# ChenyangLEI/All-In-One-Deflicker

Hardware: AMD Instinct MI355X
Metric: atlas-fit sampled points/sec (stage1, 10k iters) @1/2/4/8 GPU; PSNR vs ref (higher is better)
Workload: dtype f32 (MLP chains f16x3: operands split into 2 fp16 of their value scaled per row, 3 partial products; weight-gradient GEMM bf16x6; fp32 accumulate)

## Files before the change

### all-in-one-deflicker_amd/atlasfit.py

```python
import ctypes as C
import os
import sys

import numpy as np

NET_MAPPING1, NET_ATLAS, NET_MAPPING2, NET_ALPHA = 0, 1, 2, 3
_HERE = os.path.dirname(os.path.abspath(__file__))
_LIB_PATH = os.path.join(_HERE, "lib", "libatlasfit.so")
_lib = None

ABI_SYMBOLS = [
    "af_create", "af_destroy", "af_last_error", "af_upload_video", "af_param_count", "af_set_params",
    "af_get_params", "af_get_adam_state", "af_set_adam_state", "af_pretrain", "af_train_steps",
    "af_render_frame", "af_render_frame_u8", "af_render_frame_at", "af_psnr", "af_sync", "af_debug_forward", "af_set_debug", "af_get_last_grads",
    "af_set_timing", "af_get_timing", "af_step_work", "af_loss_width", "af_config_size", "af_debug_records", "af_debug_plan",
    "af_resize_bilinear", "af_resize_area", "af_flow_consistency", "af_debug_dw_clocks", "af_debug_step_clocks", "af_set_dw_mode", "af_set_mlp_mode", "af_debug_dw_schedule",
    "af_debug_set_dw_cost", "af_debug_tiles", "af_get_modes",
    "af_render_layers", "af_mapping_area", "af_render_atlas_texture", "af_render_edit", "af_render_loss_maps",
    "af_warp_error_pair", "af_warp_error",
    "af_filter_create", "af_filter_destroy", "af_filter_param_count", "af_filter_set_params", "af_filter_reset", "af_filter_frame",
    "af_filter_debug_activation", "af_conv2d",
    "af_raft_create", "af_raft_destroy", "af_raft_param_count", "af_raft_info", "af_raft_set_params", "af_raft_encode", "af_raft_flow",
    "af_raft_step", "af_raft_lookup", "af_raft_debug_activation", "af_raft_conv2d", "af_raft_gru", "af_raft_instance_norm",
]


AF_ERANGE = -6


class AtlasFitError(RuntimeError):
    def __init__(self, code, msg):
        super().__init__("atlasfit error %d: %s" % (code, msg))
        self.code = code


class AfConfig(C.Structure):
    _fields_ = [
        ("resx", C.c_int32), ("resy", C.c_int32), ("number_of_frames", C.c_int32),
        ("samples_batch", C.c_int32),
        ("number_of_channels_mapping1", C.c_int32), ("number_of_layers_mapping1", C.c_int32),
        ("number_of_channels_atlas", C.c_int32), ("number_of_layers_atlas", C.c_int32),
        ("positional_encoding_num_atlas", C.c_int32),
        ("use_positional_encoding_mapping1", C.c_int32),
        ("derivative_amount", C.c_int32),
        ("include_global_rigidity_loss", C.c_int32),
        ("global_rigidity_derivative_amount_fg", C.c_int32),
        ("stop_global_rigidity", C.c_int32),
        ("use_gradient_loss", C.c_int32),
        ("rgb_coeff", C.c_float), ("gradient_loss_coeff", C.c_float), ("rigidity_coeff", C.c_float),
        ("optical_flow_coeff", C.c_float),
        ("global_rigidity_coeff_fg", C.c_float),
        ("uv_mapping_scale", C.c_float),
        ("lr", C.c_float),
        ("pretrain_batch", C.c_int32),
        ("two_layer", C.c_int32),
        ("number_of_channels_mapping2", C.c_int32), ("number_of_layers_mapping2", C.c_int32),
        ("number_of_channels_alpha", C.c_int32), ("number_of_layers_alpha", C.c_int32),
        ("positional_encoding_num_alpha", C.c_int32),
        ("use_positional_encoding_mapping2", C.c_int32),
        ("global_rigidity_derivative_amount_bg", C.c_int32),
        ("stop_bootstrapping_iteration", C.c_int32),
        ("global_rigidity_coeff_bg", C.c_float),
        ("alpha_bootstrapping_factor", C.c_float), ("alpha_flow_factor", C.c_float), ("sparsity_coeff", C.c_float),
        ("number_of_positional_encoding_mapping1", C.c_int32), ("number_of_positional_encoding_mapping2", C.c_int32),
        ("reserved", C.c_int32 * 2),
    ]


REFERENCE_CONFIG = {
    "maximum_number_of_frames": 200, "iters_num": 10001, "samples_batch": 10000, "optical_flow_coeff": 500.0,
    "evaluate_every": 10000, "derivative_amount": 1, "rgb_coeff": 5000, "rigidity_coeff": 1.0,
    "uv_mapping_scale": 0.8, "pretrain_mapping1": True, "pretrain_mapping2": True,
    "alpha_bootstrapping_factor": 2000.0, "alpha_flow_factor": 4900.0, "positional_encoding_num_alpha": 5,
    "number_of_channels_atlas": 256, "number_of_layers_atlas": 8, "number_of_channels_alpha": 256,
    "number_of_layers_alpha": 8, "stop_bootstrapping_iteration": 10000, "number_of_channels_mapping1": 256,
    "number_of_layers_mapping1": 6, "number_of_channels_mapping2": 256, "number_of_layers_mapping2": 4,
    "gradient_loss_coeff": 1000, "use_gradient_loss": True, "sparsity_coeff": 1000.0,
    "positional_encoding_num_atlas": 10, "use_positional_encoding_mapping1": False,
    "number_of_positional_encoding_mapping1": 4, "use_positional_encoding_mapping2": False,
    "number_of_positional_encoding_mapping2": 2, "pretrain_iter_number": 100, "load_checkpoint": False,
    "checkpoint_path": "", "include_global_rigidity_loss": True, "global_rigidity_derivative_amount_fg": 100,
    "global_rigidity_derivative_amount_bg": 100, "global_rigidity_coeff_fg": 5.0, "global_rigidity_coeff_bg": 50.0,
    "stop_global_rigidity": 5000,
}


def default_config(resx, resy, number_of_frames, config=None, two_layer=False, **over):
    cfg = dict(REFERENCE_CONFIG)
    if config:
        cfg.update(config)
    cfg.update(over)
    c = AfConfig()
    c.two_layer = int(bool(two_layer))
    c.number_of_channels_mapping2 = int(cfg["number_of_channels_mapping2"])
    c.number_of_layers_mapping2 = int(cfg["number_of_layers_mapping2"])
    c.number_of_channels_alpha = int(cfg["number_of_channels_alpha"])
    c.number_of_layers_alpha = int(cfg["number_of_layers_alpha"])
    c.positional_encoding_num_alpha = int(cfg["positional_encoding_num_alpha"])
    c.use_positional_encoding_mapping2 = int(bool(cfg["use_positional_encoding_mapping2"]))
    c.number_of_positional_encoding_mapping1 = int(cfg.get("number_of_positional_encoding_mapping1", 4))
    c.number_of_positional_encoding_mapping2 = int(cfg.get("number_of_positional_encoding_mapping2", 2))
    c.global_rigidity_derivative_amount_bg = int(cfg["global_rigidity_derivative_amount_bg"])
    c.stop_bootstrapping_iteration = int(cfg["stop_bootstrapping_iteration"])
    c.global_rigidity_coeff_bg = float(cfg["global_rigidity_coeff_bg"])
    c.alpha_bootstrapping_factor = float(cfg["alpha_bootstrapping_factor"])
    c.alpha_flow_factor = float(cfg["alpha_flow_factor"])
    c.sparsity_coeff = float(cfg["sparsity_coeff"])
    c.resx, c.resy, c.number_of_frames = int(resx), int(resy), int(number_of_frames)
    c.samples_batch = int(cfg["samples_batch"])
    c.number_of_channels_mapping1 = int(cfg["number_of_channels_mapping1"])
    c.number_of_layers_mapping1 = int(cfg["number_of_layers_mapping1"])
    c.number_of_channels_atlas = int(cfg["number_of_channels_atlas"])
    c.number_of_layers_atlas = int(cfg["number_of_layers_atlas"])
    c.positional_encoding_num_atlas = int(cfg["positional_encoding_num_atlas"])
    c.use_positional_encoding_mapping1 = int(bool(cfg["use_positional_encoding_mapping1"]))
    c.derivative_amount = int(cfg["derivative_amount"])
    c.include_global_rigidity_loss = int(bool(cfg["include_global_rigidity_loss"]))
    c.global_rigidity_derivative_amount_fg = int(cfg["global_rigidity_derivative_amount_fg"])
    c.stop_global_rigidity = int(cfg["stop_global_rigidity"])
    c.use_gradient_loss = int(bool(cfg["use_gradient_loss"]))
    c.rgb_coeff = float(cfg["rgb_coeff"])
    c.gradient_loss_coeff = float(cfg["gradient_loss_coeff"])
    c.rigidity_coeff = float(cfg["rigidity_coeff"])
    c.optical_flow_coeff = float(cfg["optical_flow_coeff"])
    c.global_rigidity_coeff_fg = float(cfg["global_rigidity_coeff_fg"])
    c.uv_mapping_scale = float(cfg["uv_mapping_scale"])
    c.lr = float(cfg.get("lr", 1e-4))
    c.pretrain_batch = int(cfg.get("pretrain_batch", 10000))
    return c


def load_library(path=None):
    global _lib
    if _lib is not None:
        return _lib
    import torch
    path = path or os.environ.get("AF_LIB_PATH") or _LIB_PATH
    if not os.path.exists(path):
        raise AtlasFitError(-100, "libatlasfit.so not built: run `python %s`" % os.path.join(_HERE, "build.py"))
    lib = C.CDLL(path)
    vp, i32, i64, u64, sz = C.c_void_p, C.c_int, C.c_int64, C.c_uint64, C.c_size_t
    fp = C.POINTER(C.c_float)
    sig = {
        "af_create": (i32, [C.POINTER(AfConfig), i32, C.POINTER(vp)]),
        "af_destroy": (None, [vp]),
        "af_last_error": (C.c_char_p, [vp]),
        "af_upload_video": (i32, [vp, vp, vp, vp, vp, vp, vp, i32]),
        "af_param_count": (sz, [vp, i32]),
        "af_set_params": (i32, [vp, i32, vp, sz]),
        "af_get_params": (i32, [vp, i32, vp, sz]),
        "af_get_adam_state": (i32, [vp, i32, vp, vp, C.POINTER(i64)]),
        "af_set_adam_state": (i32, [vp, i32, vp, vp, i64]),
        "af_pretrain": (i32, [vp, i32, i32, vp, vp, u64, vp]),
        "af_train_steps": (i32, [vp, i32, i32, vp, u64, vp]),
        "af_render_frame": (i32, [vp, i32, vp, C.POINTER(C.c_double)]),
        "af_render_frame_u8": (i32, [vp, i32, vp, vp, i32, C.POINTER(C.c_double)]),
        "af_render_frame_at": (i32, [vp, i32, i32, i32, vp, vp, vp, C.POINTER(C.c_double), i32]),
        "af_psnr": (i32, [vp, C.POINTER(C.c_double), vp]),
        "af_sync": (i32, [vp]),
        "af_debug_forward": (i32, [vp, i32, vp, i32, vp]),
        "af_set_debug": (i32, [vp, i32]),
        "af_get_last_grads": (i32, [vp, i32, vp, sz]),
        "af_set_timing": (i32, [vp, i32]),
        "af_get_timing": (i32, [vp, vp, vp, vp, i32]),
        "af_step_work": (i32, [vp, i32, C.POINTER(i64 * 4), C.POINTER(C.c_double)]),
        "af_loss_width": (i32, [vp]),
        "af_config_size": (sz, []),
        "af_debug_records": (i32, [vp, vp, i32, vp]),
        "af_debug_plan": (i32, [i32, i32, i32, i32, C.POINTER(i32 * 3)]),
        "af_resize_bilinear": (i32, [i32, vp, i32, i32, i32, i32, vp, i32, i32, i64, i64, i64, C.c_double, C.c_double, i32]),
        "af_resize_area": (i32, [i32, vp, i32, i32, i32, vp, i32, i32, i32]),
        "af_flow_consistency": (i32, [i32, vp, vp, i32, i32, vp, i64, i64, C.c_float, i32]),
        "af_debug_dw_clocks": (i32, [vp, i32, vp, i32]),
        "af_debug_step_clocks": (i32, [vp, i32, vp, i32]),
        "af_debug_dw_schedule": (i32, [vp, i32, vp, i32]),
        "af_set_dw_mode": (i32, [vp, i32]),
        "af_set_mlp_mode": (i32, [vp, i32]),
        "af_debug_set_dw_cost": (i32, [vp, vp, C.c_double]),
        "af_debug_tiles": (i32, [vp, i32, i32, i32, i32, i32, i32, vp]),
        "af_get_modes": (i32, [vp, C.POINTER(i32), C.POINTER(i32)]),
        "af_render_layers": (i32, [vp, i32, vp, vp, vp, vp, vp]),
        "af_mapping_area": (i32, [vp, i32, vp]),
        "af_render_atlas_texture": (i32, [vp, i32, C.c_float, C.c_float, C.c_float, vp]),
        "af_render_edit": (i32, [vp, i32, i32, vp, vp, vp, vp, vp, vp, vp, vp, vp]),
        "af_render_loss_maps": (i32, [vp, i32, vp, vp, vp, vp, vp, vp, vp]),
        "af_warp_error_pair": (i32, [i32, vp, vp, vp, vp, i32, i32, i32, C.POINTER(C.c_double), vp, vp, i32]),
        "af_warp_error": (i32, [vp, i32, i32, vp, C.POINTER(C.c_double)]),
    }
    for name, (res, args) in sig.items():
        f = getattr(lib, name)
        f.restype, f.argtypes = res, args
    if lib.af_config_size() != C.sizeof(AfConfig):
        raise AtlasFitError(-101, "af_config mirror (%d B) does not match libatlasfit.so (%d B): rebuild" % (C.sizeof(AfConfig), lib.af_config_size()))
    _lib = lib
    return lib


def _f32(a):
    return np.ascontiguousarray(a, dtype=np.float32)


def _ptr(a):
    return a.ctypes.data_as(C.c_void_p) if a is not None else None


def imlp_shapes(net, cfg=None, pe_atlas=10, pe_alpha=5):
    hid = {NET_MAPPING1: 256, NET_MAPPING2: 256, NET_ATLAS: 256, NET_ALPHA: 256}
    nl = {NET_MAPPING1: 6, NET_MAPPING2: 4, NET_ATLAS: 8, NET_ALPHA: 8}
    if cfg is not None:
        hid = {NET_MAPPING1: cfg.number_of_channels_mapping1, NET_MAPPING2: cfg.number_of_channels_mapping2,
               NET_ATLAS: cfg.number_of_channels_atlas, NET_ALPHA: cfg.number_of_channels_alpha}
        nl = {NET_MAPPING1: cfg.number_of_layers_mapping1, NET_MAPPING2: cfg.number_of_layers_mapping2,
              NET_ATLAS: cfg.number_of_layers_atlas, NET_ALPHA: cfg.number_of_layers_alpha}
        pe_atlas, pe_alpha = cfg.positional_encoding_num_atlas, cfg.positional_encoding_num_alpha
    if net not in hid:
        raise ValueError("net")
    h, L = int(hid[net]), int(nl[net])
    enc = {NET_MAPPING1: 3, NET_MAPPING2: 3, NET_ATLAS: 4 * pe_atlas, NET_ALPHA: 6 * pe_alpha}[net]
    if cfg is not None:
        if net == NET_MAPPING1 and cfg.use_positional_encoding_mapping1:
            enc = 6 * int(cfg.number_of_positional_encoding_mapping1)
        if net == NET_MAPPING2 and cfg.use_positional_encoding_mapping2:
            enc = 6 * int(cfg.number_of_positional_encoding_mapping2)
    out = {NET_MAPPING1: 2, NET_MAPPING2: 2, NET_ATLAS: 3, NET_ALPHA: 1}[net]
    skips = (4, 7) if net == NET_ATLAS else ()
    dims = []
    for i in range(L):
        fan_in = enc if i == 0 else (h + enc if i in skips else h)
        dims.append((out if i == L - 1 else h, fan_in))
    return dims


def flatten_state_dict(sd, net, cfg=None):
    parts = []
    for i, (o, k) in enumerate(imlp_shapes(net, cfg)):
        w = np.asarray(sd["hidden.%d.weight" % i].detach().cpu().numpy() if hasattr(sd["hidden.%d.weight" % i], "detach") else sd["hidden.%d.weight" % i], dtype=np.float32)
        b = np.asarray(sd["hidden.%d.bias" % i].detach().cpu().numpy() if hasattr(sd["hidden.%d.bias" % i], "detach") else sd["hidden.%d.bias" % i], dtype=np.float32)
        assert w.shape == (o, k) and b.shape == (o,), (i, w.shape, b.shape)
        parts += [w.reshape(-1), b]
    return np.concatenate(parts)


def unflatten_state_dict(flat, net, cfg=None):
    out, off = {}, 0
    for i, (o, k) in enumerate(imlp_shapes(net, cfg)):
        out["hidden.%d.weight" % i] = flat[off:off + o * k].reshape(o, k).copy(); off += o * k
        out["hidden.%d.bias" % i] = flat[off:off + o].copy(); off += o
    assert off == flat.size
    return out


def _util_chk(rc):
# ... 455 lines not shown
```

### all-in-one-deflicker_amd/csrc/af_dev.h

```cpp
#pragma once
#include <stdint.h>

#define AF_HID        256
#define AF_TROWS      32
#define AF_TILE_F     (AF_HID * AF_TROWS)
#define AF_CHUNK_MAX  65536
#define AF_MAX_LAYERS 8
#define AF_KIND_MAP_PE 4
#define AF_MAX_NETS   4
#define AF_REC_F      16
#define AF_LOSS_W     16

enum { AF_NET_MAP1 = 0, AF_NET_ATLAS = 1, AF_NET_MAP2 = 2, AF_NET_ALPHA = 3 };
enum { AF_IN_XYT = 0, AF_IN_PE2 = 1, AF_IN_PE3 = 2 };

enum { REC_RGB = 0, REC_DX = 3, REC_DY = 6, REC_FF = 9, REC_FB = 11, REC_MF = 13, REC_MB = 14, REC_FG = 15 };

enum { DW_8x8 = 0, DW_8x2 = 1, DW_8x1 = 2, DW_1x8 = 3, DW_1x2 = 4 };

struct AfChunk { uint32_t off; uint32_t bytes; };

struct FwdArgs {
  const float* wimg;
  const float* bias;
  const float* in;
  const float* in1;
  float* out;
  float* acts;
  uint32_t* masks;
  float* pe_tile;
  float in_scale, in_shift0, in_shift1;
  int split_row;
  int tile0;
  int NT;
  int nt_stride;
  const int* live_rows;
  int live_base;
  int nl;
};

struct BwdArgs {
  const float* wimg;
  const float* out;
  const float* dout;
  const uint32_t* masks;
  float* dz;
  float* dz_last;
  const float* pe_tile;
  float* din0; float* din1;
  float din_scale;
  int split_row;
  int nrows;
  int tile0;
  int NT;
  int nt_stride;
  const int* live_rows; int live_base;
  int nl;
};

#define AF_STAMP_WG 4096
struct MultiFwd { int n; int net[AF_MAX_NETS]; int wg_end[AF_MAX_NETS]; FwdArgs a[AF_MAX_NETS]; unsigned long long* wg_stamp; };
struct MultiBwd { int n; int net[AF_MAX_NETS]; int wg_end[AF_MAX_NETS]; BwdArgs a[AF_MAX_NETS]; int nprod; unsigned long long* wg_stamp; };

struct DwJob {
  const float* A; const float* B;
  uint32_t a_stride, b_stride;
  int shape;
  uint32_t part_off;
  uint32_t part_blk;
  int live_base;
  const int* live_rows;
};
struct DwSeg { int job, t0, t1, slot; };
#define DW_MAXSEG 16
struct DwArgs {
  const DwJob* jobs; const DwSeg* segs;
  float* partial;
  unsigned long long* wg_clock;
  unsigned long long* wg_stamp;
};

#if defined(__HIPCC__)
#include <hip/hip_runtime.h>
#define AF_STAMP(m, i) if ((m).wg_stamp && threadIdx.x == 0 && blockIdx.x < AF_STAMP_WG) { (m).wg_stamp[blockIdx.x * 4 + 2 * (i)] = __builtin_amdgcn_s_memrealtime(); (m).wg_stamp[blockIdx.x * 4 + 2 * (i) + 1] = __builtin_amdgcn_s_memtime(); }
typedef float    f32x16 __attribute__((ext_vector_type(16)));
typedef float    f32x4  __attribute__((ext_vector_type(4)));
typedef uint32_t u32x4  __attribute__((ext_vector_type(4)));

#define AF_DEV __device__ __forceinline__

AF_DEV __amdgpu_buffer_rsrc_t af_rsrc(const void* p, uint32_t bytes) {
  return __builtin_amdgcn_make_buffer_rsrc((void*)p, 0, (int)bytes, 0x00020000);
}
AF_DEV __amdgpu_buffer_rsrc_t af_rsrc_uniform(const void* p, uint32_t bytes) {
  const uint64_t a = (uint64_t)p;
  const uint32_t lo = __builtin_amdgcn_readfirstlane((uint32_t)a), hi = __builtin_amdgcn_readfirstlane((uint32_t)(a >> 32));
  return __builtin_amdgcn_make_buffer_rsrc((void*)(((uint64_t)hi << 32) | lo), 0, (int)__builtin_amdgcn_readfirstlane(bytes), 0x00020000);
}
AF_DEV float af_bl32(__amdgpu_buffer_rsrc_t r, int voff, int soff) {
  return __builtin_bit_cast(float, __builtin_amdgcn_raw_buffer_load_b32(r, voff, soff, 0));
}
AF_DEV f32x4 af_bl128(__amdgpu_buffer_rsrc_t r, int voff, int soff) {
  return __builtin_bit_cast(f32x4, __builtin_amdgcn_raw_buffer_load_b128(r, voff, soff, 0));
}
AF_DEV void af_bs32(float v, __amdgpu_buffer_rsrc_t r, int voff, int soff) {
  __builtin_amdgcn_raw_buffer_store_b32(__builtin_bit_cast(uint32_t, v), r, voff, soff, 0);
}
#ifndef AF_TILE_AUX
#define AF_TILE_AUX 2
#endif
AF_DEV void af_bs32_tile(float v, __amdgpu_buffer_rsrc_t r, int voff, int soff) {
  __builtin_amdgcn_raw_buffer_store_b32(__builtin_bit_cast(uint32_t, v), r, voff, soff, AF_TILE_AUX);
}
AF_DEV void af_bs128(f32x4 v, __amdgpu_buffer_rsrc_t r, int voff, int soff) {
  __builtin_amdgcn_raw_buffer_store_b128(__builtin_bit_cast(u32x4, v), r, voff, soff, 0);
}
AF_DEV void af_glds16(const void* g, void* lds) {
  __builtin_amdgcn_global_load_lds((const __attribute__((address_space(1))) void*)g,
                                   (__attribute__((address_space(3))) void*)lds, 16, 0, 0);
}
AF_DEV void af_wait_vm0() { asm volatile("s_waitcnt vmcnt(0)" ::: "memory"); }

AF_DEV void af_stage_chunk(const char* src, uint32_t bytes, char* dst, int tid, int wave) {
  const int nit = (int)(bytes >> 12);
  for (int it = 0; it < nit; ++it)
    af_glds16(src + it * 4096 + tid * 16, dst + it * 4096 + wave * 1024);
}

__host__ __device__ inline int af_pe_slot_of_feature(int pe_kind, int e) {
  if (pe_kind != 2) return e;
  int h, rho;
  if (e < 24) { int k = e / 6, c = e % 6; h = k >> 1; rho = (k & 1) * 6 + c; }
  else        { int c = e - 24; h = c / 3; rho = 12 + c % 3; }
  return ((rho >> 2) << 3) + (h << 2) + (rho & 3);
}
__host__ __device__ inline uint32_t af_img_index(uint32_t mpad, uint32_t m, uint32_t k) {
  return ((((k >> 3) * 2 + ((k >> 2) & 1)) * mpad + m) << 2) + (k & 3);
}
#endif
```

### all-in-one-deflicker_amd/csrc/elem.h

```cpp
#pragma once
#include "af_dev.h"

struct PackArgs {
  const float* frames;
  const float* flow_f;
  const float* flow_b;
  const float* mask_f;
  const float* mask_b;
  const float* mask_fg;
  float* table;
  int resx, resy, F;
  unsigned long long* nvalid;
};

struct ResizeArgs {
  const void* src; int src_u8;
  int sh, sw, ch;
  float* dst; int dh, dw;
  long long pix_stride, ch_stride, offset;
  double scale0, scale1;
};
enum { AREA_GENERAL = 0, AREA_BLOCK = 1, AREA_2X2 = 2 };
struct AreaArgs {
  const unsigned char* src; int sh, sw, ch;
// ... 17 lines not shown
  int N, resx, resy, F;
  float half_main, half_grad, half_frames;
  int d_local, d_global, nseg;
  float* coords;
  float* x0_tile;
  float* samples;
  int* counts;
  float* coords2;
  float* x0_tile2;
  float* coordsA;
  int d_global2;
  int* flow_rank;
  unsigned long long* scan;
  uint32_t epoch;
  unsigned long long* ticket;
  unsigned long long ticket_base;
  int* live;
};

struct LossArgs {
  const float* samples; const float* out_map; const float* out_atlas;
  float* dout_map; float* dout_atlas;
  const int* counts;
  const int* flow_rank; const int* live;
  float* loss_part;
  int N, nseg;
  float L, uv_scale; int d_local, d_global;
  float c_rgb, c_grad, c_rig, c_grig, c_flow;
};

struct LossSegArgs {
  const float* samples;
  const float* out_m1; const float* out_m2; const float* out_alpha; const float* out_atlas;
  float* dout_m1; float* dout_m2; float* dout_alpha; float* dout_atlas;
  const int* counts; float* loss_part;
  const int* flow_rank; const int* live;
  int N, nseg;
  float L, uv_scale; int d_local, d_global_fg, d_global_bg;
  float c_rgb, c_grad, c_rig, c_grig_fg, c_grig_bg, c_flow, c_boot, c_aflow, c_sparse;
};

struct PrePrepArgs {
  const int64_t* ys; const int64_t* xs;
  uint64_t seed; uint32_t iter;
  int N, resx, resy;
  float half_main, t;
  float* coords; float* x0_tile;
};
struct PreLossArgs { const float* coords; const float* out_map; float* dout_map; float* loss_part; int N; float uv_scale; };

struct CoordsAtArgs {
  float* coords;
  int resx, resy;
  int oh, ow;
  float half_main, t;
  long long r0; int n, n_pad;
};
struct FinishAtArgs {
  const float* out_atlas; const float* out_alpha; size_t row2;
  int n;
  float* rgb_out;
  unsigned char* u8_out;
  const unsigned char* ref;
  double* sse_part;
};

struct AdamJob {
  uint32_t part_off, part_blk, nslots, pld;
  uint32_t out_real, in_real, out_real_pad;
  uint32_t p_off;
  uint32_t p_ld;
  uint32_t col0;
  int32_t  b_off;
  uint32_t f_off;
  uint32_t f_mpad;
  int32_t  b_img_off;
  uint32_t b_mpad;
  uint32_t bias_img_off;
  uint32_t pe_kind;
  uint32_t hid_cols;
  int32_t  sf_off; uint32_t sf_kind, sf_mpad, sf_k0;
  int32_t  sb_off; uint32_t sb_kind, sb_mpad;
  int32_t  hf_off, hb_off;
};
struct AdamHyper { float step_size, bc2_sqrt, one_minus_b1, beta2, one_minus_b2, eps; };
struct AdamBufs { float* params; float* m; float* v; float* img_f; float* img_b; float* bias_img; char* sf; char* sb; char* hf; char* hb; };
struct AdamArgs {
  const AdamJob* jobs; const float* partial;
  AdamBufs bufs; AdamHyper hy;
  float* grad_out;
  const float* loss_part; float* loss_out; int* counts; int loss_nblk;
  int* nan_flag;
  int check_counts;
};

struct EditArgs {
  const float* uv1; const float* uv2; const float* out_alpha;
  int npix, res;
  int active[2]; float minx[2], miny[2], pixel_size[2];
  const float* tex[2];
  float* edit; float* edit_layer[2]; float* use[2];
};

struct LossMapArgs {
  float* coords; const float* table; size_t rec0;
  int resx, resy, rows_pad, frame, d;
  int seg_c, seg_ym, seg_xm, seg_t;
  float half_main, half_frames, t_centre;
  const float* out_m1; const float* out_m2;
  const float* out_alpha;
  const float* out_atlas;
  int flow_map;
  float L, uv_scale;
  float* rigidity1; float* rigidity2; float* flow1; float* flow2; float* flow_alpha; float* rgb_err; float* residual;
};

struct WarpErrArgs {
  const float* img1; const float* img2; const float* flow12; const float* flow21;
  size_t img_pair_stride, flow_pair_stride;
  int h, w, align_corners;
  float* noc; float* warped;
  double* part;
};
```

### all-in-one-deflicker_amd/csrc/elem.hip

```cpp
#include "af_dev.h"
#include "elem.h"

AF_DEV void philox4x32(uint32_t c0, uint32_t c1, uint32_t c2, uint32_t c3, uint32_t k0, uint32_t k1, uint32_t (&o)[4]) {
#pragma unroll
  for (int r = 0; r < 10; ++r) {
    const uint64_t p0 = (uint64_t)0xD2511F53u * c0, p1 = (uint64_t)0xCD9E8D57u * c2;
    const uint32_t n0 = (uint32_t)(p1 >> 32) ^ c1 ^ k0, n1 = (uint32_t)p1;
    const uint32_t n2 = (uint32_t)(p0 >> 32) ^ c3 ^ k1, n3 = (uint32_t)p0;
    c0 = n0; c1 = n1; c2 = n2; c3 = n3;
    k0 += 0x9E3779B9u; k1 += 0xBB67AE85u;
  }
  o[0] = c0; o[1] = c1; o[2] = c2; o[3] = c3;
}
AF_DEV uint64_t af_rand_below(uint64_t seed, uint32_t iter, uint32_t n, uint32_t stream, uint64_t bound) {
  uint32_t o[4];
  philox4x32(n, iter, stream, 0x41544c53u, (uint32_t)seed, (uint32_t)(seed >> 32), o);
  const uint64_t r = ((uint64_t)o[1] << 32) | o[0];
  return __umul64hi(r, bound);
}

__global__ void k_pack_table(PackArgs a) {
  const size_t P2 = (size_t)a.resx * a.resy;
  const size_t idx = (size_t)blockIdx.x * blockDim.x + threadIdx.x;
  const bool in_range = idx < P2 * a.F;
// ... 504 lines not shown
  const int y = a.ys ? (int)a.ys[n] : (int)af_rand_below(a.seed, a.iter, (uint32_t)n, 1u, (uint64_t)a.resy);
  const int x = a.xs ? (int)a.xs[n] : (int)af_rand_below(a.seed, a.iter, (uint32_t)n, 2u, (uint64_t)a.resx);
  const float xc = (float)x / a.half_main - 1.f, yc = (float)y / a.half_main - 1.f;
  f32x4 v = {xc, yc, a.t, 0.f};
  *(f32x4*)(a.coords + (size_t)n * 4) = v;
  if (a.x0_tile) {
    float* tl = a.x0_tile + ((size_t)n >> 5) * 1024 + (n & 31);
    tl[0] = xc; tl[32] = yc; tl[64] = a.t;
  }
}

__global__ __launch_bounds__(256) void k_pre_loss(PreLossArgs a) {
  __shared__ float red[4];
  const int n = blockIdx.x * blockDim.x + threadIdx.x;
  float l = 0.f;
  if (n < a.N) {
    const f32x4 c = *(const f32x4*)(a.coords + (size_t)n * 4);
    const f32x4 o = *(const f32x4*)(a.out_map + (size_t)n * 4);
    const float eu = c[0] * a.uv_scale - o[0], ev = c[1] * a.uv_scale - o[1];
    l = sqrtf(eu * eu + ev * ev);
    const float w = l > 0.f ? -1.f / (l * (float)a.N) : 0.f;
    put_d2(a.dout_map, (size_t)n, w * eu, w * ev);
  }
  l = block_sum(l, red);
  if (threadIdx.x == 0) { float* o = a.loss_part + (size_t)blockIdx.x * AF_LOSS_W; o[0] = l; for (int i = 1; i < AF_LOSS_W; ++i) o[i] = 0.f; }
}

AF_DEV uint16_t bf16_rne(float x) {
  const uint32_t u = __builtin_bit_cast(uint32_t, x);
  return (uint16_t)((u + 0x7fffu + ((u >> 16) & 1u)) >> 16);
}
AF_DEV void emit_bf3(char* block, uint32_t m, uint32_t k, float p) {
  const uint32_t T = k >> 5, q = (k >> 3) & 3, hh = (k >> 2) & 1, pp = k & 3;
  const uint32_t s = 2 * T + (q >> 1), i = 4 * (q & 1) + pp;
  const uint16_t h = bf16_rne(p);
  const float r1 = p - __builtin_bit_cast(float, (uint32_t)h << 16);
  const uint16_t mi = bf16_rne(r1);
  const float r2 = r1 - __builtin_bit_cast(float, (uint32_t)mi << 16);
  const uint16_t lo = bf16_rne(r2);
  const size_t base = ((size_t)((s * 8 + (m >> 5)) * 3) * 2 + hh) * 32 * 16 + (size_t)(m & 31) * 16 + i * 2;
  *(uint16_t*)(block + base) = h;
  *(uint16_t*)(block + base + 1024) = mi;
  *(uint16_t*)(block + base + 2048) = lo;
}

AF_DEV void emit_hf2(char* block, uint32_t m, uint32_t k, float p) {
  const uint32_t T = k >> 5, q = (k >> 3) & 3, hh = (k >> 2) & 1, pp = k & 3;
  const uint32_t s = 2 * T + (q >> 1), i = 4 * (q & 1) + pp;
  const float ps = p * 4096.f;
  const _Float16 h = (_Float16)ps;
  const _Float16 l = (_Float16)(ps - (float)h);
  const size_t base = ((size_t)((s * 8 + (m >> 5)) * 2) * 2 + hh) * 32 * 16 + (size_t)(m & 31) * 16 + i * 2;
  *(_Float16*)(block + base) = h;
  *(_Float16*)(block + base + 1024) = l;
}

AF_DEV void emit_weight(const AdamJob& j, const AdamBufs& b, uint32_t o, uint32_t i, float p) {
  const uint32_t col = j.col0 + i;
  uint32_t k = col;
  if (col >= j.hid_cols) k = j.hid_cols + (uint32_t)af_pe_slot_of_feature((int)j.pe_kind, (int)(col - j.hid_cols));
  b.img_f[j.f_off + af_img_index(j.f_mpad, o, k)] = p;
  if (j.b_img_off >= 0 && col < (j.hid_cols ? j.hid_cols : j.p_ld)) {
    const uint32_t mrow = j.hid_cols ? col : (uint32_t)af_pe_slot_of_feature((int)j.pe_kind, (int)col);
    b.img_b[(uint32_t)j.b_img_off + af_img_index(j.b_mpad, mrow, o)] = p;
    if (b.sb && j.sb_off >= 0) {
      if (j.sb_kind == 0) ((float*)(b.sb + j.sb_off))[af_img_index(j.sb_mpad, mrow, o)] = p;
      else                emit_bf3(b.sb + j.sb_off, mrow, o, p);
    }
    if (b.hb && j.hb_off >= 0) {
      if (j.sb_kind == 0) ((float*)(b.hb + j.hb_off))[af_img_index(j.sb_mpad, mrow, o)] = p;
      else                emit_hf2(b.hb + j.hb_off, mrow, o, p);
    }
  }
  if (b.sf && j.sf_off >= 0) {
    if (j.sf_kind == 0) ((float*)(b.sf + j.sf_off))[af_img_index(j.sf_mpad, o, k - j.sf_k0)] = p;
    else                emit_bf3(b.sf + j.sf_off, o, k, p);
  }
  if (b.hf && j.hf_off >= 0) {
    if (j.sf_kind == 0) ((float*)(b.hf + j.hf_off))[af_img_index(j.sf_mpad, o, k - j.sf_k0)] = p;
    else                emit_hf2(b.hf + j.hf_off, o, k, p);
  }
}

template <bool UPDATE>
__global__ __launch_bounds__(256) void k_adam(AdamArgs a) {
  const AdamJob j = a.jobs[blockIdx.y];
  const uint32_t e = blockIdx.x * blockDim.x + threadIdx.x;
  const uint32_t nw = j.out_real * j.in_real;
  const uint32_t nb = j.b_off >= 0 ? j.out_real : 0u;
  if (e < nw + nb) {
    const bool is_bias = e >= nw;
    const uint32_t o = is_bias ? e - nw : e / j.in_real;
    const uint32_t i = is_bias ? 0u : e - o * j.in_real;
    const uint32_t pidx = is_bias ? (uint32_t)j.b_off + o : j.p_off + o * j.p_ld + i;
    float p = a.bufs.params[pidx];
    if (UPDATE) {
      const float* pp = a.partial + j.part_off + (is_bias ? j.out_real_pad * j.pld + o : o * j.pld + i);
      float g = 0.f;
      uint32_t s = 0;
      for (; s + 8 <= j.nslots; s += 8) {
        float t[8];
#pragma unroll
        for (int q = 0; q < 8; ++q) t[q] = pp[(size_t)(s + q) * j.part_blk];
#pragma unroll
        for (int q = 0; q < 8; ++q) g += t[q];
      }
      if (s + 4 <= j.nslots) {
        float t[4];
#pragma unroll
        for (int q = 0; q < 4; ++q) t[q] = pp[(size_t)(s + q) * j.part_blk];
#pragma unroll
        for (int q = 0; q < 4; ++q) g += t[q];
        s += 4;
      }
      if (s + 2 <= j.nslots) {
        const float t0 = pp[(size_t)s * j.part_blk], t1 = pp[(size_t)(s + 1) * j.part_blk];
        g += t0; g += t1; s += 2;
      }
      if (s < j.nslots) g += pp[(size_t)s * j.part_blk];
      float m = a.bufs.m[pidx], v = a.bufs.v[pidx];
      m = m + (g - m) * a.hy.one_minus_b1;
      v = v * a.hy.beta2 + (a.hy.one_minus_b2 * g) * g;
      const float denom = sqrtf(v) / a.hy.bc2_sqrt + a.hy.eps;
      p = p - a.hy.step_size * (m / denom);
      a.bufs.m[pidx] = m; a.bufs.v[pidx] = v; a.bufs.params[pidx] = p;
      if (a.grad_out) a.grad_out[pidx] = g;
    }
    if (a.nan_flag && !(fabsf(p) <= 3.4028235e38f)) atomicOr(a.nan_flag, 1);
    if (a.nan_flag && a.bufs.hf && !is_bias && j.sf_kind == 1 && fabsf(p) >= 8.f) atomicOr(a.nan_flag, 2);
    if (is_bias) a.bufs.bias_img[j.bias_img_off + o] = p;
    else emit_weight(j, a.bufs, o, i, p);
  }
  if (UPDATE && blockIdx.x == 0 && blockIdx.y == 0 && a.loss_out) {
    if (threadIdx.x < AF_LOSS_W - 2) {
      float s = 0.f;
      for (int b = 0; b < a.loss_nblk; ++b) s += a.loss_part[b * AF_LOSS_W + threadIdx.x];
      a.loss_out[threadIdx.x] = s;
      if (a.nan_flag && !(s == s)) atomicOr(a.nan_flag, 1);
    } else if (threadIdx.x < AF_LOSS_W) {
      a.loss_out[threadIdx.x] = (float)a.counts[threadIdx.x - (AF_LOSS_W - 2)];
      if (a.nan_flag && a.check_counts && a.counts[threadIdx.x - (AF_LOSS_W - 2)] == 0) atomicOr(a.nan_flag, 1);
      a.counts[threadIdx.x - (AF_LOSS_W - 2)] = 0;
    }
  }
}

__global__ void k_frame_coords(float* coords, int resx, int resy, float half_main, float t, int npix_pad) {
  const int r = blockIdx.x * blockDim.x + threadIdx.x;
  if (r >= npix_pad) return;
  const int npix = resx * resy;
  f32x4 v = {0.f, 0.f, 0.f, 0.f};
  if (r < npix) { const int y = r / resx, x = r - y * resx; v[0] = (float)x / half_main - 1.f; v[1] = (float)y / half_main - 1.f; v[2] = t; }
  *(f32x4*)(coords + (size_t)r * 4) = v;
}

__global__ __launch_bounds__(256) void k_frame_finish(const float* out_atlas, const float* table, float* rgb_out, double* sse_part,
                                                     int npix, size_t rec0) {
  __shared__ double red[4];
  const int r = blockIdx.x * blockDim.x + threadIdx.x;
  double sse = 0.0;
  if (r < npix) {
    const f32x4 t = *(const f32x4*)(out_atlas + (size_t)r * 4);
    const float* rec = table + (rec0 + r) * AF_REC_F;
#pragma unroll
    for (int c = 0; c < 3; ++c) {
      const float v = (t[c] + 1.f) * 0.5f;
      rgb_out[(size_t)r * 3 + c] = v;
      const double d = (double)rec[REC_RGB + c] - (double)v;
      sse += d * d;
    }
  }
#pragma unroll
  for (int o = 32; o > 0; o >>= 1) sse += __shfl_xor(sse, o);
  if ((threadIdx.x & 63) == 0) red[threadIdx.x >> 6] = sse;
  __syncthreads();
  if (threadIdx.x == 0) sse_part[blockIdx.x] = (red[0] + red[1]) + (red[2] + red[3]);
}

__global__ __launch_bounds__(256) void k_frame_finish_seg(const float* out_atlas, const float* out_alpha, size_t row2, const float* table,
                                                         float* rgb_out, double* sse_part, int npix, size_t rec0) {
  __shared__ double red[4];
  const int r = blockIdx.x * blockDim.x + threadIdx.x;
  double sse = 0.0;
  if (r < npix) {
    const f32x4 t1 = *(const f32x4*)(out_atlas + (size_t)r * 4);
    const f32x4 t2 = *(const f32x4*)(out_atlas + (row2 + r) * 4);
    const float al = alpha_of(out_alpha[(size_t)r * 4]);
    const float* rec = table + (rec0 + r) * AF_REC_F;
#pragma unroll
    for (int c = 0; c < 3; ++c) {
      const float v = ((t1[c] + 1.f) * 0.5f) * al + ((t2[c] + 1.f) * 0.5f) * (1.f - al);
      rgb_out[(size_t)r * 3 + c] = v;
      const double d = (double)rec[REC_RGB + c] - (double)v;
      sse += d * d;
    }
  }
#pragma unroll
  for (int o = 32; o > 0; o >>= 1) sse += __shfl_xor(sse, o);
  if ((threadIdx.x & 63) == 0) red[threadIdx.x >> 6] = sse;
  __syncthreads();
  if (threadIdx.x == 0) sse_part[blockIdx.x] = (red[0] + red[1]) + (red[2] + red[3]);
}
// ... 138 lines not shown
```

### all-in-one-deflicker_amd/csrc/host.hip

```cpp
#include <hip/hip_runtime.h>
#include <float.h>
#include <math.h>
#include <cmath>
#include <stdio.h>
#include <string.h>
#include <algorithm>
#include <string>
#include <vector>

#include "../../include/atlasfit.h"
#include "af_dev.h"
#include "elem.h"

extern "C" {
int af_launch_fwd_multi(MultiFwd* m, int train, hipStream_t s);
int af_launch_bwd_multi(MultiBwd* m, hipStream_t s);
int af_mlp_init();
int af_mlp_chunk_bytes(int net, int which, int nl);
int af_launch_fwd_multi_bf(MultiFwd* m, int train, hipStream_t s);
int af_launch_bwd_multi_bf(MultiBwd* m, hipStream_t s);
int af_mlp_bf_init();
int af_mlp_chunk_bytes_bf(int net, int which, int nl);
int af_launch_fwd_multi_hf(MultiFwd* m, int train, hipStream_t s);
int af_launch_bwd_multi_hf(MultiBwd* m, hipStream_t s);
int af_mlp_hf_init();
int af_mlp_chunk_bytes_hf(int net, int which, int nl);
int af_launch_fwd16(int net, const FwdArgs* a, hipStream_t s);
int af_launch_bwd16(int net, const BwdArgs* a, hipStream_t s);
int af_mlp16_init();
int af_launch_dw(const DwArgs* a, int nwg, int mode, hipStream_t s);
int af_dw_init();
int af_launch_pack(const PackArgs* a, hipStream_t s);
int af_launch_prep(const PrepArgs* a, hipStream_t s);
int af_launch_loss_single(const LossArgs* a, hipStream_t s);
int af_launch_loss_seg(const LossSegArgs* a, hipStream_t s);
int af_launch_resize(const ResizeArgs* a, hipStream_t s);
int af_launch_resize_area(const AreaArgs* a, hipStream_t s);
int af_launch_consistency(const ConsistencyArgs* a, hipStream_t s);
int af_launch_frame_finish_seg(const float* out_atlas, const float* out_alpha, size_t row2, const float* table, float* rgb_out, double* sse_part,
                               int npix, size_t rec0, hipStream_t s);
int af_launch_pre_prep(const PrePrepArgs* a, hipStream_t s);
int af_launch_pre_loss(const PreLossArgs* a, hipStream_t s);
int af_launch_adam(const AdamArgs* a, int njobs, int update, hipStream_t s);
int af_launch_frame_coords(float* coords, int resx, int resy, float half_main, float t, int npix_pad, hipStream_t s);
int af_launch_frame_finish(const float* out_atlas, const float* table, float* rgb_out, double* sse_part, int npix, size_t rec0, hipStream_t s);
int af_launch_frame_u8(const float* rgb, unsigned char* out, int npix, hipStream_t s);
int af_launch_frame_coords_at(const CoordsAtArgs* a, hipStream_t s);
int af_launch_frame_finish_at(const FinishAtArgs* a, hipStream_t s);
int af_launch_layer_finish(const float* uv1s, const float* uv2s, const float* out_atlas, size_t row2, const float* out_alpha, int npix,
                           float* uv1, float* uv2, float* alpha, float* rgb1, float* rgb2, hipStream_t s);
int af_launch_area_reduce(const float* uv, const float* out_alpha, const float* table, size_t rec0, int npix, int which, float* part, hipStream_t s);
int af_launch_tex_coords(float* coords, int res, int row0, int nrows, float sx, float ex, float sy, float ey, int rows_pad, hipStream_t s);
int af_launch_tex_finish(const float* out_atlas, int rows, float* out, hipStream_t s);
int af_launch_edit(const EditArgs* a, hipStream_t s);
int af_launch_lossmap_rows(const LossMapArgs* a, hipStream_t s);
int af_launch_lossmap_finish(const LossMapArgs* a, hipStream_t s);
int af_launch_warp_error(const WarpErrArgs* a, int kind, int npairs, hipStream_t s);
}

namespace {

thread_local std::string g_create_error;

struct StreamPlan {
  size_t f_base = 0, b_base = 0;
  long long f_hid[AF_MAX_LAYERS], f_fp[AF_MAX_LAYERS], b_hid[AF_MAX_LAYERS], b_fp[AF_MAX_LAYERS];
};

struct NetDesc {
  int kern = -1;
  int id = -1, NL = 0, in_kind = 0, in_feat0 = 0, out = 0, pe_feats = 0, pe_kind = 0;
  unsigned skip = 0; bool dx0 = false; bool used = false;
  int in_feat[AF_MAX_LAYERS], out_feat[AF_MAX_LAYERS];
  size_t w_off[AF_MAX_LAYERS], b_off[AF_MAX_LAYERS];
  size_t nparams = 0, p_base = 0;
  int hid = AF_HID; size_t nlogical = 0; std::vector<uint32_t> lmap;
  size_t f_off[AF_MAX_LAYERS]; int f_mpad[AF_MAX_LAYERS], f_groups[AF_MAX_LAYERS];
  long long b_off_img[AF_MAX_LAYERS]; int b_mpad[AF_MAX_LAYERS];
  size_t f_base = 0, b_base = 0, bias_base = 0;
  std::vector<AfChunk> fchunks, bchunks;
  StreamPlan bf, hf;
  int nt_cap = 0;
  float *coords = nullptr, *x0_tile = nullptr;
  float *acts = nullptr, *dz = nullptr, *dz_last = nullptr, *pe_tile = nullptr, *out_buf = nullptr, *dout = nullptr;
  uint32_t* masks = nullptr;
};

struct Sched {
  std::vector<DwJob> jobs; std::vector<AdamJob> ajobs; std::vector<DwSeg> segs;
  int nwg = 0; size_t partial_floats = 0;
  DwJob* d_jobs = nullptr; AdamJob* d_ajobs = nullptr; DwSeg* d_segs = nullptr;
};

struct TimedEv { int cls; hipEvent_t a, b; };

}

struct af_handle {
  af_config cfg;
  bool seg = false;
  int device = 0; hipStream_t stream = nullptr; int ncu = 256;
  std::string err;
  NetDesc nets[AF_MAX_NETS];
  size_t total_params = 0, img_f_floats = 0, img_b_floats = 0, bias_floats = 0, sf_bytes = 0, sb_bytes = 0;
  char *img_sf = nullptr, *img_sb = nullptr;
  char *img_hf = nullptr, *img_hb = nullptr; size_t hf_bytes = 0, hb_bytes = 0;
  int mlp_mode = 3;
  float *params = nullptr, *adam_m = nullptr, *adam_v = nullptr, *pre_m = nullptr, *pre_v = nullptr, *grads = nullptr;
  float *img_f = nullptr, *img_b = nullptr, *bias_img = nullptr;
  long long adam_step = 0;
  float* table = nullptr; bool have_video = false;
  int N = 0;
  float *samples = nullptr, *loss_part = nullptr, *loss_log = nullptr;
  int* counts = nullptr; int loss_nblk_cap = 0; size_t loss_log_cap = 0;
  int* nan_flag = nullptr;
  int cur_nseg = 0;
  int* flow_rank = nullptr; unsigned long long* scan = nullptr; int* live = nullptr; uint32_t prep_epoch = 0; unsigned long long prep_tickets = 0;
  unsigned long long* nvalid = nullptr; double p_valid[2] = {1.0, 1.0};
  int plan_flow_rows = 0;
  Sched sched[4]; float* partial = nullptr; size_t partial_cap = 0;
  unsigned long long* dw_clock = nullptr;
  unsigned long long* step_stamp = nullptr;
  int render_rows_cap = 0; float *r_coords = nullptr, *r_uv = nullptr, *r_uv2 = nullptr, *r_al = nullptr, *r_t = nullptr, *r_rgb = nullptr; double* r_sse = nullptr;
  unsigned char* r_u8 = nullptr;
  unsigned char* r_at = nullptr;
  std::vector<double> frame_sse; std::vector<char> frame_sse_valid;
  float* l_buf = nullptr; size_t l_cap = 0;
  bool debug = false; unsigned timing = 0, timing_every = 1; bool timing_live = true;
  double flop_fwd[AF_MAX_NETS] = {0}, flop_dx[AF_MAX_NETS] = {0};
  bool dw_cost_set = false; double dw_cost[5] = {0}, dw_seg_cost = 0;
  int dw_mode = 1;
  std::vector<TimedEv> evs; double t_ms[16] = {0}, t_flops[16] = {0}; long long t_cnt[16] = {0};

  int fail(int code, const char* what, hipError_t e = hipSuccess) {
    char buf[512];
    if (e != hipSuccess) snprintf(buf, sizeof buf, "%s: %s", what, hipGetErrorString(e));
    else snprintf(buf, sizeof buf, "%s", what);
    err = buf;
    return code;
  }
};

#define HCHK(x) do { hipError_t e_ = (x); if (e_ != hipSuccess) return h->fail(AF_EHIP, #x, e_); } while (0)
#define AF_TEX_MAX 16384
#define LCHK(x) do { int r_ = (x); if (r_ != 0) return h->fail(AF_EHIP, #x, (hipError_t)r_); } while (0)

namespace {

enum { T_PREP = 0, T_FWD_1 = 1, T_FWD_2 = 2, T_LOSS = 3, T_BWD_1 = 4, T_BWD_2 = 5, T_DW = 6, T_ADAM = 7 };

template <class T> hipError_t dalloc(T** p, size_t n) { return hipMalloc((void**)p, std::max<size_t>(n, 1) * sizeof(T)); }

void describe_net(NetDesc& n, int id, int NL, int in_kind, int pe_freqs, int out, unsigned skip, bool dx0, int hid = AF_HID) {
  n.id = id; n.kern = (in_kind == AF_IN_PE3 && out == 2) ? AF_KIND_MAP_PE : id; n.NL = NL; n.in_kind = in_kind; n.out = out; n.skip = skip; n.dx0 = dx0; n.used = true;
  const int in_dim = in_kind == AF_IN_PE2 ? 2 : 3;
  n.pe_feats = in_kind == AF_IN_XYT ? 0 : 2 * in_dim * pe_freqs;
  n.pe_kind = in_kind == AF_IN_PE3 ? 2 : (in_kind == AF_IN_PE2 ? 1 : 0);
  n.in_feat0 = in_kind == AF_IN_XYT ? 3 : n.pe_feats;
  size_t off = 0;
  for (int l = 0; l < NL; ++l) {
    n.in_feat[l] = l == 0 ? n.in_feat0 : (AF_HID + (((skip >> l) & 1) ? n.pe_feats : 0));
    n.out_feat[l] = l == NL - 1 ? out : AF_HID;
    n.w_off[l] = off; off += (size_t)n.in_feat[l] * n.out_feat[l];
    n.b_off[l] = off; off += n.out_feat[l];
  }
  n.nparams = off;
  n.hid = hid; n.nlogical = off; n.lmap.clear();
  if (hid != AF_HID) {
    for (int l = 0; l < NL; ++l) {
      const int pin = n.in_feat[l], pout = n.out_feat[l];
      const int lout = l == NL - 1 ? out : hid;
      const int extra = l == 0 ? n.in_feat0 : (pin - AF_HID);
// ... 31 lines not shown
      for (int c = 0; c < 4; ++c) { n.fchunks.push_back({(uint32_t)foff, (uint32_t)(8 * gbytes)}); foff += 8 * gbytes; }
      if ((n.skip >> l) & 1) { const size_t bytes = round_up(peg * gbytes, 4096); n.fchunks.push_back({(uint32_t)foff, (uint32_t)bytes}); foff += bytes; }
    }
  }
  f_cursor += foff / 4;
  size_t boff = 0;
  for (int l = 0; l < n.NL; ++l) { n.b_off_img[l] = -1; n.b_mpad[l] = 0; }
  for (int l = n.NL - 1; l >= (n.dx0 ? 0 : 1); --l) {
    const int mpad = l == 0 ? 64 : AF_HID;
    const int groups = l == n.NL - 1 ? 1 : 32;
    n.b_mpad[l] = mpad; n.b_off_img[l] = (long long)(n.b_base + boff / 4);
    const size_t gbytes = (size_t)2 * mpad * 16;
    if (groups * gbytes <= AF_CHUNK_MAX) { n.bchunks.push_back({(uint32_t)boff, (uint32_t)(groups * gbytes)}); boff += groups * gbytes; }
    else for (int c = 0; c < 4; ++c) { n.bchunks.push_back({(uint32_t)boff, (uint32_t)(8 * gbytes)}); boff += 8 * gbytes; }
  }
  b_cursor += boff / 4;
}

struct ChainFamily {
  int cls;
  int (*fwd)(MultiFwd*, int, hipStream_t);
  int (*bwd)(MultiBwd*, hipStream_t);
  int (*chunk_bytes)(int net, int which, int nl);
  int hid_chunks, wbytes;
};
const ChainFamily k_fp32 = {0, af_launch_fwd_multi, af_launch_bwd_multi, af_mlp_chunk_bytes, 4, 4};
const ChainFamily k_bf16x6 = {1, af_launch_fwd_multi_bf, af_launch_bwd_multi_bf, af_mlp_chunk_bytes_bf, 8, 6};
const ChainFamily k_f16x3 = {2, af_launch_fwd_multi_hf, af_launch_bwd_multi_hf, af_mlp_chunk_bytes_hf, 4, 4};
const ChainFamily& chain_family(int mlp_mode) { return mlp_mode == 3 ? k_f16x3 : (mlp_mode ? k_bf16x6 : k_fp32); }

bool plan_stream(NetDesc& n, StreamPlan& sp, const ChainFamily& fam, size_t& f_cursor, size_t& b_cursor) {
  const auto chunk_bytes = fam.chunk_bytes; const int hid_chunks = fam.hid_chunks;
  const int peg = n.in_kind == AF_IN_PE3 ? 4 : (n.in_kind == AF_IN_PE2 ? 5 : 0);
  const int cb_l0 = chunk_bytes(n.kern, 0, n.NL), cb_hid = chunk_bytes(n.kern, 1, n.NL), cb_skip = chunk_bytes(n.kern, 2, n.NL);
  const int cb_last = chunk_bytes(n.kern, 3, n.NL), cb_blast = chunk_bytes(n.kern, 4, n.NL), cb_bl0h = chunk_bytes(n.kern, 5, n.NL);
  for (int l = 0; l < AF_MAX_LAYERS; ++l) sp.f_hid[l] = sp.f_fp[l] = sp.b_hid[l] = sp.b_fp[l] = -1;
  sp.f_base = f_cursor; sp.b_base = b_cursor;
  size_t off = 0;
  sp.f_fp[0] = (long long)off; off += cb_l0;
  if ((size_t)cb_l0 < round_up((size_t)(n.in_kind == AF_IN_XYT ? 1 : peg) * 2 * AF_HID * 16, 4096)) return false;
  for (int l = 1; l < n.NL - 1; ++l) {
    sp.f_hid[l] = (long long)off; off += (size_t)hid_chunks * cb_hid;
    if ((n.skip >> l) & 1) { sp.f_fp[l] = (long long)off; off += cb_skip; }
  }
  sp.f_fp[n.NL - 1] = (long long)off; off += cb_last;
  f_cursor += off;
  off = 0;
  sp.b_fp[n.NL - 1] = (long long)off; off += cb_blast;
  for (int l = n.NL - 2; l >= 1; --l) { sp.b_hid[l] = (long long)off; off += (size_t)hid_chunks * cb_hid; }
  if (n.dx0) { sp.b_fp[0] = (long long)off; off += (size_t)2 * cb_bl0h; }
  b_cursor += off;
  return hid_chunks * cb_hid == AF_HID * AF_HID * fam.wbytes && cb_blast == 2 * AF_HID * 16 && 2 * cb_bl0h == 32 * 2 * 64 * 16;
}

bool check_chunk_plan(const NetDesc& n) {
  std::vector<int> f, b;
  f.push_back(af_mlp_chunk_bytes(n.kern, 0, n.NL));
  for (int l = 1; l < n.NL - 1; ++l) { for (int c = 0; c < 4; ++c) f.push_back(af_mlp_chunk_bytes(n.kern, 1, n.NL)); if ((n.skip >> l) & 1) f.push_back(af_mlp_chunk_bytes(n.kern, 2, n.NL)); }
  f.push_back(af_mlp_chunk_bytes(n.kern, 3, n.NL));
  b.push_back(af_mlp_chunk_bytes(n.kern, 4, n.NL));
  for (int l = n.NL - 2; l >= 1; --l) for (int c = 0; c < 4; ++c) b.push_back(af_mlp_chunk_bytes(n.kern, 1, n.NL));
  if (n.dx0) b.push_back(af_mlp_chunk_bytes(n.kern, 5, n.NL));
  auto same = [](const std::vector<AfChunk>& plan, const std::vector<int>& want) {
    if (plan.size() != want.size()) return false;
    uint32_t off = 0;
    for (size_t i = 0; i < plan.size(); ++i) { if (plan[i].off != off || (int)plan[i].bytes != want[i]) return false; off += plan[i].bytes; }
    return true;
  };
  return same(n.fchunks, f) && same(n.bchunks, b);
}

int shape_tiles(int shape, int& To, int& Ti) {
  switch (shape) {
    case DW_8x8: To = 8; Ti = 8; return 256;
    case DW_8x2: To = 8; Ti = 2; return 64;
    case DW_8x1: To = 8; Ti = 1; return 32;
    case DW_1x8: To = 1; Ti = 8; return 32;
    default:     To = 1; Ti = 2; return 16;
  }
}

struct NetUse { NetDesc* n; int NT; int live_base = -1; int NT_plan = -1; };

bool build_sched(af_handle* h, Sched& sc, const std::vector<NetUse>& uses) {
  sc.jobs.clear(); sc.ajobs.clear(); sc.segs.clear();
  std::vector<int> job_nt, job_cap;
  int cur_live_base = -1, cur_cap = 0;
  auto add = [&](NetDesc& n, int NT, int l, int shape, const float* A, uint32_t as, const float* B, uint32_t bs,
                 int col0, int in_real, bool owns_bias) {
    int To, Ti; shape_tiles(shape, To, Ti);
    DwJob j{}; j.A = A; j.B = B; j.a_stride = as; j.b_stride = bs; j.shape = shape;
    if (cur_live_base >= 0) { j.live_base = cur_live_base; j.live_rows = h->live; }
    j.part_blk = (uint32_t)(To * 32 * Ti * 32 + To * 32);
    sc.jobs.push_back(j); job_nt.push_back(NT); job_cap.push_back(cur_cap);
    AdamJob a{};
    a.part_blk = j.part_blk; a.pld = Ti * 32; a.out_real = n.out_feat[l]; a.in_real = in_real; a.out_real_pad = To * 32;
    a.p_off = (uint32_t)(n.p_base + n.w_off[l] + col0); a.p_ld = n.in_feat[l]; a.col0 = col0;
    a.b_off = owns_bias ? (int32_t)(n.p_base + n.b_off[l]) : -1;
    a.f_off = (uint32_t)n.f_off[l]; a.f_mpad = n.f_mpad[l];
    a.b_img_off = (int32_t)n.b_off_img[l]; a.b_mpad = n.b_mpad[l];
    a.bias_img_off = (uint32_t)(n.bias_base + (size_t)l * AF_HID);
    a.pe_kind = n.pe_kind;
    a.hid_cols = l == 0 ? (n.in_kind == AF_IN_XYT ? n.in_feat[l] : 0) : AF_HID;
    const bool last_l = l == n.NL - 1;
    a.sf_k0 = 0; a.sf_mpad = last_l ? 4 : AF_HID; a.sb_mpad = l == 0 ? 64 : AF_HID;
    if (l == 0 || last_l)  { a.sf_kind = 0; a.sf_off = (int32_t)(n.bf.f_base + n.bf.f_fp[l]); }
    else if (col0 == 0)    { a.sf_kind = 1; a.sf_off = (int32_t)(n.bf.f_base + n.bf.f_hid[l]); }
    else                   { a.sf_kind = 0; a.sf_off = (int32_t)(n.bf.f_base + n.bf.f_fp[l]); a.sf_k0 = AF_HID; }
    if (n.b_off_img[l] < 0)      { a.sb_kind = 0; a.sb_off = -1; }
    else if (last_l || l == 0)   { a.sb_kind = 0; a.sb_off = (int32_t)(n.bf.b_base + n.bf.b_fp[l]); }
    else                         { a.sb_kind = 1; a.sb_off = (int32_t)(n.bf.b_base + n.bf.b_hid[l]); }
    a.hf_off = (int32_t)(n.hf.f_base + (a.sf_kind == 1 ? n.hf.f_hid[l] : n.hf.f_fp[l]));
    a.hb_off = a.sb_off < 0 ? -1 : (int32_t)(n.hf.b_base + (a.sb_kind == 1 ? n.hf.b_hid[l] : n.hf.b_fp[l]));
    sc.ajobs.push_back(a);
  };
  for (const NetUse& u : uses) {
    NetDesc& n = *u.n;
    const int NT = u.NT_plan >= 0 ? std::min(u.NT_plan, u.NT) : u.NT;
    cur_live_base = u.live_base; cur_cap = u.NT;
    const size_t ts = (size_t)u.NT * AF_TILE_F;
    for (int l = 0; l < n.NL; ++l) {
      const bool last = l == n.NL - 1, sk = (n.skip >> l) & 1;
      if (l == 0) {
        if (n.in_kind == AF_IN_XYT) add(n, NT, 0, DW_8x1, n.dz, AF_TILE_F, n.x0_tile, 1024, 0, 3, true);
        else                        add(n, NT, 0, DW_8x2, n.dz, AF_TILE_F, n.pe_tile, 2048, 0, n.pe_feats, true);
      } else if (!last) {
        add(n, NT, l, DW_8x8, n.dz + l * ts, AF_TILE_F, n.acts + (l - 1) * ts, AF_TILE_F, 0, AF_HID, true);
        if (sk) add(n, NT, l, DW_8x2, n.dz + l * ts, AF_TILE_F, n.pe_tile, 2048, AF_HID, n.pe_feats, false);
      } else {
        add(n, NT, l, DW_1x8, n.dz_last, 1024, n.acts + (l - 1) * ts, AF_TILE_F, 0, AF_HID, true);
        if (sk) add(n, NT, l, DW_1x2, n.dz_last, 1024, n.pe_tile, 2048, AF_HID, n.pe_feats, false);
      }
    }
  }
  const int nj = (int)sc.jobs.size();
  static const double kTileCost[3][5] = {{306.0, 94.0, 62.0, 62.0, 46.0}, {306.0, 166.0, 140.0, 143.0, 97.0}, {306.0, 168.0, 157.0, 150.0, 95.0}};
  double seg_cost = 60.0;
  double cost_row[5];
  for (int i = 0; i < 5; ++i) cost_row[i] = kTileCost[h->dw_mode][i];
  if (h->dw_cost_set) {
    for (int i = 0; i < 5; ++i) cost_row[i] = h->dw_cost[i];
    if (h->dw_seg_cost > 0) seg_cost = h->dw_seg_cost;
  }
  auto tile_cost = [&](int j) { return cost_row[sc.jobs[j].shape]; };
  double work = 0;
  for (int j = 0; j < nj; ++j) work += tile_cost(j) * job_nt[j];
  int nwg = (int)std::min<double>(h->ncu, std::max(1.0, work / (4.0 * 276.0)));
  std::vector<int> order(nj);
  for (int j = 0; j < nj; ++j) order[j] = j;
  std::stable_sort(order.begin(), order.end(), [&](int a, int b) { return tile_cost(a) * job_nt[a] > tile_cost(b) * job_nt[b]; });
  std::vector<int> nslots(nj, 0);
  std::vector<std::vector<DwSeg>> wg(nwg);
  const double total = work + seg_cost * (nj + nwg);
  const double target = total / nwg;
  int w = 0; double cum = 0;
  for (int oi = 0; oi < nj; ++oi) {
    const int j = order[oi]; int t = 0; const double tc = tile_cost(j);
    while (t < job_nt[j]) {
      const double bound = (w + 1) * target;
      int take;
      if (w == nwg - 1) take = job_nt[j] - t;
      else {
        take = (int)floor((bound - cum - seg_cost) / tc + 0.5);
        if (take <= 0 || (int)wg[w].size() >= DW_MAXSEG) { ++w; continue; }
        take = std::min(take, job_nt[j] - t);
      }
      wg[w].push_back({j, t, t + take, nslots[j]++});
      cum += seg_cost + tc * take; t += take;
      if (t == job_nt[j]) wg[w].back().t1 = job_cap[j];
      if (w < nwg - 1 && cum >= bound - 0.5 * tc) ++w;
    }
  }
  sc.nwg = nwg;
  for (int i = 0; i < nwg; ++i) if (wg[i].size() > DW_MAXSEG) return false;
  sc.segs.assign((size_t)nwg * DW_MAXSEG, DwSeg{-1, 0, 0, 0});
  for (int i = 0; i < nwg; ++i)
    for (size_t s = 0; s < wg[i].size() && s < DW_MAXSEG; ++s) sc.segs[(size_t)i * DW_MAXSEG + s] = wg[i][s];
  size_t off = 0;
  for (int j = 0; j < nj; ++j) {
    sc.jobs[j].part_off = (uint32_t)off; sc.ajobs[j].part_off = (uint32_t)off; sc.ajobs[j].nslots = nslots[j];
    off += (size_t)nslots[j] * sc.jobs[j].part_blk;
  }
  sc.partial_floats = off;
  return true;
}

hipError_t upload_sched(Sched& sc) {
  hipError_t e;
  if (sc.d_jobs) { (void)hipFree(sc.d_jobs); (void)hipFree(sc.d_ajobs); (void)hipFree(sc.d_segs); sc.d_jobs = nullptr; }
  if ((e = dalloc(&sc.d_jobs, sc.jobs.size())) != hipSuccess) return e;
  if ((e = dalloc(&sc.d_ajobs, sc.ajobs.size())) != hipSuccess) return e;
  if ((e = dalloc(&sc.d_segs, sc.segs.size())) != hipSuccess) return e;
  if ((e = hipMemcpy(sc.d_jobs, sc.jobs.data(), sc.jobs.size() * sizeof(DwJob), hipMemcpyHostToDevice)) != hipSuccess) return e;
  if ((e = hipMemcpy(sc.d_ajobs, sc.ajobs.data(), sc.ajobs.size() * sizeof(AdamJob), hipMemcpyHostToDevice)) != hipSuccess) return e;
  return hipMemcpy(sc.d_segs, sc.segs.data(), sc.segs.size() * sizeof(DwSeg), hipMemcpyHostToDevice);
}

int tiles_of(int rows) { return (rows + 31) / 32; }

int planned_flow_rows(const af_handle* h) {
  const double N = h->N, pf = h->p_valid[0], pb = h->p_valid[1];
  const double e = N * (pf + pb), sd = sqrt(std::max(0.0, N * (pf * (1.0 - pf) + pb * (1.0 - pb))));
  return (int)std::min(2.0 * N, ceil(e + 4.0 * sd) + 32.0);
}

bool build_main_scheds(af_handle* h) {
  NetDesc& M = h->nets[AF_NET_MAP1]; NetDesc& A = h->nets[AF_NET_ATLAS]; NetDesc& M2 = h->nets[AF_NET_MAP2]; NetDesc& AL = h->nets[AF_NET_ALPHA];
  const int N = h->N; const bool seg = h->seg;
  h->plan_flow_rows = planned_flow_rows(h);
  for (int v = 0; v < 2; ++v) {
    const int nseg = v == 0 ? 9 : 7, fb = (nseg - 2) * N;
    std::vector<NetUse> uses = {{&M, tiles_of(nseg * N), fb, tiles_of(fb + h->plan_flow_rows)}};
    if (seg) { uses.push_back({&M2, tiles_of(nseg * N), fb, tiles_of(fb + h->plan_flow_rows)}); uses.push_back({&AL, tiles_of(5 * N), 3 * N, tiles_of(3 * N + h->plan_flow_rows)}); }
    uses.push_back({&A, tiles_of((seg ? 6 : 3) * N)});
    if (!build_sched(h, h->sched[v], uses)) return false;
  }
  return true;
}

hipError_t alloc_net_buffers(NetDesc& n, int rows_cap, bool own_coords) {
  n.nt_cap = tiles_of(rows_cap);
  const size_t nt = n.nt_cap, rp = nt * 32;
  hipError_t e;
  if ((e = dalloc(&n.acts, (size_t)(n.NL - 1) * nt * AF_TILE_F)) != hipSuccess) return e;
  if ((e = dalloc(&n.dz, (size_t)(n.NL - 1) * nt * AF_TILE_F)) != hipSuccess) return e;
  if ((e = dalloc(&n.masks, (size_t)(n.NL - 1) * nt * 64 * 4)) != hipSuccess) return e;
  if ((e = dalloc(&n.dz_last, nt * 1024)) != hipSuccess) return e;
  if ((e = dalloc(&n.pe_tile, n.pe_feats ? nt * 2048 : 1)) != hipSuccess) return e;
  if ((e = dalloc(&n.out_buf, rp * 4)) != hipSuccess) return e;
  if ((e = dalloc(&n.dout, rp * 4)) != hipSuccess) return e;
  if ((e = hipMemset(n.dz_last, 0, nt * 1024 * 4)) != hipSuccess) return e;
  if (n.pe_feats && (e = hipMemset(n.pe_tile, 0, nt * 2048 * 4)) != hipSuccess) return e;
  if ((e = hipMemset(n.out_buf, 0, rp * 16)) != hipSuccess) return e;
  if ((e = hipMemset(n.dout, 0, rp * 16)) != hipSuccess) return e;
  if (own_coords) {
    if ((e = dalloc(&n.coords, rp * 4)) != hipSuccess) return e;
    if ((e = hipMemset(n.coords, 0, rp * 16)) != hipSuccess) return e;
    if (n.in_kind == AF_IN_XYT) {
      if ((e = dalloc(&n.x0_tile, nt * 1024)) != hipSuccess) return e;
      if ((e = hipMemset(n.x0_tile, 0, nt * 4096)) != hipSuccess) return e;
    }
  }
  return hipSuccess;
}

void free_net(NetDesc& n) {
  (void)hipFree(n.acts); (void)hipFree(n.dz); (void)hipFree(n.masks); (void)hipFree(n.dz_last); (void)hipFree(n.pe_tile); (void)hipFree(n.out_buf); (void)hipFree(n.dout);
  (void)hipFree(n.coords); (void)hipFree(n.x0_tile);
}

const float* chain_wimg(const af_handle* h, const NetDesc& n, bool fwd) {
  switch (chain_family(h->mlp_mode).cls) {
    case 0:  return fwd ? h->img_f + n.f_base : h->img_b + n.b_base;
    case 1:  return (const float*)(fwd ? h->img_sf + n.bf.f_base : h->img_sb + n.bf.b_base);
    default: return (const float*)(fwd ? h->img_hf + n.hf.f_base : h->img_hb + n.hf.b_base);
  }
}

FwdArgs fwd_args(af_handle* h, NetDesc& n, const float* in, float* out, int NT, bool train) {
  FwdArgs a{};
  a.wimg = chain_wimg(h, n, true); a.bias = h->bias_img + n.bias_base;
  a.in = in; a.in1 = nullptr; a.out = out; a.acts = train ? n.acts : nullptr; a.masks = train ? n.masks : nullptr; a.pe_tile = train ? n.pe_tile : nullptr;
  a.in_scale = 0.5f; a.in_shift0 = 0.5f; a.in_shift1 = -0.5f; a.split_row = 0x7fffffff;
  a.NT = NT; a.nt_stride = NT; a.nl = n.NL;
  return a;
}

BwdArgs bwd_args(af_handle* h, NetDesc& n, int NT) {
  BwdArgs a{};
  a.wimg = chain_wimg(h, n, false); a.out = n.out_buf; a.dout = n.dout; a.masks = n.masks;
  a.dz = n.dz; a.dz_last = n.dz_last; a.pe_tile = n.pe_tile; a.din0 = nullptr; a.din1 = nullptr; a.din_scale = 0.5f;
  a.split_row = 0x7fffffff; a.nrows = 0; a.NT = NT; a.nt_stride = NT; a.nl = n.NL;
  return a;
}
FwdArgs fp32_images(FwdArgs a, const af_handle* h, const NetDesc& n) { a.wimg = h->img_f + n.f_base; return a; }
BwdArgs fp32_images(BwdArgs a, const af_handle* h, const NetDesc& n) { a.wimg = h->img_b + n.b_base; return a; }

struct Timer {
  af_handle* h; int cls; hipEvent_t a = nullptr, b = nullptr;
  Timer(af_handle* h_, int c, double flops = 0.0) : h(h_), cls(c) {
    if (on()) { (void)hipEventCreate(&a); (void)hipEventCreate(&b); (void)hipEventRecord(a, h->stream); h->t_flops[cls] += flops; }
  }
  ~Timer() { if (on()) { (void)hipEventRecord(b, h->stream); h->evs.push_back({cls, a, b}); } }
  bool on() const { return h->timing_live && ((h->timing >> cls) & 1u); }
};

void drain_timers(af_handle* h) {
  for (TimedEv& e : h->evs) {
    float ms = 0; (void)hipEventSynchronize(e.b); (void)hipEventElapsedTime(&ms, e.a, e.b);
    h->t_ms[e.cls] += ms; h->t_cnt[e.cls] += 1;
    (void)hipEventDestroy(e.a); (void)hipEventDestroy(e.b);
  }
  h->evs.clear();
}

AdamHyper adam_hyper(double lr, long long step) {
  const double b1 = 0.9, b2 = 0.999, eps = 1e-8;
  const double bc1 = 1.0 - pow(b1, (double)step), bc2 = 1.0 - pow(b2, (double)step);
  AdamHyper hy;
  hy.step_size = (float)(lr / bc1); hy.bc2_sqrt = (float)sqrt(bc2);
  hy.one_minus_b1 = (float)(1.0 - b1); hy.beta2 = (float)b2; hy.one_minus_b2 = (float)(1.0 - b2); hy.eps = (float)eps;
  return hy;
}

AdamBufs adam_bufs(af_handle* h, float* m, float* v) {
  const int cls = chain_family(h->mlp_mode).cls;
  const bool bf = cls == 1, hf = cls == 2;
  return {h->params, m, v, h->img_f, h->img_b, h->bias_img, bf ? h->img_sf : nullptr, bf ? h->img_sb : nullptr, hf ? h->img_hf : nullptr, hf ? h->img_hb : nullptr};
}

int repack(af_handle* h, Sched& sc) {
  AdamArgs a{};
  a.jobs = sc.d_ajobs; a.partial = h->partial;
  a.bufs = adam_bufs(h, h->adam_m, h->adam_v);
  a.nan_flag = h->nan_flag;
  LCHK(af_launch_adam(&a, (int)sc.ajobs.size(), 0, h->stream));
  return 0;
}

bool glob_on(const af_config& c, int iter) { return c.include_global_rigidity_loss && iter <= c.stop_global_rigidity; }

double part_rows(int tile0, int NT, int rows_total) { return (double)std::max(0, std::min(NT * 32, rows_total) - tile0 * 32); }

struct FwdPart { int net; FwdArgs a; int rows_total; };
struct BwdPart { int net; BwdArgs a; int rows_total; };

int launch_fwd(af_handle* h, int cls, std::initializer_list<FwdPart> parts, bool train) {
  MultiFwd m{}; double fl = 0;
  for (const FwdPart& p : parts) {
    if (p.a.NT <= p.a.tile0) continue;
    m.net[m.n] = h->nets[p.net].kern; m.a[m.n] = p.a; ++m.n;
    fl += part_rows(p.a.tile0, p.a.NT, p.rows_total) * h->flop_fwd[p.net];
  }
  if (m.n == 0) return 0;
  if (h->step_stamp && train && (cls == T_FWD_1 || cls == T_FWD_2)) m.wg_stamp = h->step_stamp + (size_t)(cls == T_FWD_1 ? 0 : 1) * AF_STAMP_WG * 4;
  Timer t(h, cls, fl);
  LCHK(chain_family(h->mlp_mode).fwd(&m, train ? 1 : 0, h->stream));
  return 0;
}
int launch_bwd(af_handle* h, int cls, std::initializer_list<BwdPart> parts) {
  MultiBwd m{}; double fl = 0;
  for (const BwdPart& p : parts) {
    if (p.a.NT <= p.a.tile0) continue;
    m.net[m.n] = h->nets[p.net].kern; m.a[m.n] = p.a; ++m.n;
    fl += part_rows(p.a.tile0, p.a.NT, p.rows_total) * h->flop_dx[p.net];
  }
  if (m.n == 0) return 0;
  if (h->step_stamp && (cls == T_BWD_1 || cls == T_BWD_2)) m.wg_stamp = h->step_stamp + (size_t)(cls == T_BWD_1 ? 2 : 3) * AF_STAMP_WG * 4;
  Timer t(h, cls, fl);
  m.nprod = h->mlp_mode == 2 ? 3 : 6;
  LCHK(chain_family(h->mlp_mode).bwd(&m, h->stream));
  return 0;
}
template <class Args> Args with_live(Args a, const af_handle* h, int live_base) { a.live_rows = h->live; a.live_base = live_base; return a; }
FwdArgs tile_range(FwdArgs a, int t0, int t1) { a.tile0 = t0; a.NT = t1; return a; }
BwdArgs tile_range(BwdArgs a, int t0, int t1) { a.tile0 = t0; a.NT = t1; return a; }

void plan_mapping_split(int ncu, int NT_map, int NT_atlas, int dep_rows, int& T1, int& T2) {
  const int round = ncu * 4, t1 = NT_map / round * round;
  T1 = t1 * 32 >= dep_rows ? t1 : NT_map;
  const int extra = (NT_atlas + 3) / 4 + (NT_map - T1 + 3) / 4 - ncu;
  T2 = std::min(NT_map, T1 + 4 * std::max(0, extra));
}

int finish_step(af_handle* h, Sched& sc, float* m, float* v, long long step, float* loss_out, int loss_nblk, double dw_flops, bool check_counts = true) {
  { Timer t(h, T_DW, dw_flops); DwArgs d{sc.d_jobs, sc.d_segs, h->partial, h->dw_clock, h->step_stamp ? h->step_stamp + (size_t)4 * AF_STAMP_WG * 4 : nullptr}; LCHK(af_launch_dw(&d, sc.nwg, h->dw_mode, h->stream)); }
  {
    Timer t(h, T_ADAM);
    AdamArgs a{};
    a.jobs = sc.d_ajobs; a.partial = h->partial;
    a.bufs = adam_bufs(h, m, v);
    a.hy = adam_hyper(h->cfg.lr, step);
    a.grad_out = h->debug ? h->grads : nullptr;
    a.loss_part = h->loss_part; a.loss_out = loss_out; a.counts = h->counts; a.loss_nblk = loss_nblk; a.nan_flag = h->nan_flag;
    a.check_counts = check_counts ? 1 : 0;
    LCHK(af_launch_adam(&a, (int)sc.ajobs.size(), 1, h->stream));
  }
  return 0;
}

int take_nan_flag(af_handle* h, int& flag) {
  flag = 0;
  HCHK(hipMemcpy(&flag, h->nan_flag, 4, hipMemcpyDeviceToHost));
  if (flag) HCHK(hipMemset(h->nan_flag, 0, 4));
  return 0;
}

int ensure_loss_log(af_handle* h, size_t steps) {
  if (steps * AF_LOSS_W <= h->loss_log_cap) return 0;
  if (h->loss_log) (void)hipFree(h->loss_log);
  h->loss_log = nullptr; h->loss_log_cap = 0;
  HCHK(dalloc(&h->loss_log, steps * AF_LOSS_W));
  h->loss_log_cap = steps * AF_LOSS_W;
  return 0;
}

int enqueue_single_step(af_handle* h, int i, const int64_t* d_inds, uint64_t seed, float* loss_out) {
  const af_config& c = h->cfg;
  NetDesc& M = h->nets[AF_NET_MAP1]; NetDesc& A = h->nets[AF_NET_ATLAS];
  const int N = h->N, L = std::max(c.resx, c.resy);
  const bool glob = glob_on(c, i);
  const int nseg = glob ? 9 : 7;
  Sched& sc = h->sched[glob ? 0 : 1];
  const int NT_map = tiles_of(nseg * N), NT_atlas = tiles_of(3 * N);
  if (nseg != h->cur_nseg) {
    HCHK(hipMemsetAsync(M.dout, 0, (size_t)M.nt_cap * 32 * 16, h->stream));
    h->cur_nseg = nseg;
  }
  {
    Timer t(h, T_PREP);
    PrepArgs p{};
    p.table = h->table; p.inds = d_inds; p.seed = seed; p.iter = (uint32_t)i;
    p.N = N; p.resx = c.resx; p.resy = c.resy; p.F = c.number_of_frames;
    p.half_main = (float)(L / 2.0); p.half_grad = (float)(c.resx / 2.0); p.half_frames = (float)(c.number_of_frames / 2.0);
    p.d_local = c.derivative_amount; p.d_global = c.global_rigidity_derivative_amount_fg; p.nseg = nseg;
    p.coords = M.coords; p.x0_tile = M.x0_tile; p.samples = h->samples; p.counts = h->counts;
    p.flow_rank = h->flow_rank; p.scan = h->scan; p.live = h->live; p.epoch = ++h->prep_epoch;
    p.ticket = h->scan + (N + 255) / 256; p.ticket_base = h->prep_tickets;
    LCHK(af_launch_prep(&p, h->stream));
    h->prep_tickets += (unsigned long long)((N + 255) / 256);
  }
  int rc, T1, T2;
  plan_mapping_split(h->ncu, std::min(NT_map, tiles_of((nseg - 2) * N + h->plan_flow_rows)), NT_atlas, 3 * N, T1, T2);
  const int flow_base = (nseg - 2) * N;
  const FwdArgs fm = with_live(fwd_args(h, M, M.coords, M.out_buf, NT_map, true), h, flow_base);
  if ((rc = launch_fwd(h, T_FWD_1, {{AF_NET_MAP1, tile_range(fm, 0, T1), nseg * N}}, true)) != 0) return rc;
  if ((rc = launch_fwd(h, T_FWD_2, {{AF_NET_MAP1, tile_range(fm, T1, T2), nseg * N},
                                    {AF_NET_ATLAS, fwd_args(h, A, M.out_buf, A.out_buf, NT_atlas, true), 3 * N},
                                    {AF_NET_MAP1, tile_range(fm, T2, NT_map), nseg * N}}, true)) != 0) return rc;
  {
    Timer t(h, T_LOSS);
    LossArgs l{};
    l.samples = h->samples; l.out_map = M.out_buf; l.out_atlas = A.out_buf; l.dout_map = M.dout; l.dout_atlas = A.dout;
    l.counts = h->counts; l.loss_part = h->loss_part; l.N = N; l.nseg = nseg; l.flow_rank = h->flow_rank; l.live = h->live;
    l.L = (float)L; l.uv_scale = c.uv_mapping_scale; l.d_local = c.derivative_amount; l.d_global = c.global_rigidity_derivative_amount_fg;
    l.c_rgb = c.rgb_coeff; l.c_grad = c.use_gradient_loss ? c.gradient_loss_coeff : 0.f; l.c_rig = c.rigidity_coeff;
    l.c_grig = glob ? c.global_rigidity_coeff_fg : 0.f; l.c_flow = c.optical_flow_coeff;
    LCHK(af_launch_loss_single(&l, h->stream));
  }
  h->adam_step += 1;
  {
    BwdArgs ba = bwd_args(h, A, NT_atlas); ba.din0 = M.dout; ba.nrows = 3 * N;
    const BwdArgs bm = with_live(bwd_args(h, M, NT_map), h, flow_base);
    if ((rc = launch_bwd(h, T_BWD_1, {{AF_NET_MAP1, tile_range(bm, T1, T2), nseg * N}, {AF_NET_ATLAS, ba, 3 * N},
                                      {AF_NET_MAP1, tile_range(bm, T2, NT_map), nseg * N}})) != 0) return rc;
    if ((rc = launch_bwd(h, T_BWD_2, {{AF_NET_MAP1, tile_range(bm, 0, T1), nseg * N}})) != 0) return rc;
  }
  const double dwf = (double)nseg * N * h->flop_fwd[AF_NET_MAP1] + 3.0 * N * h->flop_fwd[AF_NET_ATLAS];
  return finish_step(h, sc, h->adam_m, h->adam_v, h->adam_step, loss_out, (N + 255) / 256, dwf);
}

int enqueue_seg_step(af_handle* h, int i, const int64_t* d_inds, uint64_t seed, float* loss_out) {
  const af_config& c = h->cfg;
  NetDesc& M1 = h->nets[AF_NET_MAP1]; NetDesc& M2 = h->nets[AF_NET_MAP2]; NetDesc& A = h->nets[AF_NET_ATLAS]; NetDesc& AL = h->nets[AF_NET_ALPHA];
  const int N = h->N, L = std::max(c.resx, c.resy);
  const bool glob = glob_on(c, i);
  const int nseg = glob ? 9 : 7;
  Sched& sc = h->sched[glob ? 0 : 1];
  const int NT_map = tiles_of(nseg * N), NT_atlas = tiles_of(6 * N), NT_alpha = tiles_of(5 * N);
  if (nseg != h->cur_nseg) {
    HCHK(hipMemsetAsync(M1.dout, 0, (size_t)M1.nt_cap * 32 * 16, h->stream));
    HCHK(hipMemsetAsync(M2.dout, 0, (size_t)M2.nt_cap * 32 * 16, h->stream));
    h->cur_nseg = nseg;
  }
  {
    Timer t(h, T_PREP);
    PrepArgs p{};
    p.table = h->table; p.inds = d_inds; p.seed = seed; p.iter = (uint32_t)i;
    p.N = N; p.resx = c.resx; p.resy = c.resy; p.F = c.number_of_frames;
    p.half_main = (float)(L / 2.0); p.half_grad = (float)(c.resx / 2.0); p.half_frames = (float)(c.number_of_frames / 2.0);
    p.d_local = c.derivative_amount; p.d_global = c.global_rigidity_derivative_amount_fg; p.nseg = nseg;
    p.coords = M1.coords; p.x0_tile = M1.x0_tile; p.samples = h->samples; p.counts = h->counts;
    p.coords2 = M2.coords; p.x0_tile2 = M2.x0_tile; p.coordsA = AL.coords; p.d_global2 = c.global_rigidity_derivative_amount_bg;
    p.flow_rank = h->flow_rank; p.scan = h->scan; p.live = h->live; p.epoch = ++h->prep_epoch;
    p.ticket = h->scan + (N + 255) / 256; p.ticket_base = h->prep_tickets;
    LCHK(af_launch_prep(&p, h->stream));
    h->prep_tickets += (unsigned long long)((N + 255) / 256);
  }
  int rc;
  const int wg_atlas = (NT_atlas + 3) / 4, pad = (h->ncu - wg_atlas % h->ncu) % h->ncu;
  const int T_al = std::max(0, std::min(NT_alpha, tiles_of(3 * N + h->plan_flow_rows)) - 4 * pad);
  const int flow_base = (nseg - 2) * N;
  const FwdArgs fal = with_live(fwd_args(h, AL, AL.coords, AL.out_buf, NT_alpha, true), h, 3 * N);
  FwdArgs fat = fwd_args(h, A, M1.out_buf, A.out_buf, NT_atlas, true);
  fat.in1 = M2.out_buf; fat.split_row = 3 * N;
  if ((rc = launch_fwd(h, T_FWD_1, {{AF_NET_ALPHA, tile_range(fal, 0, T_al), 5 * N},
                                    {AF_NET_MAP1, with_live(fwd_args(h, M1, M1.coords, M1.out_buf, NT_map, true), h, flow_base), nseg * N},
                                    {AF_NET_MAP2, with_live(fwd_args(h, M2, M2.coords, M2.out_buf, NT_map, true), h, flow_base), nseg * N}}, true)) != 0) return rc;
  if ((rc = launch_fwd(h, T_FWD_2, {{AF_NET_ATLAS, fat, 6 * N}, {AF_NET_ALPHA, tile_range(fal, T_al, NT_alpha), 5 * N}}, true)) != 0) return rc;
  {
    Timer t(h, T_LOSS);
    LossSegArgs l{};
    l.samples = h->samples; l.out_m1 = M1.out_buf; l.out_m2 = M2.out_buf; l.out_alpha = AL.out_buf; l.out_atlas = A.out_buf;
    l.dout_m1 = M1.dout; l.dout_m2 = M2.dout; l.dout_alpha = AL.dout; l.dout_atlas = A.dout;
    l.counts = h->counts; l.loss_part = h->loss_part; l.N = N; l.nseg = nseg; l.flow_rank = h->flow_rank; l.live = h->live;
    l.L = (float)L; l.uv_scale = c.uv_mapping_scale; l.d_local = c.derivative_amount;
    l.d_global_fg = c.global_rigidity_derivative_amount_fg; l.d_global_bg = c.global_rigidity_derivative_amount_bg;
    l.c_rgb = c.rgb_coeff; l.c_grad = c.use_gradient_loss ? c.gradient_loss_coeff : 0.f; l.c_rig = c.rigidity_coeff;
    l.c_grig_fg = glob ? c.global_rigidity_coeff_fg : 0.f; l.c_grig_bg = glob ? c.global_rigidity_coeff_bg : 0.f;
    l.c_flow = c.optical_flow_coeff;
    l.c_boot = i > c.stop_bootstrapping_iteration ? 0.f : c.alpha_bootstrapping_factor;
    l.c_aflow = c.alpha_flow_factor; l.c_sparse = c.sparsity_coeff;
    LCHK(af_launch_loss_seg(&l, h->stream));
  }
  h->adam_step += 1;
  {
    BwdArgs ba = bwd_args(h, A, NT_atlas);
    ba.din0 = M1.dout; ba.din1 = M2.dout; ba.split_row = 3 * N; ba.nrows = 6 * N;
    const BwdArgs bal = with_live(bwd_args(h, AL, NT_alpha), h, 3 * N);
    if ((rc = launch_bwd(h, T_BWD_1, {{AF_NET_ATLAS, ba, 6 * N}, {AF_NET_ALPHA, tile_range(bal, T_al, NT_alpha), 5 * N}})) != 0) return rc;
    if ((rc = launch_bwd(h, T_BWD_2, {{AF_NET_ALPHA, tile_range(bal, 0, T_al), 5 * N}, {AF_NET_MAP1, with_live(bwd_args(h, M1, NT_map), h, flow_base), nseg * N},
                                      {AF_NET_MAP2, with_live(bwd_args(h, M2, NT_map), h, flow_base), nseg * N}})) != 0) return rc;
  }
  const double dwf = (double)nseg * N * (h->flop_fwd[AF_NET_MAP1] + h->flop_fwd[AF_NET_MAP2]) + 6.0 * N * h->flop_fwd[AF_NET_ATLAS] + 5.0 * N * h->flop_fwd[AF_NET_ALPHA];
  return finish_step(h, sc, h->adam_m, h->adam_v, h->adam_step, loss_out, (N + 255) / 256, dwf);
}

}

extern "C" {

size_t af_config_size(void) { return sizeof(af_config); }

namespace {
struct Staged {
  void* d = nullptr; bool own = false;
  hipError_t in(const void* p, size_t bytes, bool on_device) {
    if (on_device) { d = const_cast<void*>(p); return hipSuccess; }
    hipError_t e = hipMalloc(&d, std::max<size_t>(bytes, 1)); if (e != hipSuccess) return e;
    own = true;
    return p ? hipMemcpy(d, p, bytes, hipMemcpyHostToDevice) : hipSuccess;
  }
  ~Staged() { if (own) (void)hipFree(d); }
};
int util_fail(const char* what, hipError_t e) { g_create_error = std::string(what) + ": " + hipGetErrorString(e); return AF_EHIP; }
}

int af_resize_bilinear(int device_ordinal, const void* src, int src_u8, int sh, int sw, int ch, float* dst, int dh, int dw,
                       int64_t pix_stride, int64_t ch_stride, int64_t offset, double scale0, double scale1, int on_device) {
  if (!src || !dst || sh <= 0 || sw <= 0 || dh <= 0 || dw <= 0 || ch <= 0 || pix_stride <= 0) { g_create_error = "af_resize_bilinear: arguments"; return AF_EINVAL; }
  hipError_t e = hipSetDevice(device_ordinal); if (e != hipSuccess) return util_fail("hipSetDevice", e);
  if (!on_device && (pix_stride != ch || ch_stride != 1 || offset != 0)) { g_create_error = "af_resize_bilinear: host destinations must be HWC contiguous"; return AF_EINVAL; }
  Staged s, d;
  const size_t sbytes = (size_t)sh * sw * ch * (src_u8 ? 1 : 4), dbytes = (size_t)dh * dw * ch * 4;
  if ((e = s.in(src, sbytes, on_device)) != hipSuccess) return util_fail("stage source", e);
  if ((e = d.in(on_device ? (const void*)dst : nullptr, dbytes, on_device)) != hipSuccess) return util_fail("stage destination", e);
  ResizeArgs a{s.d, src_u8, sh, sw, ch, (float*)d.d, dh, dw, pix_stride, ch_stride, offset, scale0, scale1};
  int r = af_launch_resize(&a, nullptr); if (r) return util_fail("k_resize_bilinear", (hipError_t)r);
  if ((e = hipStreamSynchronize(nullptr)) != hipSuccess) return util_fail("k_resize_bilinear", e);
  if (!on_device && (e = hipMemcpy(dst, d.d, dbytes, hipMemcpyDeviceToHost)) != hipSuccess) return util_fail("copy back", e);
  return AF_OK;
}

static void area_table(int ssize, int dsize, double scale, std::vector<int>& ofs, std::vector<int>& idx, std::vector<float>& w) {
  for (int d = 0; d < dsize; ++d) {
    const double f1 = d * scale, f2 = f1 + scale, cell = std::min(scale, ssize - f1);
    int s1 = (int)std::ceil(f1);
    const int s2 = std::min((int)std::floor(f2), ssize - 1);
    s1 = std::min(s1, s2);
    ofs.push_back((int)idx.size());
    if (s1 - f1 > 1e-3) { idx.push_back(s1 - 1); w.push_back((float)((s1 - f1) / cell)); }
    for (int s = s1; s < s2; ++s) { idx.push_back(s); w.push_back((float)(1.0 / cell)); }
    if (f2 - s2 > 1e-3) { idx.push_back(s2); w.push_back((float)(std::min(std::min(f2 - s2, 1.0), cell) / cell)); }
  }
  ofs.push_back((int)idx.size());
}

int af_resize_area(int device_ordinal, const uint8_t* src, int sh, int sw, int ch, uint8_t* dst, int dh, int dw, int on_device) {
  if (!src || !dst) { g_create_error = "af_resize_area: null pointer"; return AF_EINVAL; }
  if (ch < 1 || ch > 4) { g_create_error = "af_resize_area: ch must be 1..4"; return AF_EINVAL; }
  if (dh < 1) { g_create_error = "af_resize_area: dh < 1"; return AF_EINVAL; }
  if (dw < 1) { g_create_error = "af_resize_area: dw < 1"; return AF_EINVAL; }
  if (dh > sh) { g_create_error = "af_resize_area: dh > sh (INTER_AREA is implemented for shrinking only)"; return AF_EINVAL; }
  if (dw > sw) { g_create_error = "af_resize_area: dw > sw (INTER_AREA is implemented for shrinking only)"; return AF_EINVAL; }
  if (dh == sh && dw == sw) { g_create_error = "af_resize_area: dh == sh && dw == sw (nothing to resize)"; return AF_EINVAL; }
  if ((int64_t)dh * dw > ((int64_t)1 << 38)) { g_create_error = "af_resize_area: image too large"; return AF_EINVAL; }
  hipError_t e = hipSetDevice(device_ordinal); if (e != hipSuccess) return util_fail("hipSetDevice", e);
  AreaArgs a{};
  a.sh = sh; a.sw = sw; a.ch = ch; a.dh = dh; a.dw = dw;
  const double scale_x = 1.0 / ((double)dw / sw), scale_y = 1.0 / ((double)dh / sh);
  const int isx = (int)std::nearbyint(scale_x), isy = (int)std::nearbyint(scale_y);
  const bool fast = std::fabs(scale_x - isx) < DBL_EPSILON && std::fabs(scale_y - isy) < DBL_EPSILON &&
                    (int64_t)isx * dw == sw && (int64_t)isy * dh == sh;
  std::vector<int> tab;
  Staged t;
  if (fast) {
    a.mode = (isx == 2 && isy == 2 && ch != 2) ? AREA_2X2 : AREA_BLOCK;
    a.isx = isx; a.isy = isy; a.inv_area = (float)(1.f / (float)((int64_t)isx * isy));
  } else {
    std::vector<int> xofs, yofs, xidx, yidx; std::vector<float> xa, ya;
    area_table(sw, dw, scale_x, xofs, xidx, xa);
    area_table(sh, dh, scale_y, yofs, yidx, ya);
    for (int v : xidx) if (v < 0 || v >= sw) { g_create_error = "af_resize_area: x table out of range"; return AF_EINVAL; }
    for (int v : yidx) if (v < 0 || v >= sh) { g_create_error = "af_resize_area: y table out of range"; return AF_EINVAL; }
    const size_t o_yofs = xofs.size(), o_xidx = o_yofs + yofs.size(), o_yidx = o_xidx + xidx.size(), o_xa = o_yidx + yidx.size(), o_ya = o_xa + xa.size();
    tab.resize(o_ya + ya.size());
    std::copy(xofs.begin(), xofs.end(), tab.begin()); std::copy(yofs.begin(), yofs.end(), tab.begin() + o_yofs);
    std::copy(xidx.begin(), xidx.end(), tab.begin() + o_xidx); std::copy(yidx.begin(), yidx.end(), tab.begin() + o_yidx);
    if (!xa.empty()) memcpy(tab.data() + o_xa, xa.data(), xa.size() * 4);
    if (!ya.empty()) memcpy(tab.data() + o_ya, ya.data(), ya.size() * 4);
    if ((e = t.in(tab.data(), tab.size() * 4, false)) != hipSuccess) return util_fail("stage tables", e);
    const int* base = (const int*)t.d;
    a.mode = AREA_GENERAL;
    a.xofs = base; a.yofs = base + o_yofs; a.xidx = base + o_xidx; a.yidx = base + o_yidx;
    a.xa = (const float*)(base + o_xa); a.ya = (const float*)(base + o_ya);
  }
  Staged s, d;
  const size_t sbytes = (size_t)sh * sw * ch, dbytes = (size_t)dh * dw * ch;
  if ((e = s.in(src, sbytes, on_device)) != hipSuccess) return util_fail("stage source", e);
  if ((e = d.in(on_device ? (const void*)dst : nullptr, dbytes, on_device)) != hipSuccess) return util_fail("stage destination", e);
  a.src = (const unsigned char*)s.d; a.dst = (unsigned char*)d.d;
  int r = af_launch_resize_area(&a, nullptr); if (r) return util_fail("k_resize_area", (hipError_t)r);
  if ((e = hipStreamSynchronize(nullptr)) != hipSuccess) return util_fail("k_resize_area", e);
  if (!on_device && (e = hipMemcpy(dst, d.d, dbytes, hipMemcpyDeviceToHost)) != hipSuccess) return util_fail("copy back", e);
  return AF_OK;
}

int af_flow_consistency(int device_ordinal, const float* f12, const float* f21, int h, int w, float* out,
                        int64_t pix_stride, int64_t offset, float thresh, int on_device) {
  if (!f12 || !f21 || !out || h <= 0 || w <= 0 || pix_stride <= 0) { g_create_error = "af_flow_consistency: arguments"; return AF_EINVAL; }
  hipError_t e = hipSetDevice(device_ordinal); if (e != hipSuccess) return util_fail("hipSetDevice", e);
  if (!on_device && (pix_stride != 1 || offset != 0)) { g_create_error = "af_flow_consistency: host destinations must be contiguous"; return AF_EINVAL; }
  Staged a12, a21, o;
  const size_t fb = (size_t)h * w * 8, ob = (size_t)h * w * 4;
  if ((e = a12.in(f12, fb, on_device)) != hipSuccess || (e = a21.in(f21, fb, on_device)) != hipSuccess) return util_fail("stage flows", e);
  if ((e = o.in(on_device ? (const void*)out : nullptr, ob, on_device)) != hipSuccess) return util_fail("stage output", e);
  ConsistencyArgs a{(const float*)a12.d, (const float*)a21.d, h, w, (float*)o.d, pix_stride, offset, thresh};
  int r = af_launch_consistency(&a, nullptr); if (r) return util_fail("k_flow_consistency", (hipError_t)r);
  if ((e = hipStreamSynchronize(nullptr)) != hipSuccess) return util_fail("k_flow_consistency", e);
  if (!on_device && (e = hipMemcpy(out, o.d, ob, hipMemcpyDeviceToHost)) != hipSuccess) return util_fail("copy back", e);
  return AF_OK;
}

static double warp_error_of(const double* part, int nblk, int npix) {
  double sse = 0.0, cnt = 0.0;
  for (int b = 0; b < nblk; ++b) { sse += part[2 * b]; cnt += part[2 * b + 1]; }
  return sse / (3.0 * (cnt > 0.0 ? cnt : (double)npix));
}

int af_warp_error_pair(int device_ordinal, const float* img1, const float* img2, const float* flow12, const float* flow21, int h, int w,
                       int align_corners, double* err, float* noc, float* warped, int on_device) {
  if (!img1 || !img2 || !flow12 || !flow21 || !err || h < 2 || w < 2 || (align_corners != 0 && align_corners != 1)) {
    g_create_error = "af_warp_error_pair: arguments"; return AF_EINVAL;
  }
  if ((int64_t)h * w > INT32_MAX / 4) { g_create_error = "af_warp_error_pair: image too large"; return AF_EINVAL; }
  hipError_t e = hipSetDevice(device_ordinal); if (e != hipSuccess) return util_fail("hipSetDevice", e);
  const int npix = h * w, nblk = (npix + 255) / 256;
  const size_t ib = (size_t)npix * 12, fb = (size_t)npix * 8;
  Staged s1, s2, s12, s21, sn, sw, sp;
  if ((e = s1.in(img1, ib, on_device)) != hipSuccess || (e = s2.in(img2, ib, on_device)) != hipSuccess ||
      (e = s12.in(flow12, fb, on_device)) != hipSuccess || (e = s21.in(flow21, fb, on_device)) != hipSuccess) return util_fail("stage inputs", e);
  if (noc && (e = sn.in(on_device ? (const void*)noc : nullptr, (size_t)npix * 4, on_device)) != hipSuccess) return util_fail("stage noc", e);
  if (warped && (e = sw.in(on_device ? (const void*)warped : nullptr, ib, on_device)) != hipSuccess) return util_fail("stage warped", e);
  if ((e = sp.in(nullptr, (size_t)nblk * 16, false)) != hipSuccess) return util_fail("block partials", e);
  WarpErrArgs a{(const float*)s1.d, (const float*)s2.d, (const float*)s12.d, (const float*)s21.d, 0, 0, h, w, align_corners,
                noc ? (float*)sn.d : nullptr, warped ? (float*)sw.d : nullptr, (double*)sp.d};
  int r = af_launch_warp_error(&a, 2, 1, nullptr); if (r) return util_fail("k_warp_error", (hipError_t)r);
  std::vector<double> part((size_t)nblk * 2);
  if ((e = hipMemcpy(part.data(), sp.d, (size_t)nblk * 16, hipMemcpyDeviceToHost)) != hipSuccess) return util_fail("k_warp_error", e);
  if (!on_device && noc && (e = hipMemcpy(noc, sn.d, (size_t)npix * 4, hipMemcpyDeviceToHost)) != hipSuccess) return util_fail("copy back", e);
  if (!on_device && warped && (e = hipMemcpy(warped, sw.d, ib, hipMemcpyDeviceToHost)) != hipSuccess) return util_fail("copy back", e);
  *err = warp_error_of(part.data(), nblk, npix);
  return AF_OK;
}

const char* af_last_error(const af_handle* h) { return h ? h->err.c_str() : g_create_error.c_str(); }

void af_set_thread_error(const char* m) { g_create_error = m; }

int af_create(const af_config* cfg, int device_ordinal, af_handle** out) {
  if (!cfg || !out) { g_create_error = "af_create: null argument"; return AF_EINVAL; }
  *out = nullptr;
  auto bad = [&](const char* m) { g_create_error = std::string("af_create: ") + m; return (int)AF_EINVAL; };
  if (cfg->resx <= 1 || cfg->resy <= 1 || cfg->number_of_frames <= 0) return bad("resx/resy/number_of_frames");
  if (cfg->samples_batch <= 0) return bad("samples_batch");
  auto width_ok = [](int w) { return w >= 1 && w <= AF_HID; };
  if (!width_ok(cfg->number_of_channels_mapping1) || !width_ok(cfg->number_of_channels_atlas)) return bad("number_of_channels_mapping1 / number_of_channels_atlas must be 1..256 (config_flow_100.json:19,24)");
  auto layers_ok = [](int n) { return n >= 2 && n <= AF_MAX_LAYERS; };
  if (!layers_ok(cfg->number_of_layers_mapping1) || !layers_ok(cfg->number_of_layers_atlas)) return bad("number_of_layers_mapping1 / number_of_layers_atlas must be 2..8");
  if (cfg->positional_encoding_num_atlas < 1 || cfg->positional_encoding_num_atlas > 10) return bad("positional_encoding_num_atlas must be 1..10");
  auto pe_ok = [](int k) { return k >= 1 && k <= 5; };
  if (cfg->use_positional_encoding_mapping1 && !pe_ok(cfg->number_of_positional_encoding_mapping1)) return bad("number_of_positional_encoding_mapping1 must be 1..5 when use_positional_encoding_mapping1 is set");
  if (cfg->derivative_amount <= 0 || cfg->global_rigidity_derivative_amount_fg <= 0) return bad("derivative amounts");
  const bool seg = cfg->two_layer != 0;
  if (seg) {
    if (!width_ok(cfg->number_of_channels_mapping2) || !width_ok(cfg->number_of_channels_alpha)) return bad("number_of_channels_mapping2 / number_of_channels_alpha must be 1..256 (config_flow_100.json:21,26)");
    if (!layers_ok(cfg->number_of_layers_mapping2) || !layers_ok(cfg->number_of_layers_alpha)) return bad("number_of_layers_mapping2 / number_of_layers_alpha must be 2..8");
    if (cfg->positional_encoding_num_alpha < 1 || cfg->positional_encoding_num_alpha > 5) return bad("positional_encoding_num_alpha must be 1..5");
    if (cfg->use_positional_encoding_mapping2 && !pe_ok(cfg->number_of_positional_encoding_mapping2)) return bad("number_of_positional_encoding_mapping2 must be 1..5 when use_positional_encoding_mapping2 is set");
    if (cfg->global_rigidity_derivative_amount_bg <= 0) return bad("global_rigidity_derivative_amount_bg");
  }
  hipError_t e = hipSetDevice(device_ordinal);
  if (e != hipSuccess) { g_create_error = std::string("af_create: hipSetDevice: ") + hipGetErrorString(e); return AF_EHIP; }
  af_handle* h = new af_handle();
  h->cfg = *cfg; h->device = device_ordinal; h->seg = seg;
  if (h->cfg.pretrain_batch <= 0) h->cfg.pretrain_batch = 10000;
  if (h->cfg.lr <= 0) h->cfg.lr = 1e-4f;
  auto die = [&](int code) { g_create_error = h->err; af_destroy(h); return code; };
#define CCHK(x) do { hipError_t e_ = (x); if (e_ != hipSuccess) { h->fail(AF_EHIP, #x, e_); return die(e_ == hipErrorOutOfMemory ? AF_ENOMEM : AF_EHIP); } } while (0)
  hipDeviceProp_t prop; CCHK(hipGetDeviceProperties(&prop, device_ordinal));
  h->ncu = prop.multiProcessorCount > 0 ? prop.multiProcessorCount : 256;
  CCHK(hipStreamCreateWithFlags(&h->stream, hipStreamNonBlocking));
  CCHK((hipError_t)af_mlp_init()); CCHK((hipError_t)af_mlp16_init()); CCHK((hipError_t)af_dw_init()); CCHK((hipError_t)af_mlp_bf_init()); CCHK((hipError_t)af_mlp_hf_init());

  const int nl_atlas = cfg->number_of_layers_atlas;
  const unsigned atlas_skip = (nl_atlas > 4 ? (1u << 4) : 0u) | (nl_atlas > 7 ? (1u << 7) : 0u);
  if (cfg->use_positional_encoding_mapping1) describe_net(h->nets[AF_NET_MAP1], AF_NET_MAP1, cfg->number_of_layers_mapping1, AF_IN_PE3, cfg->number_of_positional_encoding_mapping1, 2, 0u, false, cfg->number_of_channels_mapping1);
  else describe_net(h->nets[AF_NET_MAP1], AF_NET_MAP1, cfg->number_of_layers_mapping1, AF_IN_XYT, 0, 2, 0u, false, cfg->number_of_channels_mapping1);
  describe_net(h->nets[AF_NET_ATLAS], AF_NET_ATLAS, nl_atlas, AF_IN_PE2, cfg->positional_encoding_num_atlas, 3, atlas_skip, true, cfg->number_of_channels_atlas);
  if (seg) {
    if (cfg->use_positional_encoding_mapping2) describe_net(h->nets[AF_NET_MAP2], AF_NET_MAP2, cfg->number_of_layers_mapping2, AF_IN_PE3, cfg->number_of_positional_encoding_mapping2, 2, 0u, false, cfg->number_of_channels_mapping2);
    else describe_net(h->nets[AF_NET_MAP2], AF_NET_MAP2, cfg->number_of_layers_mapping2, AF_IN_XYT, 0, 2, 0u, false, cfg->number_of_channels_mapping2);
    describe_net(h->nets[AF_NET_ALPHA], AF_NET_ALPHA, cfg->number_of_layers_alpha, AF_IN_PE3, cfg->positional_encoding_num_alpha, 1, 0u, false, cfg->number_of_channels_alpha);
  }
  for (NetDesc& n : h->nets) if (n.used) {
    auto lw = [&](int w) { return w == AF_HID ? n.hid : (w > AF_HID ? w - AF_HID + n.hid : w); };
    double f = 0, d = n.dx0 ? (double)n.in_feat0 * n.hid : 0.0;
    for (int l = 0; l < n.NL; ++l) {
      const double lin = l == 0 ? n.in_feat0 : lw(n.in_feat[l]), lout = l == n.NL - 1 ? n.out : n.hid;
      f += lin * lout; if (l >= 1) d += (double)n.hid * lout;
    }
    h->flop_fwd[n.id] = 2.0 * f; h->flop_dx[n.id] = 2.0 * d;
  }
  size_t fc = 0, bc = 0, biasc = 0, pc = 0;
  for (NetDesc& n : h->nets) if (n.used) {
    n.p_base = pc; pc += n.nparams; plan_images(n, fc, bc, biasc);
    if (!check_chunk_plan(n)) { h->fail(AF_EINVAL, "weight-image plan does not match the kernels' chunk sequence"); return die(AF_EINVAL); }
    if (!plan_stream(n, n.bf, k_bf16x6, h->sf_bytes, h->sb_bytes)) { h->fail(AF_EINVAL, "bf16 stream plan does not match the kernels' chunk sizes"); return die(AF_EINVAL); }
    if (!plan_stream(n, n.hf, k_f16x3, h->hf_bytes, h->hb_bytes)) { h->fail(AF_EINVAL, "fp16 stream plan does not match the kernels' chunk sizes"); return die(AF_EINVAL); }
  }
  h->sf_bytes += 49152 + 65536; h->sb_bytes += 49152 + 65536;
  if (h->sf_bytes >= ((size_t)1 << 31) || h->sb_bytes >= ((size_t)1 << 31)) { h->fail(AF_EINVAL, "stream images exceed 2 GB"); return die(AF_EINVAL); }
  CCHK(hipMalloc((void**)&h->img_sf, h->sf_bytes)); CCHK(hipMalloc((void**)&h->img_sb, h->sb_bytes));
  CCHK(hipMemset(h->img_sf, 0, h->sf_bytes)); CCHK(hipMemset(h->img_sb, 0, h->sb_bytes));
  h->hf_bytes += 2 * 65536; h->hb_bytes += 2 * 65536;
  if (h->hf_bytes >= ((size_t)1 << 31) || h->hb_bytes >= ((size_t)1 << 31)) { h->fail(AF_EINVAL, "stream images exceed 2 GB"); return die(AF_EINVAL); }
  CCHK(hipMalloc((void**)&h->img_hf, h->hf_bytes)); CCHK(hipMalloc((void**)&h->img_hb, h->hb_bytes));
  CCHK(hipMemset(h->img_hf, 0, h->hf_bytes)); CCHK(hipMemset(h->img_hb, 0, h->hb_bytes));
  fc += AF_CHUNK_MAX / 4; bc += AF_CHUNK_MAX / 4;
  h->total_params = pc; h->img_f_floats = fc; h->img_b_floats = bc; h->bias_floats = biasc;
  CCHK(dalloc(&h->params, pc)); CCHK(dalloc(&h->adam_m, pc)); CCHK(dalloc(&h->adam_v, pc));
  CCHK(dalloc(&h->pre_m, pc)); CCHK(dalloc(&h->pre_v, pc)); CCHK(dalloc(&h->grads, pc));
  CCHK(dalloc(&h->img_f, fc)); CCHK(dalloc(&h->img_b, bc)); CCHK(dalloc(&h->bias_img, biasc));
  CCHK(hipMemset(h->params, 0, pc * 4)); CCHK(hipMemset(h->adam_m, 0, pc * 4)); CCHK(hipMemset(h->adam_v, 0, pc * 4));
  CCHK(hipMemset(h->pre_m, 0, pc * 4)); CCHK(hipMemset(h->pre_v, 0, pc * 4)); CCHK(hipMemset(h->grads, 0, pc * 4));
  CCHK(hipMemset(h->img_f, 0, fc * 4)); CCHK(hipMemset(h->img_b, 0, bc * 4)); CCHK(hipMemset(h->bias_img, 0, biasc * 4));
  h->N = cfg->samples_batch;
  const int N = h->N, rows_pre = h->cfg.pretrain_batch;
  NetDesc& M = h->nets[AF_NET_MAP1]; NetDesc& A = h->nets[AF_NET_ATLAS]; NetDesc& M2 = h->nets[AF_NET_MAP2]; NetDesc& AL = h->nets[AF_NET_ALPHA];
  CCHK(alloc_net_buffers(M, std::max(9 * N, rows_pre), true));
  CCHK(alloc_net_buffers(A, (seg ? 6 : 3) * N, false));
  if (seg) {
    CCHK(alloc_net_buffers(M2, std::max(9 * N, rows_pre), true));
    CCHK(alloc_net_buffers(AL, 5 * N, true));
  }
  CCHK(dalloc(&h->samples, (size_t)N * AF_REC_F));
  h->loss_nblk_cap = (std::max(N, rows_pre) + 255) / 256;
  CCHK(dalloc(&h->loss_part, (size_t)h->loss_nblk_cap * AF_LOSS_W)); CCHK(hipMemset(h->loss_part, 0, (size_t)h->loss_nblk_cap * AF_LOSS_W * 4));
  CCHK(dalloc(&h->counts, 2)); CCHK(hipMemset(h->counts, 0, 8));
  CCHK(dalloc(&h->nan_flag, 1)); CCHK(hipMemset(h->nan_flag, 0, 4));
  CCHK(dalloc(&h->flow_rank, (size_t)2 * N)); CCHK(hipMemset(h->flow_rank, 0xff, (size_t)2 * N * 4));
  CCHK(dalloc(&h->scan, (size_t)(N + 255) / 256 + 1)); CCHK(hipMemset(h->scan, 0, (size_t)((N + 255) / 256 + 1) * 8));
  CCHK(dalloc(&h->live, 1)); CCHK(hipMemset(h->live, 0, 4));
  CCHK(dalloc(&h->nvalid, 128));
  bool ok = build_main_scheds(h);
  ok = ok && build_sched(h, h->sched[2], {{&M, tiles_of(rows_pre)}});
  if (seg) ok = ok && build_sched(h, h->sched[3], {{&M2, tiles_of(rows_pre)}});
  if (!ok) { h->fail(AF_EINVAL, "dW schedule needs more than DW_MAXSEG segments per workgroup"); return die(AF_EINVAL); }
  size_t pf = 0;
  for (int i = 0; i < (seg ? 4 : 3); ++i) { CCHK(upload_sched(h->sched[i])); pf = std::max(pf, h->sched[i].partial_floats); }
  CCHK(dalloc(&h->partial, pf)); h->partial_cap = pf;
  h->frame_sse.assign(cfg->number_of_frames, 0.0); h->frame_sse_valid.assign(cfg->number_of_frames, 0);
  if (repack(h, h->sched[0]) != 0) return die(AF_EHIP);
  CCHK(hipStreamSynchronize(h->stream));
#undef CCHK
  *out = h;
  return AF_OK;
}

void af_destroy(af_handle* h) {
  if (!h) return;
  (void)hipSetDevice(h->device);
  if (h->stream) (void)hipStreamSynchronize(h->stream);
  drain_timers(h);
  for (NetDesc& n : h->nets) if (n.used) free_net(n);
  for (Sched& s : h->sched) { (void)hipFree(s.d_jobs); (void)hipFree(s.d_ajobs); (void)hipFree(s.d_segs); }
  (void)hipFree(h->params); (void)hipFree(h->adam_m); (void)hipFree(h->adam_v); (void)hipFree(h->pre_m); (void)hipFree(h->pre_v); (void)hipFree(h->grads);
  (void)hipFree(h->img_f); (void)hipFree(h->img_b); (void)hipFree(h->bias_img); (void)hipFree(h->table); (void)hipFree(h->img_sf); (void)hipFree(h->img_sb); (void)hipFree(h->img_hf); (void)hipFree(h->img_hb);
  (void)hipFree(h->samples); (void)hipFree(h->loss_part); (void)hipFree(h->loss_log); (void)hipFree(h->counts); (void)hipFree(h->nan_flag); (void)hipFree(h->flow_rank); (void)hipFree(h->scan); (void)hipFree(h->live); (void)hipFree(h->nvalid);
  (void)hipFree(h->partial); (void)hipFree(h->dw_clock); (void)hipFree(h->step_stamp); (void)hipFree(h->r_coords); (void)hipFree(h->r_uv); (void)hipFree(h->r_uv2); (void)hipFree(h->r_al);
  (void)hipFree(h->r_t); (void)hipFree(h->r_rgb); (void)hipFree(h->r_sse); (void)hipFree(h->r_u8); (void)hipFree(h->r_at); (void)hipFree(h->l_buf);
  if (h->stream) (void)hipStreamDestroy(h->stream);
  delete h;
}

int af_sync(af_handle* h) {
  if (!h) return AF_EINVAL;
  HCHK(hipSetDevice(h->device)); HCHK(hipStreamSynchronize(h->stream));
  return AF_OK;
}

int af_upload_video(af_handle* h, const float* frames, const float* flow_fwd, const float* flow_bwd,
                    const float* mask_fwd, const float* mask_bwd, const float* mask_fg, int on_device) {
  if (!h) return AF_EINVAL;
  if (!frames || !flow_fwd || !flow_bwd || !mask_fwd || !mask_bwd) return h->fail(AF_EINVAL, "af_upload_video: null tensor");
  if (h->seg && !mask_fg) return h->fail(AF_EINVAL, "af_upload_video: a two_layer handle needs mask_fg (mask_frames, unwrap_utils.py:68-70)");
  HCHK(hipSetDevice(h->device));
  const size_t P2 = (size_t)h->cfg.resx * h->cfg.resy, F = h->cfg.number_of_frames, P = P2 * F;
  if (!h->table) { hipError_t e = dalloc(&h->table, P * AF_REC_F); if (e != hipSuccess) return h->fail(AF_ENOMEM, "record table", e); }
  const float* src[6] = {frames, flow_fwd, flow_bwd, mask_fwd, mask_bwd, mask_fg};
  const size_t cnt[6] = {P * 3, P * 2, P * 2, P, P, P};
  float* tmp[6] = {nullptr, nullptr, nullptr, nullptr, nullptr, nullptr};
  const float* dev[6];
// ... 72 lines not shown
  std::fill(h->frame_sse_valid.begin(), h->frame_sse_valid.end(), 0);
  return AF_OK;
}

int af_get_params(af_handle* h, int net, float* flat, size_t n) {
  int rc = check_net(h, net, n); if (rc) return rc;
  if (!flat) return h->fail(AF_EINVAL, "af_get_params: null");
  HCHK(hipSetDevice(h->device)); HCHK(hipStreamSynchronize(h->stream));
  return get_flat(h, h->nets[net], h->params, flat);
}

int af_get_adam_state(af_handle* h, int net, float* m, float* v, int64_t* step) {
  if (!h) return AF_EINVAL;
  if (net < 0 || net >= AF_MAX_NETS || !h->nets[net].used) return h->fail(AF_EINVAL, "unknown net");
  HCHK(hipSetDevice(h->device)); HCHK(hipStreamSynchronize(h->stream));
  const NetDesc& n = h->nets[net];
  int rc = AF_OK;
  if (m && (rc = get_flat(h, n, h->adam_m, m)) != AF_OK) return rc;
  if (v && (rc = get_flat(h, n, h->adam_v, v)) != AF_OK) return rc;
  if (step) *step = h->adam_step;
  return AF_OK;
}

int af_set_adam_state(af_handle* h, int net, const float* m, const float* v, int64_t step) {
  if (!h) return AF_EINVAL;
  if (net < 0 || net >= AF_MAX_NETS || !h->nets[net].used) return h->fail(AF_EINVAL, "unknown net");
  if (step < 0) return h->fail(AF_EINVAL, "negative step");
  HCHK(hipSetDevice(h->device)); HCHK(hipStreamSynchronize(h->stream));
  const NetDesc& n = h->nets[net];
  int rc = AF_OK;
  if (m && (rc = put_flat(h, n, h->adam_m, m)) != AF_OK) return rc;
  if (v && (rc = put_flat(h, n, h->adam_v, v)) != AF_OK) return rc;
  h->adam_step = step;
  return AF_OK;
}

static int rebuild_dw_scheds(af_handle* h) {
  HCHK(hipSetDevice(h->device)); HCHK(hipStreamSynchronize(h->stream));
  bool ok = build_main_scheds(h);
  ok = ok && build_sched(h, h->sched[2], {{&h->nets[AF_NET_MAP1], tiles_of(h->cfg.pretrain_batch)}});
  if (h->seg) ok = ok && build_sched(h, h->sched[3], {{&h->nets[AF_NET_MAP2], tiles_of(h->cfg.pretrain_batch)}});
  if (!ok) return h->fail(AF_EINVAL, "dW schedule needs more than DW_MAXSEG segments per workgroup");
  for (int i = 0; i < (h->seg ? 4 : 3); ++i) {
    HCHK(upload_sched(h->sched[i]));
    if (h->sched[i].partial_floats > h->partial_cap) {
      (void)hipFree(h->partial); h->partial = nullptr; h->partial_cap = 0;
      HCHK(dalloc(&h->partial, h->sched[i].partial_floats)); h->partial_cap = h->sched[i].partial_floats;
    }
  }
  return AF_OK;
}
int af_set_dw_mode(af_handle* h, int mode) {
  if (!h) return AF_EINVAL;
  if (mode < 0 || mode > 2) return h->fail(AF_EINVAL, "af_set_dw_mode: 0 (fp32 MFMA), 1 (bf16x6) or 2 (bf16x3)");
  if (mode == h->dw_mode) return AF_OK;
  h->dw_mode = mode;
  return rebuild_dw_scheds(h);
}
int af_debug_set_dw_cost(af_handle* h, const double* cost5, double seg_cost) {
  if (!h) return AF_EINVAL;
  if (!cost5) { if (!h->dw_cost_set) return AF_OK; h->dw_cost_set = false; h->dw_seg_cost = 0; return rebuild_dw_scheds(h); }
  for (int i = 0; i < 5; ++i)
    if (!(cost5[i] > 0.0) || !std::isfinite(cost5[i])) return h->fail(AF_EINVAL, "af_debug_set_dw_cost: every tile cost must be finite and > 0");
  if (std::isnan(seg_cost) || std::isinf(seg_cost)) return h->fail(AF_EINVAL, "af_debug_set_dw_cost: seg_cost must be finite (<= 0 keeps the shipped one)");
  const double r = *std::max_element(cost5, cost5 + 5) / *std::min_element(cost5, cost5 + 5);
  if (r > 1.0e3) return h->fail(AF_EINVAL, "af_debug_set_dw_cost: cost ratios beyond 1000:1 cut segments the DW_MAXSEG lists cannot hold");
  double keep[5]; const bool was = h->dw_cost_set; const double keep_seg = h->dw_seg_cost;
  for (int i = 0; i < 5; ++i) { keep[i] = h->dw_cost[i]; h->dw_cost[i] = cost5[i]; }
  h->dw_cost_set = true; h->dw_seg_cost = seg_cost > 0 ? seg_cost : 0;
  const int rc = rebuild_dw_scheds(h);
  if (rc != AF_OK) {
    const std::string msg = h->err;
    for (int i = 0; i < 5; ++i) h->dw_cost[i] = keep[i];
    h->dw_cost_set = was; h->dw_seg_cost = keep_seg;
    (void)rebuild_dw_scheds(h);
    h->err = msg;
  }
  return rc;
}
int af_set_mlp_mode(af_handle* h, int mode) {
  if (!h) return AF_EINVAL;
  if (mode < 0 || mode > 3) return h->fail(AF_EINVAL, "af_set_mlp_mode: 0 (fp32 MFMA), 1 (bf16x6), 2 (bf16x6 forward, three-product bf16 backward chain) or 3 (f16x3: two-term fp16 split with a scale per row)");
  const int cls_old = chain_family(h->mlp_mode).cls, cls_new = chain_family(mode).cls;
  h->mlp_mode = mode;
  if (cls_new != cls_old && cls_new != 0) {
    HCHK(hipSetDevice(h->device));
    const int rc = repack(h, h->sched[0]); if (rc) return rc;
    HCHK(hipStreamSynchronize(h->stream));
  }
  return AF_OK;
}
int af_get_modes(const af_handle* h, int* mlp_mode, int* dw_mode) {
  if (!h) return AF_EINVAL;
  if (mlp_mode) *mlp_mode = h->mlp_mode;
  if (dw_mode) *dw_mode = h->dw_mode;
  return AF_OK;
}
int af_set_debug(af_handle* h, int enable) { if (!h) return AF_EINVAL; h->debug = enable != 0; return AF_OK; }
int af_set_timing(af_handle* h, int class_mask) {
  if (!h) return AF_EINVAL;
  h->timing = (unsigned)class_mask & 0xFFFFu;
  const unsigned every = ((unsigned)class_mask >> 16) & 0xFFu;
  h->timing_every = every ? every : 1;
  return AF_OK;
}
int af_get_timing(af_handle* h, double* ms16, int64_t* counts16, double* flops16, int reset) {
  if (!h) return AF_EINVAL;
  (void)hipSetDevice(h->device); (void)hipStreamSynchronize(h->stream); drain_timers(h);
  for (int i = 0; i < 16; ++i) {
    if (ms16) ms16[i] = h->t_ms[i];
    if (counts16) counts16[i] = h->t_cnt[i];
    if (flops16) flops16[i] = h->t_flops[i];
    if (reset) { h->t_ms[i] = 0; h->t_cnt[i] = 0; h->t_flops[i] = 0; }
  }
  return AF_OK;
}

int af_get_last_grads(af_handle* h, int net, float* flat, size_t n) {
  int rc = check_net(h, net, n); if (rc) return rc;
  HCHK(hipSetDevice(h->device)); HCHK(hipStreamSynchronize(h->stream));
  return get_flat(h, h->nets[net], h->grads, flat);
}

int af_loss_width(const af_handle* h) { return h && h->seg ? 16 : 8; }

int af_pretrain(af_handle* h, int net, int pretrain_iters, const int64_t* ys, const int64_t* xs, uint64_t seed, float* losses_out) {
  if (!h) return AF_EINVAL;
  if (!(net == AF_MAPPING1 || (net == AF_MAPPING2 && h->seg))) return h->fail(AF_EINVAL, "af_pretrain: net must be a mapping net of this handle");
  if (pretrain_iters < 0 || ((ys == nullptr) != (xs == nullptr))) return h->fail(AF_EINVAL, "af_pretrain: arguments");
  HCHK(hipSetDevice(h->device));
  const int F = h->cfg.number_of_frames, NB = h->cfg.pretrain_batch;
  const size_t steps = (size_t)pretrain_iters * F;
  if (steps == 0) return AF_OK;
  NetDesc& M = h->nets[net];
  Sched& sc = h->sched[net == AF_MAPPING1 ? 2 : 3];
  int rc = ensure_loss_log(h, steps); if (rc) return rc;
  int64_t *d_ys = nullptr, *d_xs = nullptr;
  if (ys) {
    HCHK(dalloc(&d_ys, steps * NB)); HCHK(dalloc(&d_xs, steps * NB));
    HCHK(hipMemcpy(d_ys, ys, steps * NB * 8, hipMemcpyHostToDevice));
    HCHK(hipMemcpy(d_xs, xs, steps * NB * 8, hipMemcpyHostToDevice));
  }
  const int NT = tiles_of(NB);
  HCHK(hipMemsetAsync(M.dout, 0, (size_t)M.nt_cap * 32 * 16, h->stream));
  HCHK(hipMemsetAsync(h->pre_m, 0, h->total_params * 4, h->stream));
  HCHK(hipMemsetAsync(h->pre_v, 0, h->total_params * 4, h->stream));
  h->cur_nseg = 0;
  const float half_main = (float)(std::max(h->cfg.resx, h->cfg.resy) / 2.0);
  size_t s = 0;
  for (int it = 0; it < pretrain_iters && rc == 0; ++it)
    for (int f = 0; f < F && rc == 0; ++f, ++s) {
      PrePrepArgs p{};
      p.ys = d_ys ? d_ys + s * NB : nullptr; p.xs = d_xs ? d_xs + s * NB : nullptr;
      p.seed = seed; p.iter = (uint32_t)s; p.N = NB; p.resx = h->cfg.resx; p.resy = h->cfg.resy;
      p.half_main = half_main; p.t = (float)((double)f / (F / 2.0) - 1.0);
      p.coords = M.coords; p.x0_tile = M.x0_tile;
      if (af_launch_pre_prep(&p, h->stream)) { rc = h->fail(AF_EHIP, "pre_prep"); break; }
      const bool hf = h->mlp_mode == 3;
      if (hf) { if ((rc = launch_fwd(h, T_FWD_1, {{net, fwd_args(h, M, M.coords, M.out_buf, NT, true), NB}}, true)) != 0) break; }
      else { Timer t(h, T_FWD_1, (double)NB * h->flop_fwd[net]); const FwdArgs fa = fp32_images(fwd_args(h, M, M.coords, M.out_buf, NT, true), h, M);
        if (af_launch_fwd16(M.kern, &fa, h->stream)) { rc = h->fail(AF_EHIP, "fwd16"); break; } }
      PreLossArgs l{M.coords, M.out_buf, M.dout, h->loss_part, NB, h->cfg.uv_mapping_scale};
      if (af_launch_pre_loss(&l, h->stream)) { rc = h->fail(AF_EHIP, "pre_loss"); break; }
      if (hf) { if ((rc = launch_bwd(h, T_BWD_2, {{net, bwd_args(h, M, NT), NB}})) != 0) break; }
      else { Timer t(h, T_BWD_2, (double)NB * h->flop_dx[net]); const BwdArgs ba = fp32_images(bwd_args(h, M, NT), h, M);
        if (af_launch_bwd16(M.kern, &ba, h->stream)) { rc = h->fail(AF_EHIP, "bwd16"); break; } }
      rc = finish_step(h, sc, h->pre_m, h->pre_v, (long long)s + 1, h->loss_log + s * AF_LOSS_W, (NB + 255) / 256, (double)NB * h->flop_fwd[net], false);
    }
  hipError_t e = hipStreamSynchronize(h->stream);
  drain_timers(h);
  if (d_ys) { (void)hipFree(d_ys); (void)hipFree(d_xs); }
  if (rc) return rc;
  if (e != hipSuccess) return h->fail(AF_EHIP, "af_pretrain sync", e);
  { int dev_nan = 0; int r2 = take_nan_flag(h, dev_nan); if (r2) return r2; if (dev_nan & 1) return h->fail(AF_ENAN, "af_pretrain: NaN loss or non-finite parameter");
    if ((dev_nan & 2) && h->mlp_mode == 3) return h->fail(AF_ERANGE, "af_pretrain: a hidden-layer weight reached |w| >= 8, beyond what the fp16 weight images of af_set_mlp_mode(h, 3) are scaled for; use mode 1 (bf16x6)"); }
  if (losses_out) {
    std::vector<float> tmp(steps * AF_LOSS_W);
    HCHK(hipMemcpy(tmp.data(), h->loss_log, steps * AF_LOSS_W * 4, hipMemcpyDeviceToHost));
    for (size_t i = 0; i < steps; ++i) losses_out[i] = tmp[i * AF_LOSS_W] / (float)NB;
  }
  std::fill(h->frame_sse_valid.begin(), h->frame_sse_valid.end(), 0);
  return AF_OK;
}

int af_train_steps(af_handle* h, int first_iter, int n_iters, const int64_t* inds, uint64_t seed, float* losses_out) {
  if (!h) return AF_EINVAL;
  if (!h->have_video) return h->fail(AF_ESTATE, "af_train_steps: no video uploaded");
  if (n_iters < 0 || first_iter < 0) return h->fail(AF_EINVAL, "af_train_steps: arguments");
  if (n_iters == 0) return AF_OK;
  HCHK(hipSetDevice(h->device));
  const af_config& c = h->cfg;
  const int N = h->N;
  int rc = ensure_loss_log(h, n_iters); if (rc) return rc;
  int64_t* d_inds = nullptr;
  if (inds) {
    HCHK(dalloc(&d_inds, (size_t)n_iters * N));
    HCHK(hipMemcpy(d_inds, inds, (size_t)n_iters * N * 8, hipMemcpyHostToDevice));
  }
  HCHK(hipMemsetAsync(h->counts, 0, 8, h->stream));
  for (int k = 0; k < n_iters && rc == 0; ++k) {
    const int64_t* di = d_inds ? d_inds + (size_t)k * N : nullptr;
    float* lo = h->loss_log + (size_t)k * AF_LOSS_W;
    h->timing_live = (k % (int)h->timing_every) == 0;
    rc = h->seg ? enqueue_seg_step(h, first_iter + k, di, seed, lo) : enqueue_single_step(h, first_iter + k, di, seed, lo);
  }
  h->timing_live = true;
  hipError_t e = hipStreamSynchronize(h->stream);
  drain_timers(h);
  if (d_inds) (void)hipFree(d_inds);
  if (rc) return rc;
  if (e != hipSuccess) return h->fail(AF_EHIP, "af_train_steps sync", e);
  std::fill(h->frame_sse_valid.begin(), h->frame_sse_valid.end(), 0);
  int dev_nan = 0;
  if ((rc = take_nan_flag(h, dev_nan)) != 0) return rc;
  if (losses_out) {
    std::vector<float> tmp((size_t)n_iters * AF_LOSS_W);
    HCHK(hipMemcpy(tmp.data(), h->loss_log, (size_t)n_iters * AF_LOSS_W * 4, hipMemcpyDeviceToHost));
    bool nan = false;
    const float invN = 1.f / (float)N;
    for (int k = 0; k < n_iters; ++k) {
      const int i = first_iter + k;
      const bool glob = glob_on(c, i);
      const float* s = &tmp[(size_t)k * AF_LOSS_W];
      const float nf = s[AF_LOSS_W - 2], nb = s[AF_LOSS_W - 1];
      float total;
      if (!h->seg) {
        float* o = losses_out + (size_t)k * 8;
        o[0] = s[0] * invN; o[1] = c.use_gradient_loss ? s[1] * invN : 0.f; o[2] = s[2] * invN; o[3] = glob ? s[3] * invN : 0.f;
        o[4] = 0.5f * (s[5] / nb) + 0.5f * (s[4] / nf);
        o[5] = c.rigidity_coeff * o[2] + (glob ? c.global_rigidity_coeff_fg * o[3] : 0.f) + c.rgb_coeff * o[0] + c.optical_flow_coeff * o[4] + c.gradient_loss_coeff * o[1];
        o[6] = nf; o[7] = nb;
        total = o[5];
      } else {
        float* o = losses_out + (size_t)k * 16;
        const float boot = i > c.stop_bootstrapping_iteration ? 0.f : c.alpha_bootstrapping_factor;
        o[0] = s[0] * invN; o[1] = c.use_gradient_loss ? s[1] * invN : 0.f; o[2] = s[2] * invN; o[3] = s[3] * invN;
        o[4] = glob ? s[4] * invN : 0.f; o[5] = glob ? s[5] * invN : 0.f;
        o[6] = 0.5f * (s[7] / nb) + 0.5f * (s[6] / nf);
        o[7] = 0.5f * (s[9] / nb) + 0.5f * (s[8] / nf);
        o[8] = (s[10] / nf + s[11] / nb) * 0.5f;
        o[9] = s[12] * invN; o[10] = s[13] * invN;
        o[11] = c.rigidity_coeff * (o[2] + o[3]) + c.rgb_coeff * o[0] + c.optical_flow_coeff * (o[6] + o[7]) + boot * o[9]
              + c.alpha_flow_factor * o[8] + c.sparsity_coeff * o[10] + c.gradient_loss_coeff * o[1]
              + (glob ? c.global_rigidity_coeff_fg * o[4] + c.global_rigidity_coeff_bg * o[5] : 0.f);
        o[12] = nf; o[13] = nb; o[14] = 0.f; o[15] = 0.f;
        total = o[11];
      }
      if (!(total == total)) nan = true;
    }
    if (nan) return h->fail(AF_ENAN, "af_train_steps: NaN loss (a batch without valid flow pixels, as in the reference, or divergence)");
  }
  if (dev_nan & 1) return h->fail(AF_ENAN, "af_train_steps: NaN loss or non-finite parameter (a batch without valid flow pixels, as in the reference, or divergence)");
  if ((dev_nan & 2) && h->mlp_mode == 3) return h->fail(AF_ERANGE, "af_train_steps: a hidden-layer weight reached |w| >= 8, beyond what the fp16 weight images of af_set_mlp_mode(h, 3) are scaled for; use mode 1 (bf16x6)");
  return AF_OK;
}

int af_step_work(const af_handle* h, int iter, int64_t rows4[4], double* flops) {
  if (!h) return AF_EINVAL;
  const int64_t nseg = glob_on(h->cfg, iter) ? 9 : 7, N = h->N;
  int64_t r[4] = {nseg * N, (h->seg ? 6 : 3) * N, h->seg ? nseg * N : 0, h->seg ? 5 * N : 0};
  double f = 0;
  for (int i = 0; i < 4; ++i) { if (rows4) rows4[i] = r[i]; f += (double)r[i] * (2.0 * h->flop_fwd[i] + h->flop_dx[i]); }
  if (flops) *flops = f;
  return AF_OK;
}

static int ensure_render(af_handle* h, int rows) {
  if (rows <= h->render_rows_cap) return 0;
  (void)hipFree(h->r_coords); (void)hipFree(h->r_uv); (void)hipFree(h->r_uv2); (void)hipFree(h->r_al); (void)hipFree(h->r_t); (void)hipFree(h->r_rgb); (void)hipFree(h->r_sse);
  h->r_coords = h->r_uv = h->r_uv2 = h->r_al = h->r_t = h->r_rgb = nullptr; h->r_sse = nullptr; h->render_rows_cap = 0;
  const size_t rp = (size_t)tiles_of(rows) * 32;
  HCHK(dalloc(&h->r_coords, rp * 4)); HCHK(dalloc(&h->r_uv, rp * 4)); HCHK(dalloc(&h->r_t, rp * 4 * (h->seg ? 2 : 1)));
  if (h->seg) { HCHK(dalloc(&h->r_uv2, rp * 4)); HCHK(dalloc(&h->r_al, rp * 4)); }
  HCHK(dalloc(&h->r_rgb, rp * 3)); HCHK(dalloc(&h->r_sse, (rp + 255) / 256));
  h->render_rows_cap = rows;
  return 0;
}

int af_debug_plan(int ncu, int rows_map, int rows_atlas, int dep_rows, int out3[3]) {
  if (!out3 || ncu <= 0) return AF_EINVAL;
  const int NT_map = tiles_of(rows_map), NT_atlas = tiles_of(rows_atlas);
  plan_mapping_split(ncu, NT_map, NT_atlas, dep_rows, out3[0], out3[1]);
  out3[2] = NT_map;
  return AF_OK;
}

int af_debug_dw_clocks(af_handle* h, int enable, uint64_t* out, int cap_wg) {
  if (!h) return AF_EINVAL;
  HCHK(hipSetDevice(h->device)); HCHK(hipStreamSynchronize(h->stream));
  if (enable && !h->dw_clock) { HCHK(dalloc(&h->dw_clock, (size_t)h->ncu * 2)); HCHK(hipMemset(h->dw_clock, 0, (size_t)h->ncu * 16)); }
  if (out && h->dw_clock) HCHK(hipMemcpy(out, h->dw_clock, (size_t)std::min(cap_wg, h->ncu) * 16, hipMemcpyDeviceToHost));
  if (!enable && h->dw_clock) { (void)hipFree(h->dw_clock); h->dw_clock = nullptr; }
  return h->ncu;
}

int af_debug_step_clocks(af_handle* h, int enable, uint64_t* out, int cap_wg) {
  if (!h) return AF_EINVAL;
  HCHK(hipSetDevice(h->device)); HCHK(hipStreamSynchronize(h->stream));
  const size_t n = (size_t)5 * AF_STAMP_WG * 4;
  if (enable && !h->step_stamp) { HCHK(dalloc(&h->step_stamp, n)); HCHK(hipMemset(h->step_stamp, 0, n * 8)); }
  if (out && h->step_stamp) {
    const int w = std::min(cap_wg, AF_STAMP_WG);
    for (int l = 0; l < 5; ++l) HCHK(hipMemcpy(out + (size_t)l * w * 4, h->step_stamp + (size_t)l * AF_STAMP_WG * 4, (size_t)w * 32, hipMemcpyDeviceToHost));
  }
  if (h->step_stamp) HCHK(hipMemset(h->step_stamp, 0, n * 8));
  if (!enable && h->step_stamp) { (void)hipFree(h->step_stamp); h->step_stamp = nullptr; }
  return AF_STAMP_WG;
}

int af_debug_dw_schedule(af_handle* h, int which, int32_t* out, int cap_wg) {
  if (!h || which < 0 || which > 3) return AF_EINVAL;
  const Sched& sc = h->sched[which];
  int live = 0;
  if (out) { (void)hipSetDevice(h->device); (void)hipStreamSynchronize(h->stream); (void)hipMemcpy(&live, h->live, 4, hipMemcpyDeviceToHost); }
  if (out) {
    for (int w = 0; w < std::min(cap_wg, sc.nwg); ++w)
      for (int k = 0; k < DW_MAXSEG; ++k) {
        const DwSeg& sg = sc.segs[(size_t)w * DW_MAXSEG + k];
        int32_t* o = out + ((size_t)w * DW_MAXSEG + k) * 4;
        o[0] = sg.job < 0 ? -1 : sc.jobs[sg.job].shape; o[1] = sg.t0; o[2] = sg.t1; o[3] = sg.job;
        if (sg.job >= 0 && sc.jobs[sg.job].live_rows) o[2] = std::max(sg.t0, std::min(sg.t1, tiles_of(sc.jobs[sg.job].live_base + live)));
      }
  }
  return sc.nwg;
}

int af_debug_records(af_handle* h, const int64_t* inds, int n, float* out) {
  if (!h || !inds || !out || n <= 0) return AF_EINVAL;
  if (!h->have_video) return h->fail(AF_ESTATE, "af_debug_records: no video uploaded");
  HCHK(hipSetDevice(h->device)); HCHK(hipStreamSynchronize(h->stream));
  const int64_t P = (int64_t)h->cfg.resx * h->cfg.resy * h->cfg.number_of_frames;
  for (int i = 0; i < n; ++i) {
    if (inds[i] < 0 || inds[i] >= P) return h->fail(AF_EINVAL, "af_debug_records: index out of range");
    HCHK(hipMemcpy(out + (size_t)i * AF_REC_F, h->table + (size_t)inds[i] * AF_REC_F, AF_REC_F * 4, hipMemcpyDeviceToHost));
  }
  return AF_OK;
}

int af_debug_forward(af_handle* h, int net, const float* in, int rows, float* out) {
  if (!h || !in || !out || rows <= 0) return AF_EINVAL;
  if (net < 0 || net >= AF_MAX_NETS || !h->nets[net].used) return h->fail(AF_EINVAL, "unknown net");
  HCHK(hipSetDevice(h->device));
  int rc = ensure_render(h, rows); if (rc) return rc;
  const int NT = tiles_of(rows);
  HCHK(hipMemsetAsync(h->r_coords, 0, (size_t)NT * 32 * 16, h->stream));
  HCHK(hipMemcpyAsync(h->r_coords, in, (size_t)rows * 16, hipMemcpyHostToDevice, h->stream));
  FwdArgs fa = fwd_args(h, h->nets[net], h->r_coords, h->r_uv, NT, false);
  if (h->nets[net].in_kind != AF_IN_XYT) { fa.in_scale = 1.f; fa.in_shift0 = 0.f; fa.in_shift1 = 0.f; }
  { int rc2 = launch_fwd(h, T_FWD_1, {{net, fa, rows}}, false); if (rc2) return rc2; }
  HCHK(hipMemcpyAsync(out, h->r_uv, (size_t)rows * 16, hipMemcpyDeviceToHost, h->stream));
  HCHK(hipStreamSynchronize(h->stream));
  return AF_OK;
}

int af_debug_tiles(af_handle* h, int net, int which, int layer, int nt_stride, int tile0, int ntiles, float* out) {
  if (!h || !out || ntiles <= 0 || tile0 < 0 || layer < 0 || nt_stride <= 0) return AF_EINVAL;
  if (net < 0 || net >= AF_MAX_NETS || !h->nets[net].used) return h->fail(AF_EINVAL, "unknown net");
  const NetDesc& n = h->nets[net];
  if (tile0 + ntiles > nt_stride || nt_stride > n.nt_cap) return h->fail(AF_EINVAL, "af_debug_tiles: tile range");
  const float* src = nullptr; size_t per = 0; bool planes = false;
  switch (which) {
    case 0: src = n.acts; per = AF_TILE_F; planes = true; break;
    case 1: src = n.dz; per = AF_TILE_F; planes = true; break;
    case 2: src = (const float*)n.masks; per = 64 * 4; planes = true; break;
    case 3: src = n.pe_tile; per = 2048; break;
    case 4: src = n.dz_last; per = 1024; break;
    case 5: src = n.x0_tile; per = 1024; break;
    default: return h->fail(AF_EINVAL, "af_debug_tiles: which");
  }
// ... 363 lines not shown
```

### all-in-one-deflicker_amd/csrc/mlphf.hip

```cpp
#include "mlp_common.h"

typedef _Float16 f16x8 __attribute__((ext_vector_type(8)));

#define AF_SLOT_HF 65536
#define AF_BIAS_LDS_HF (2 * AF_SLOT_HF)
#define AF_LDS_BYTES_HF (2 * AF_SLOT_HF + AF_MAX_LAYERS * AF_HID * 4)
#define AF_HF_WSHIFT 12
#define AF_HF_KEEP 8

#ifdef AF_HF_CLK
__device__ unsigned long long* g_hf_clk;
#define HF_MARK(i) do { if (g_hf_clk && threadIdx.x == 0) g_hf_clk[(size_t)blockIdx.x * 32 + (i)] = __builtin_amdgcn_s_memtime(); } while (0)
#else
#define HF_MARK(i) do { } while (0)
#endif

template <class NS> using ChunkBytesHf = ChunkBytes16<NS, AF_SLOT_HF>;

struct HfStream {
  static constexpr int NI = AF_SLOT_HF / 4096;
  const char* src; char* smem; int wave, stg; char* p_dst; int p_it;
  AF_DEV void begin_stage() { p_dst = smem + (stg & 1) * AF_SLOT_HF + wave * 1024; p_it = 0; }
  AF_DEV void issue1() {
    const int k = p_it < NI ? p_it : NI - 1;
// ... 196 lines not shown
#pragma unroll
        for (int p = 0; p < 4; ++p) {
          const int r = q * 4 + p;
          float z = acc[T][r];
          if constexpr (SCALED) z = __builtin_fmaf(z, inv, bq[p]);
          in[T * 16 + r] = z;
        }
        hf_max3(mx, in[T * 16 + q * 4], in[T * 16 + q * 4 + 1]);
        hf_max3(mx, in[T * 16 + q * 4 + 2], in[T * 16 + q * 4 + 3]);
        bq = bnx;
      }
      __builtin_amdgcn_sched_barrier(0);
    }
    if constexpr (TRAIN) ts.r = af_rsrc_uniform(a.acts + ((size_t)l * a.nt_stride + tile) * AF_TILE_F, live ? AF_TILE_F * 4 : 0);
    hf_row_scale(mx, sc, inv);
  };
  auto store_masks = [&](int l) {
    if constexpr (TRAIN) {
      if (live) {
        u32x4 m4 = {fin.mk[0], fin.mk[1], fin.mk[2], fin.mk[3]};
        *(u32x4*)(a.masks + (((size_t)l * a.nt_stride + tile) * 64 + lane) * 4) = m4;
      }
#pragma unroll
      for (int i = 0; i < 4; ++i) fin.mk[i] = 0u;
    }
  };
  auto hook_dma = [&](auto gi) { if constexpr (decltype(gi)::value < 6) { cs.issue1(); cs.issue1(); } };
  auto hook_none = [&](auto) {};

  HF_MARK(1);
  const char* cur = cs.publish(CB::L0);
  cs.issue_bytes(nl > 2 ? CB::HID : CB::last_bytes(nl));
  HF_MARK(2);
  init_bias(acc, bias_lds, 0, h);
  mm_block<8, NS::K0G, 0, 4>(acc, pe, cur + a_off8, hook_none);
  HF_MARK(3);
  pre_out(0, std::false_type{});
  HF_MARK(4);
  const char* lane_base = cs.publish(nl > 2 ? CB::HID : CB::last_bytes(nl)) + lane_off;
  cs.lead5();
  HF_MARK(5);

  if constexpr (HID) {
  int l = 1;
#pragma unroll 1
  do {
    hf_enter<FIN>(pp, in, sc, lane_base, fin);
    const bool skip = NS::SKIP != 0 && ((NS::SKIP >> l) & 1);
    const int behind = l == nl - 2 ? CB::last_bytes(nl) : CB::HID;
    hf_block<(TRAIN && !(AF_ABL & 1)), FIN>(acc, in, sc, pp, lane_base, cs, lane_off, skip ? CB::SKIP : behind, ts, fin);
    store_masks(l - 1);
    if constexpr (NS::SKIP != 0) {
      if (skip) {
        const float up = sc * (float)(1 << AF_HF_WSHIFT);
#pragma unroll
        for (int i = 0; i < NPE; ++i) pe[i] *= up;
        mm_block<8, NS::PEG, 0, 4>(acc, pe, lane_base - lane_off + a_off8, hook_dma);
#pragma unroll
        for (int i = 0; i < NPE; ++i) pe[i] *= inv;
        lane_base = cs.publish(behind) + lane_off;
        cs.lead5();
      }
    }
    HF_MARK(4 + 2 * l);
    pre_out(l, std::true_type{});
    HF_MARK(5 + 2 * l);
  } while (++l <= nl - 2);
  }
  lane_base -= lane_off;
  hf_finish_range<FIN, 0>(in, fin, std::make_integer_sequence<int, 128>{});
  store_masks(nl - 2);
  AF_ELEMWISE_FENCE();

  chain_out_layer<NS, TRAIN>(a, nl, lane_base, bias_lds + (nl - 1) * AF_HID * 4, in, pe, ts, row, lane, h, live);
  HF_MARK(30);
}

template <int... Ps> AF_DEV float hf_absmax(const float (&in)[128], std::integer_sequence<int, Ps...>) {
  float mx = 0.f;
  (hf_max3_abs(mx, in[2 * Ps], in[2 * Ps + 1]), ...);
  return mx;
}

template <class NS>
AF_DEV void mlp_bwd_body_hf(const BwdArgs& a, int wg, char* smem) {
  ChainRows cr;
  if (!chain_rows(a, wg, cr)) return;
  const int tid = cr.tid, wave = cr.wave, lane = cr.lane, j = cr.j, h = cr.h, tile = cr.tile, row = cr.row; const bool live = cr.live;

  using CB = ChunkBytesHf<NS>;
  HfStream cs; cs.smem = smem;
  cs.start(a.wimg, tid, wave);
  cs.issue_bytes(CB::BLAST);
  const int nl = a.nl;

  float dzl[4];
  chain_seed<NS>(a, dzl, row, tile, j, h, live);

  const int a_off8 = (h * 256 + j) * 16;
  const int lane_off = (h * 32 + j) * 16;
  const int voff_t = (4 * h * 32 + j) * 4;
  f32x16 acc[8];
  float in[128];
  TileStore ts{af_rsrc(a.dz, 0), voff_t};
  HfPipe pp;
  float sc = 1.f, inv = 1.f;

  HfFin fin; fin.invp = 1.f;
  auto pre_mask = [&](int l, auto scaled) {
    const u32x4 m4 = *(const u32x4*)(a.masks + (((size_t)(l - 1) * a.nt_stride + tile) * 64 + lane) * 4);
    fin.mk[0] = m4[0]; fin.mk[1] = m4[1]; fin.mk[2] = m4[2]; fin.mk[3] = m4[3];
    fin.invp = decltype(scaled)::value ? inv : 1.f;
#pragma unroll
    for (int T = 0; T < 8; ++T)
#pragma unroll
      for (int r = 0; r < 16; ++r) in[T * 16 + r] = acc[T][r];
    const float mx = hf_absmax(in, std::make_integer_sequence<int, 64>{});
    ts.r = af_rsrc_uniform(a.dz + ((size_t)(l - 1) * a.nt_stride + tile) * AF_TILE_F, live ? AF_TILE_F * 4 : 0);
    hf_row_scale(mx * fin.invp, sc, inv);
  };
  auto hook_dma = [&](auto gi) { if constexpr (decltype(gi)::value < 6) { cs.issue1(); cs.issue1(); } };
  auto hook_dma_store = [&](auto gi) { if constexpr (decltype(gi)::value < 6) { cs.issue1(); cs.issue1(); } ts.template part<decltype(gi)::value>(in); };
  auto hook_none = [&](auto) {};

  HF_MARK(1);
  const char* cur = cs.publish(CB::BLAST);
  cs.issue_bytes(nl > 2 ? CB::HID : (NS::DX0 ? CB::BL0C : 4096));
  HF_MARK(2);
  mm_block<8, 1, 0, NS::OUT, true>(acc, dzl, cur + a_off8, hook_none);
  HF_MARK(3);
  pre_mask(nl - 1, std::false_type{});
  HF_MARK(4);
  const char* lane_base = cs.publish(nl > 2 ? CB::HID : (NS::DX0 ? CB::BL0C : 4096)) + lane_off;
  cs.lead5();
  HF_MARK(5);

#pragma unroll 1
  for (int l = nl - 2; l >= 1; --l) {
    hf_enter<3>(pp, in, sc, lane_base, fin);
    hf_block<!(AF_ABL & 1), 3>(acc, in, sc, pp, lane_base, cs, lane_off, l > 1 ? CB::HID : (NS::DX0 ? CB::BL0C : 4096), ts, fin);
    HF_MARK(4 + 2 * (nl - 1 - l));
    pre_mask(l, std::true_type{});
    HF_MARK(5 + 2 * (nl - 1 - l));
  }
  lane_base -= lane_off;
  hf_finish_range<3, 0>(in, fin, std::make_integer_sequence<int, 128>{});
  AF_ELEMWISE_FENCE();

  if constexpr (NS::DX0) {
    f32x16 acc2[2];
    mm_block<2, 16, 0, 4, true>(acc2, in, lane_base + (h * 64 + j) * 16, hook_dma_store);
    const char* half2 = cs.publish(CB::BL0C);
    mm_block<2, 16, 64, 4>(acc2, in, half2 + (h * 64 + j) * 16, hook_dma);
    chain_dpe_to_uv<NS>(a, acc2, row, tile, j, h, live);
  } else {
    ts.all(in);
  }
  HF_MARK(30);
}

struct HfChains {
  template <class NS, bool TRAIN, bool HID> static AF_DEV void fwd(const FwdArgs& a, int wg, char* smem) { mlp_fwd_body_hf<NS, TRAIN, HID>(a, wg, smem); }
  template <class NS> static AF_DEV void bwd(const BwdArgs& a, int wg, char* smem) { mlp_bwd_body_hf<NS>(a, wg, smem); }
};

template <bool TRAIN>
__global__ __launch_bounds__(256, 1) void k_mlp_fwd_multi_hf(MultiFwd m) {
  extern __shared__ __attribute__((aligned(16))) char smem[];
  AF_STAMP(m, 0);
  HF_MARK(0);
  chains_fwd_multi<HfChains, TRAIN>(m, smem);
  AF_STAMP(m, 1);
}

__global__ __launch_bounds__(256, 1) void k_mlp_bwd_multi_hf(MultiBwd m) {
  extern __shared__ __attribute__((aligned(16))) char smem[];
  AF_STAMP(m, 0);
  HF_MARK(0);
  chains_bwd_multi<HfChains>(m, smem);
  AF_STAMP(m, 1);
}

extern "C" int af_launch_fwd_multi_hf(MultiFwd* m, int train, hipStream_t s) {
  const int tot = multi_grid(*m);
  if (tot <= 0) return 0;
  if (train) hipLaunchKernelGGL((k_mlp_fwd_multi_hf<true>), dim3(tot), dim3(256), AF_LDS_BYTES_HF, s, *m);
  else       hipLaunchKernelGGL((k_mlp_fwd_multi_hf<false>), dim3(tot), dim3(256), AF_LDS_BYTES_HF, s, *m);
  return (int)hipGetLastError();
}
extern "C" int af_launch_bwd_multi_hf(MultiBwd* m, hipStream_t s) {
  const int tot = multi_grid(*m);
  if (tot <= 0) return 0;
  hipLaunchKernelGGL(k_mlp_bwd_multi_hf, dim3(tot), dim3(256), AF_LDS_BYTES_HF, s, *m);
  return (int)hipGetLastError();
}
extern "C" int af_mlp_chunk_bytes_hf(int net, int which, int nl) { return chunk_bytes<ChunkBytesHf>(net, which, nl); }
extern "C" int af_mlp_hf_init() { return lds_opt_in(AF_LDS_BYTES_HF, k_mlp_fwd_multi_hf<true>, k_mlp_fwd_multi_hf<false>, k_mlp_bwd_multi_hf); }
```

### include/atlasfit.h

```cpp
#ifndef ATLASFIT_H
#define ATLASFIT_H
#include <stddef.h>
#include <stdint.h>
#ifdef __cplusplus
extern "C" {
#endif

typedef struct af_handle af_handle;

enum af_status { AF_OK = 0, AF_EINVAL = -1, AF_EHIP = -2, AF_ENOMEM = -3, AF_ENAN = -4, AF_ESTATE = -5,
                 AF_ERANGE = -6    };
enum af_net { AF_MAPPING1 = 0, AF_ATLAS = 1, AF_MAPPING2 = 2, AF_ALPHA = 3 };

typedef struct af_config {
  int32_t resx, resy, number_of_frames;
  int32_t samples_batch;
  int32_t number_of_channels_mapping1, number_of_layers_mapping1;
  int32_t number_of_channels_atlas, number_of_layers_atlas;
  int32_t positional_encoding_num_atlas;
  int32_t use_positional_encoding_mapping1;
  int32_t derivative_amount;
  int32_t include_global_rigidity_loss;
  int32_t global_rigidity_derivative_amount_fg;
  int32_t stop_global_rigidity;
// ... 16 lines not shown
  int32_t number_of_positional_encoding_mapping2;
  int32_t reserved[2];
} af_config;

int af_create(const af_config* cfg, int device_ordinal, af_handle** out);
size_t af_config_size(void);
void af_destroy(af_handle* h);
const char* af_last_error(const af_handle* h);

int af_upload_video(af_handle* h, const float* frames, const float* flow_fwd, const float* flow_bwd,
                    const float* mask_fwd, const float* mask_bwd, const float* mask_fg, int on_device);

int af_resize_bilinear(int device_ordinal, const void* src, int src_u8, int sh, int sw, int ch, float* dst, int dh, int dw,
                       int64_t pix_stride, int64_t ch_stride, int64_t offset, double scale0, double scale1, int on_device);
int af_resize_area(int device_ordinal, const uint8_t* src, int sh, int sw, int ch, uint8_t* dst, int dh, int dw, int on_device);
int af_flow_consistency(int device_ordinal, const float* f12, const float* f21, int h, int w, float* out,
                        int64_t pix_stride, int64_t offset, float thresh, int on_device);

size_t af_param_count(const af_handle* h, int net);
int af_set_params(af_handle* h, int net, const float* flat, size_t n);
int af_get_params(af_handle* h, int net, float* flat, size_t n);
int af_get_adam_state(af_handle* h, int net, float* exp_avg, float* exp_avg_sq, int64_t* step);
int af_set_adam_state(af_handle* h, int net, const float* exp_avg, const float* exp_avg_sq, int64_t step);

int af_pretrain(af_handle* h, int net, int pretrain_iters, const int64_t* ys, const int64_t* xs,
                uint64_t seed, float* losses_out);

int af_train_steps(af_handle* h, int first_iter, int n_iters, const int64_t* inds, uint64_t seed,
                   float* losses_out);
int af_loss_width(const af_handle* h);

int af_render_frame(af_handle* h, int frame, float* rgb_out, double* sse_out);
int af_render_frame_u8(af_handle* h, int frame, float* rgb_out, uint8_t* u8_out, int on_device, double* sse_out);
int af_render_frame_at(af_handle* h, int frame, int oh, int ow, float* rgb_out, uint8_t* u8_out, const uint8_t* ref_u8, double* sse_out,
                       int on_device);
int af_psnr(af_handle* h, double* mean_psnr, double* per_frame);

int af_render_layers(af_handle* h, int frame, float* uv1, float* uv2, float* alpha, float* rgb1, float* rgb2);
int af_mapping_area(af_handle* h, int which, float out5[5]);
int af_render_atlas_texture(af_handle* h, int res, float minx, float miny, float edge, float* out);
int af_render_edit(af_handle* h, int frame, int res, const float* tex_fg, const float win_fg[3], const float* tex_bg, const float win_bg[3],
                   float* edit, float* edit_fg, float* edit_bg, float* use_fg, float* use_bg);

int af_render_loss_maps(af_handle* h, int frame, float* rigidity1, float* rigidity2, float* flow1, float* flow2,
                        float* flow_alpha, float* rgb_err, float* residual);

int af_warp_error_pair(int device_ordinal, const float* img1, const float* img2, const float* flow12, const float* flow21, int h, int w,
                       int align_corners, double* err, float* noc, float* warped, int on_device);
int af_warp_error(af_handle* h, int which, int align_corners, double* per_pair, double* mean);

int af_sync(af_handle* h);

typedef struct af_filter af_filter;
int af_filter_create(int device_ordinal, int h, int w, af_filter** out);
void af_filter_destroy(af_filter* f);
size_t af_filter_param_count(const af_filter* f, int net);
int af_filter_set_params(af_filter* f, int net, const float* flat, size_t n);
int af_filter_reset(af_filter* f);
int af_filter_frame(af_filter* f, const float* content, const float* style, float* pred_out, float* final_out, int on_device);
int af_filter_debug_activation(af_filter* f, const char* name, float* out, size_t n);
int af_conv2d(int device_ordinal, const float* x, int h, int w, int cin, const float* weight, const float* bias, int cout, int k, int stride,
              int pad_mode, int act, const float* residual, float* y, int on_device);

typedef struct af_raft af_raft;
int af_raft_create(int device_ordinal, int h, int w, int capacity, af_raft** out);
void af_raft_destroy(af_raft* r);
size_t af_raft_param_count(const af_raft* r);
int af_raft_info(const af_raft* r, int* hp, int* wp, int* slots);
int af_raft_set_params(af_raft* r, const float* flat, size_t n);
int af_raft_encode(af_raft* r, int slot, const float* image, int on_device);
int af_raft_flow(af_raft* r, int n, const int* slot_a, const int* slot_b, int iters, float* flow_up, float* flow_lo, int on_device);
int af_raft_step(af_raft* r, int slot_a, int slot_b, const float* net, const float* coords1, float* net_out, float* delta_out);
int af_raft_lookup(af_raft* r, int slot_a, int slot_b, const float* coords, float* out);
int af_raft_debug_activation(af_raft* r, const char* name, float* out, size_t n);
int af_raft_conv2d(int device_ordinal, const float* x, int batch, int h, int w, int cin, const float* weight, const float* bias, int cout, int kh, int kw,
                   int stride, int act, float* y);
int af_raft_gru(int device_ordinal, int batch, int h, int w, int vertical, const float* net, const float* x, const float* wz, const float* bz, const float* wr,
                const float* br, const float* wq, const float* bq, float* net_out);
int af_raft_instance_norm(int device_ordinal, const float* x, int h, int w, int c, int relu, const float* residual, float* y);

int af_debug_forward(af_handle* h, int net, const float* in, int rows, float* out);
int af_debug_tiles(af_handle* h, int net, int which, int layer, int nt_stride, int tile0, int ntiles, float* out);
int af_debug_plan(int ncu, int rows_map, int rows_atlas, int dep_rows, int out3[3]);
int af_debug_dw_clocks(af_handle* h, int enable, uint64_t* out, int cap_wg);
int af_debug_step_clocks(af_handle* h, int enable, uint64_t* out, int cap_wg);
int af_debug_dw_schedule(af_handle* h, int which, int32_t* out, int cap_wg);
int af_debug_records(af_handle* h, const int64_t* inds, int n, float* out);
int af_set_dw_mode(af_handle* h, int mode);
int af_debug_set_dw_cost(af_handle* h, const double* cost5, double seg_cost);
int af_set_mlp_mode(af_handle* h, int mode);
int af_get_modes(const af_handle* h, int* mlp_mode, int* dw_mode);
int af_set_debug(af_handle* h, int enable);
int af_get_last_grads(af_handle* h, int net, float* flat, size_t n);
int af_set_timing(af_handle* h, int class_mask);
int af_get_timing(af_handle* h, double* ms16, int64_t* counts16, double* flops16, int reset);
int af_step_work(const af_handle* h, int iter, int64_t rows4[4], double* flops);

#ifdef __cplusplus
}
#endif
#endif
```

Before: 11.55 million.

## Fuse last-layer weight gradient into f16x3 backward chain kernel

In mlp_mode 3, the last layer's weight and bias gradients are computed inside the backward chain kernel. Each workgroup runs fp32 4x4 MFMAs over the saved activations and dz_last, then writes a per-workgroup partial block. That layer's job is dropped from the separate dW schedule, and the Adam kernel sums the chain partials across slots. This removes a dW job and its re-reading of activations, at the cost of extra work and registers in the backward kernel and an alignment constraint on part boundaries.

```diff
diff --git a/all-in-one-deflicker_amd/atlasfit.py b/all-in-one-deflicker_amd/atlasfit.py
--- a/all-in-one-deflicker_amd/atlasfit.py
+++ b/all-in-one-deflicker_amd/atlasfit.py
@@ -14,6 +14,7 @@
     "af_get_params", "af_get_adam_state", "af_set_adam_state", "af_pretrain", "af_train_steps",
     "af_render_frame", "af_render_frame_u8", "af_render_frame_at", "af_psnr", "af_sync", "af_debug_forward", "af_set_debug", "af_get_last_grads",
     "af_set_timing", "af_get_timing", "af_step_work", "af_loss_width", "af_config_size", "af_debug_records", "af_debug_plan",
+    "af_debug_plan_sched", "af_debug_chain_slots",
     "af_resize_bilinear", "af_resize_area", "af_flow_consistency", "af_debug_dw_clocks", "af_debug_step_clocks", "af_set_dw_mode", "af_set_mlp_mode", "af_debug_dw_schedule",
     "af_debug_set_dw_cost", "af_debug_tiles", "af_get_modes",
     "af_render_layers", "af_mapping_area", "af_render_atlas_texture", "af_render_edit", "af_render_loss_maps",
@@ -168,6 +169,8 @@
         "af_config_size": (sz, []),
         "af_debug_records": (i32, [vp, vp, i32, vp]),
         "af_debug_plan": (i32, [i32, i32, i32, i32, C.POINTER(i32 * 3)]),
+        "af_debug_plan_sched": (i32, [C.POINTER(AfConfig), i32, i32, i32, vp, i32, vp]),
+        "af_debug_chain_slots": (i32, [i32, i32, C.POINTER(C.c_int32 * 2)]),
         "af_resize_bilinear": (i32, [i32, vp, i32, i32, i32, i32, vp, i32, i32, i64, i64, i64, C.c_double, C.c_double, i32]),
         "af_resize_area": (i32, [i32, vp, i32, i32, i32, vp, i32, i32, i32]),
         "af_flow_consistency": (i32, [i32, vp, vp, i32, i32, vp, i64, i64, C.c_float, i32]),
diff --git a/all-in-one-deflicker_amd/csrc/af_dev.h b/all-in-one-deflicker_amd/csrc/af_dev.h
--- a/all-in-one-deflicker_amd/csrc/af_dev.h
+++ b/all-in-one-deflicker_amd/csrc/af_dev.h
@@ -39,6 +39,11 @@
   int nl;
 };
 
+#if defined(__HIPCC__)
+__host__ __device__
+#endif
+inline int af_chain_slot(int tile0, int wg) { return (tile0 >> 2) + wg; }
+
 struct BwdArgs {
   const float* wimg;
   const float* out;
@@ -56,6 +61,8 @@
   int nt_stride;
   const int* live_rows; int live_base;
   int nl;
+  const float* acts;
+  float* chain_part; int chain_blk;
 };
 
 #define AF_STAMP_WG 4096
diff --git a/all-in-one-deflicker_amd/csrc/elem.h b/all-in-one-deflicker_amd/csrc/elem.h
--- a/all-in-one-deflicker_amd/csrc/elem.h
+++ b/all-in-one-deflicker_amd/csrc/elem.h
@@ -123,6 +123,7 @@
   int32_t  sf_off; uint32_t sf_kind, sf_mpad, sf_k0;
   int32_t  sb_off; uint32_t sb_kind, sb_mpad;
   int32_t  hf_off, hb_off;
+  const float* chain_src; uint32_t chain_bias;
 };
 struct AdamHyper { float step_size, bc2_sqrt, one_minus_b1, beta2, one_minus_b2, eps; };
 struct AdamBufs { float* params; float* m; float* v; float* img_f; float* img_b; float* bias_img; char* sf; char* sb; char* hf; char* hb; };
diff --git a/all-in-one-deflicker_amd/csrc/elem.hip b/all-in-one-deflicker_amd/csrc/elem.hip
--- a/all-in-one-deflicker_amd/csrc/elem.hip
+++ b/all-in-one-deflicker_amd/csrc/elem.hip
@@ -610,21 +610,62 @@
   }
 }
 
+#define AF_ADAM_CHAIN_E 16
+template <bool UPDATE>
+AF_DEV bool adam_chain_grad(const AdamJob& j, uint32_t& o, uint32_t& i, bool& is_bias, float& g) {
+  __shared__ float red[16][AF_ADAM_CHAIN_E];
+  const uint32_t grp = threadIdx.x >> 4, pos = blockIdx.x * AF_ADAM_CHAIN_E + (threadIdx.x & 15);
+  const uint32_t first = (j.col0 >> 2) * 16, nw = ((j.in_real + 3) >> 2) * 16;
+  bool valid; uint32_t idx;
+  if (pos < nw) {
+    is_bias = false; o = (pos >> 2) & 3; i = (pos >> 4) * 4 + (pos & 3);
+    valid = o < j.out_real && i < j.in_real; idx = first + pos;
+  } else {
+    is_bias = true; o = pos - nw; i = 0;
+    valid = j.b_off >= 0 && o < j.out_real; idx = j.chain_bias + o;
+  }
+  if (!UPDATE) return valid && grp == 0;
+  float t = 0.f;
+  if (valid) {
+    const float* pp = j.chain_src + idx;
+    uint32_t s = grp;
+    for (; s + 7 * 16 < j.nslots; s += 8 * 16) {
+      float v[8];
+#pragma unroll
+      for (int q = 0; q < 8; ++q) v[q] = pp[(size_t)(s + 16 * q) * j.part_blk];
+#pragma unroll
+      for (int q = 0; q < 8; ++q) t += v[q];
+    }
+    for (; s < j.nslots; s += 16) t += pp[(size_t)s * j.part_blk];
+  }
+  red[grp][threadIdx.x & 15] = t;
+  __syncthreads();
+  if (grp != 0 || !valid) return false;
+  g = 0.f;
+#pragma unroll
+  for (int q = 0; q < 16; ++q) g += red[q][threadIdx.x];
+  return true;
+}
+
 template <bool UPDATE>
 __global__ __launch_bounds__(256) void k_adam(AdamArgs a) {
   const AdamJob j = a.jobs[blockIdx.y];
   const uint32_t e = blockIdx.x * blockDim.x + threadIdx.x;
   const uint32_t nw = j.out_real * j.in_real;
   const uint32_t nb = j.b_off >= 0 ? j.out_real : 0u;
-  if (e < nw + nb) {
-    const bool is_bias = e >= nw;
-    const uint32_t o = is_bias ? e - nw : e / j.in_real;
-    const uint32_t i = is_bias ? 0u : e - o * j.in_real;
+  bool is_bias = e >= nw, mine = e < nw + nb;
+  uint32_t o = is_bias ? e - nw : e / j.in_real;
+  uint32_t i = is_bias ? 0u : e - o * j.in_real;
+  float g = 0.f;
+  if (j.chain_src) {
+    mine = blockIdx.x * AF_ADAM_CHAIN_E < ((j.in_real + 3) >> 2) * 16 + 4 && adam_chain_grad<UPDATE>(j, o, i, is_bias, g);
+  }
+  if (mine) {
     const uint32_t pidx = is_bias ? (uint32_t)j.b_off + o : j.p_off + o * j.p_ld + i;
     float p = a.bufs.params[pidx];
     if (UPDATE) {
+      if (!j.chain_src) {
       const float* pp = a.partial + j.part_off + (is_bias ? j.out_real_pad * j.pld + o : o * j.pld + i);
-      float g = 0.f;
       uint32_t s = 0;
       for (; s + 8 <= j.nslots; s += 8) {
         float t[8];
@@ -646,6 +687,7 @@
         g += t0; g += t1; s += 2;
       }
       if (s < j.nslots) g += pp[(size_t)s * j.part_blk];
+      }
       float m = a.bufs.m[pidx], v = a.bufs.v[pidx];
       m = m + (g - m) * a.hy.one_minus_b1;
       v = v * a.hy.beta2 + (a.hy.one_minus_b2 * g) * g;
diff --git a/all-in-one-deflicker_amd/csrc/host.hip b/all-in-one-deflicker_amd/csrc/host.hip
--- a/all-in-one-deflicker_amd/csrc/host.hip
+++ b/all-in-one-deflicker_amd/csrc/host.hip
@@ -84,10 +84,13 @@
   float *coords = nullptr, *x0_tile = nullptr;
   float *acts = nullptr, *dz = nullptr, *dz_last = nullptr, *pe_tile = nullptr, *out_buf = nullptr, *dout = nullptr;
   uint32_t* masks = nullptr;
+  float* chain_part = nullptr;
+  int chain_blk() const { return 4 * (AF_HID + (((skip >> (NL - 1)) & 1) ? 64 : 0)) + 4; }
 };
 
 struct Sched {
   std::vector<DwJob> jobs; std::vector<AdamJob> ajobs; std::vector<DwSeg> segs;
+  std::vector<int> ajob_of;
   int nwg = 0; size_t partial_floats = 0;
   DwJob* d_jobs = nullptr; AdamJob* d_ajobs = nullptr; DwSeg* d_segs = nullptr;
 };
@@ -285,8 +288,10 @@
 
 struct NetUse { NetDesc* n; int NT; int live_base = -1; int NT_plan = -1; };
 
+bool dw_in_chain(const af_handle* h, const NetDesc& n, int l) { return h->mlp_mode == 3 && l == n.NL - 1; }
+
 bool build_sched(af_handle* h, Sched& sc, const std::vector<NetUse>& uses) {
-  sc.jobs.clear(); sc.ajobs.clear(); sc.segs.clear();
+  sc.jobs.clear(); sc.ajobs.clear(); sc.segs.clear(); sc.ajob_of.clear();
   std::vector<int> job_nt, job_cap;
   int cur_live_base = -1, cur_cap = 0;
   auto add = [&](NetDesc& n, int NT, int l, int shape, const float* A, uint32_t as, const float* B, uint32_t bs,
@@ -295,9 +300,14 @@
     DwJob j{}; j.A = A; j.B = B; j.a_stride = as; j.b_stride = bs; j.shape = shape;
     if (cur_live_base >= 0) { j.live_base = cur_live_base; j.live_rows = h->live; }
     j.part_blk = (uint32_t)(To * 32 * Ti * 32 + To * 32);
-    sc.jobs.push_back(j); job_nt.push_back(NT); job_cap.push_back(cur_cap);
+    const bool in_chain = dw_in_chain(h, n, l);
+    if (!in_chain) { sc.jobs.push_back(j); job_nt.push_back(NT); job_cap.push_back(cur_cap); sc.ajob_of.push_back((int)sc.ajobs.size()); }
     AdamJob a{};
-    a.part_blk = j.part_blk; a.pld = Ti * 32; a.out_real = n.out_feat[l]; a.in_real = in_real; a.out_real_pad = To * 32;
+    a.part_blk = j.part_blk; a.pld = Ti * 32;
+    if (in_chain) {
+      a.chain_src = n.chain_part; a.part_blk = (uint32_t)n.chain_blk(); a.pld = 4; a.nslots = (uint32_t)((cur_cap + 3) / 4);
+      a.chain_bias = a.part_blk - 4;
+    } a.out_real = n.out_feat[l]; a.in_real = in_real; a.out_real_pad = To * 32;
     a.p_off = (uint32_t)(n.p_base + n.w_off[l] + col0); a.p_ld = n.in_feat[l]; a.col0 = col0;
     a.b_off = owns_bias ? (int32_t)(n.p_base + n.b_off[l]) : -1;
     a.f_off = (uint32_t)n.f_off[l]; a.f_mpad = n.f_mpad[l];
@@ -381,7 +391,7 @@
     for (size_t s = 0; s < wg[i].size() && s < DW_MAXSEG; ++s) sc.segs[(size_t)i * DW_MAXSEG + s] = wg[i][s];
   size_t off = 0;
   for (int j = 0; j < nj; ++j) {
-    sc.jobs[j].part_off = (uint32_t)off; sc.ajobs[j].part_off = (uint32_t)off; sc.ajobs[j].nslots = nslots[j];
+    sc.jobs[j].part_off = (uint32_t)off; sc.ajobs[sc.ajob_of[j]].part_off = (uint32_t)off; sc.ajobs[sc.ajob_of[j]].nslots = nslots[j];
     off += (size_t)nslots[j] * sc.jobs[j].part_blk;
   }
   sc.partial_floats = off;
@@ -432,6 +442,9 @@
   if ((e = dalloc(&n.pe_tile, n.pe_feats ? nt * 2048 : 1)) != hipSuccess) return e;
   if ((e = dalloc(&n.out_buf, rp * 4)) != hipSuccess) return e;
   if ((e = dalloc(&n.dout, rp * 4)) != hipSuccess) return e;
+  const size_t cp = (nt + 3) / 4 * (size_t)n.chain_blk();
+  if ((e = dalloc(&n.chain_part, cp)) != hipSuccess) return e;
+  if ((e = hipMemset(n.chain_part, 0, cp * 4)) != hipSuccess) return e;
   if ((e = hipMemset(n.dz_last, 0, nt * 1024 * 4)) != hipSuccess) return e;
   if (n.pe_feats && (e = hipMemset(n.pe_tile, 0, nt * 2048 * 4)) != hipSuccess) return e;
   if ((e = hipMemset(n.out_buf, 0, rp * 16)) != hipSuccess) return e;
@@ -449,7 +462,7 @@
 
 void free_net(NetDesc& n) {
   (void)hipFree(n.acts); (void)hipFree(n.dz); (void)hipFree(n.masks); (void)hipFree(n.dz_last); (void)hipFree(n.pe_tile); (void)hipFree(n.out_buf); (void)hipFree(n.dout);
-  (void)hipFree(n.coords); (void)hipFree(n.x0_tile);
+  (void)hipFree(n.coords); (void)hipFree(n.x0_tile); (void)hipFree(n.chain_part);
 }
 
 const float* chain_wimg(const af_handle* h, const NetDesc& n, bool fwd) {
@@ -474,6 +487,7 @@
   a.wimg = chain_wimg(h, n, false); a.out = n.out_buf; a.dout = n.dout; a.masks = n.masks;
   a.dz = n.dz; a.dz_last = n.dz_last; a.pe_tile = n.pe_tile; a.din0 = nullptr; a.din1 = nullptr; a.din_scale = 0.5f;
   a.split_row = 0x7fffffff; a.nrows = 0; a.NT = NT; a.nt_stride = NT; a.nl = n.NL;
+  a.acts = n.acts; a.chain_part = dw_in_chain(h, n, n.NL - 1) ? n.chain_part : nullptr; a.chain_blk = n.chain_blk();
   return a;
 }
 FwdArgs fp32_images(FwdArgs a, const af_handle* h, const NetDesc& n) { a.wimg = h->img_f + n.f_base; return a; }
@@ -525,6 +539,12 @@
 
 double part_rows(int tile0, int NT, int rows_total) { return (double)std::max(0, std::min(NT * 32, rows_total) - tile0 * 32); }
 
+double chain_dw_flops(const af_handle* h, int net) {
+  const NetDesc& n = h->nets[net];
+  return dw_in_chain(h, n, n.NL - 1) ? 2.0 * n.in_feat[n.NL - 1] * n.out_feat[n.NL - 1] : 0.0;
+}
+double kdw_flops(const af_handle* h, int net) { return h->flop_fwd[net] - chain_dw_flops(h, net); }
+
 struct FwdPart { int net; FwdArgs a; int rows_total; };
 struct BwdPart { int net; BwdArgs a; int rows_total; };
 
@@ -546,7 +566,8 @@
   for (const BwdPart& p : parts) {
     if (p.a.NT <= p.a.tile0) continue;
     m.net[m.n] = h->nets[p.net].kern; m.a[m.n] = p.a; ++m.n;
-    fl += part_rows(p.a.tile0, p.a.NT, p.rows_total) * h->flop_dx[p.net];
+    if (p.a.chain_part && (p.a.tile0 & 3)) return h->fail(AF_EINVAL, "backward launch: a part of a net with in-chain dW must start at a multiple of four row tiles");
+    fl += part_rows(p.a.tile0, p.a.NT, p.rows_total) * (h->flop_dx[p.net] + chain_dw_flops(h, p.net));
   }
   if (m.n == 0) return 0;
   if (h->step_stamp && (cls == T_BWD_1 || cls == T_BWD_2)) m.wg_stamp = h->step_stamp + (size_t)(cls == T_BWD_1 ? 2 : 3) * AF_STAMP_WG * 4;
@@ -649,7 +670,7 @@
                                       {AF_NET_MAP1, tile_range(bm, T2, NT_map), nseg * N}})) != 0) return rc;
     if ((rc = launch_bwd(h, T_BWD_2, {{AF_NET_MAP1, tile_range(bm, 0, T1), nseg * N}})) != 0) return rc;
   }
-  const double dwf = (double)nseg * N * h->flop_fwd[AF_NET_MAP1] + 3.0 * N * h->flop_fwd[AF_NET_ATLAS];
+  const double dwf = (double)nseg * N * kdw_flops(h, AF_NET_MAP1) + 3.0 * N * kdw_flops(h, AF_NET_ATLAS);
   return finish_step(h, sc, h->adam_m, h->adam_v, h->adam_step, loss_out, (N + 255) / 256, dwf);
 }
 
@@ -682,7 +703,7 @@
   }
   int rc;
   const int wg_atlas = (NT_atlas + 3) / 4, pad = (h->ncu - wg_atlas % h->ncu) % h->ncu;
-  const int T_al = std::max(0, std::min(NT_alpha, tiles_of(3 * N + h->plan_flow_rows)) - 4 * pad);
+  const int T_al = std::max(0, std::min(NT_alpha, tiles_of(3 * N + h->plan_flow_rows)) - 4 * pad) & ~3;
   const int flow_base = (nseg - 2) * N;
   const FwdArgs fal = with_live(fwd_args(h, AL, AL.coords, AL.out_buf, NT_alpha, true), h, 3 * N);
   FwdArgs fat = fwd_args(h, A, M1.out_buf, A.out_buf, NT_atlas, true);
@@ -715,7 +736,7 @@
     if ((rc = launch_bwd(h, T_BWD_2, {{AF_NET_ALPHA, tile_range(bal, 0, T_al), 5 * N}, {AF_NET_MAP1, with_live(bwd_args(h, M1, NT_map), h, flow_base), nseg * N},
                                       {AF_NET_MAP2, with_live(bwd_args(h, M2, NT_map), h, flow_base), nseg * N}})) != 0) return rc;
   }
-  const double dwf = (double)nseg * N * (h->flop_fwd[AF_NET_MAP1] + h->flop_fwd[AF_NET_MAP2]) + 6.0 * N * h->flop_fwd[AF_NET_ATLAS] + 5.0 * N * h->flop_fwd[AF_NET_ALPHA];
+  const double dwf = (double)nseg * N * (kdw_flops(h, AF_NET_MAP1) + kdw_flops(h, AF_NET_MAP2)) + 6.0 * N * kdw_flops(h, AF_NET_ATLAS) + 5.0 * N * kdw_flops(h, AF_NET_ALPHA);
   return finish_step(h, sc, h->adam_m, h->adam_v, h->adam_step, loss_out, (N + 255) / 256, dwf);
 }
 
@@ -871,6 +892,36 @@
 
 void af_set_thread_error(const char* m) { g_create_error = m; }
 
+static const char* describe_and_plan(af_handle* h, size_t& fc, size_t& bc, size_t& biasc, size_t& pc) {
+  const bool seg = h->seg;
+  const int nl_atlas = h->cfg.number_of_layers_atlas;
+  const unsigned atlas_skip = (nl_atlas > 4 ? (1u << 4) : 0u) | (nl_atlas > 7 ? (1u << 7) : 0u);
+  if (h->cfg.use_positional_encoding_mapping1) describe_net(h->nets[AF_NET_MAP1], AF_NET_MAP1, h->cfg.number_of_layers_mapping1, AF_IN_PE3, h->cfg.number_of_positional_encoding_mapping1, 2, 0u, false, h->cfg.number_of_channels_mapping1);
+  else describe_net(h->nets[AF_NET_MAP1], AF_NET_MAP1, h->cfg.number_of_layers_mapping1, AF_IN_XYT, 0, 2, 0u, false, h->cfg.number_of_channels_mapping1);
+  describe_net(h->nets[AF_NET_ATLAS], AF_NET_ATLAS, nl_atlas, AF_IN_PE2, h->cfg.positional_encoding_num_atlas, 3, atlas_skip, true, h->cfg.number_of_channels_atlas);
+  if (seg) {
+    if (h->cfg.use_positional_encoding_mapping2) describe_net(h->nets[AF_NET_MAP2], AF_NET_MAP2, h->cfg.number_of_layers_mapping2, AF_IN_PE3, h->cfg.number_of_positional_encoding_mapping2, 2, 0u, false, h->cfg.number_of_channels_mapping2);
+    else describe_net(h->nets[AF_NET_MAP2], AF_NET_MAP2, h->cfg.number_of_layers_mapping2, AF_IN_XYT, 0, 2, 0u, false, h->cfg.number_of_channels_mapping2);
+    describe_net(h->nets[AF_NET_ALPHA], AF_NET_ALPHA, h->cfg.number_of_layers_alpha, AF_IN_PE3, h->cfg.positional_encoding_num_alpha, 1, 0u, false, h->cfg.number_of_channels_alpha);
+  }
+  for (NetDesc& n : h->nets) if (n.used) {
+    auto lw = [&](int w) { return w == AF_HID ? n.hid : (w > AF_HID ? w - AF_HID + n.hid : w); };
+    double f = 0, d = n.dx0 ? (double)n.in_feat0 * n.hid : 0.0;
+    for (int l = 0; l < n.NL; ++l) {
+      const double lin = l == 0 ? n.in_feat0 : lw(n.in_feat[l]), lout = l == n.NL - 1 ? n.out : n.hid;
+      f += lin * lout; if (l >= 1) d += (double)n.hid * lout;
+    }
+    h->flop_fwd[n.id] = 2.0 * f; h->flop_dx[n.id] = 2.0 * d;
+  }
+  for (NetDesc& n : h->nets) if (n.used) {
+    n.p_base = pc; pc += n.nparams; plan_images(n, fc, bc, biasc);
+    if (!check_chunk_plan(n)) return "weight-image plan does not match the kernels' chunk sequence";
+    if (!plan_stream(n, n.bf, k_bf16x6, h->sf_bytes, h->sb_bytes)) return "bf16 stream plan does not match the kernels' chunk sizes";
+    if (!plan_stream(n, n.hf, k_f16x3, h->hf_bytes, h->hb_bytes)) return "fp16 stream plan does not match the kernels' chunk sizes";
+  }
+  return nullptr;
+}
+
 int af_create(const af_config* cfg, int device_ordinal, af_handle** out) {
   if (!cfg || !out) { g_create_error = "af_create: null argument"; return AF_EINVAL; }
   *out = nullptr;
@@ -906,32 +957,8 @@
   CCHK(hipStreamCreateWithFlags(&h->stream, hipStreamNonBlocking));
   CCHK((hipError_t)af_mlp_init()); CCHK((hipError_t)af_mlp16_init()); CCHK((hipError_t)af_dw_init()); CCHK((hipError_t)af_mlp_bf_init()); CCHK((hipError_t)af_mlp_hf_init());
 
-  const int nl_atlas = cfg->number_of_layers_atlas;
-  const unsigned atlas_skip = (nl_atlas > 4 ? (1u << 4) : 0u) | (nl_atlas > 7 ? (1u << 7) : 0u);
-  if (cfg->use_positional_encoding_mapping1) describe_net(h->nets[AF_NET_MAP1], AF_NET_MAP1, cfg->number_of_layers_mapping1, AF_IN_PE3, cfg->number_of_positional_encoding_mapping1, 2, 0u, false, cfg->number_of_channels_mapping1);
-  else describe_net(h->nets[AF_NET_MAP1], AF_NET_MAP1, cfg->number_of_layers_mapping1, AF_IN_XYT, 0, 2, 0u, false, cfg->number_of_channels_mapping1);
-  describe_net(h->nets[AF_NET_ATLAS], AF_NET_ATLAS, nl_atlas, AF_IN_PE2, cfg->positional_encoding_num_atlas, 3, atlas_skip, true, cfg->number_of_channels_atlas);
-  if (seg) {
-    if (cfg->use_positional_encoding_mapping2) describe_net(h->nets[AF_NET_MAP2], AF_NET_MAP2, cfg->number_of_layers_mapping2, AF_IN_PE3, cfg->number_of_positional_encoding_mapping2, 2, 0u, false, cfg->number_of_channels_mapping2);
-    else describe_net(h->nets[AF_NET_MAP2], AF_NET_MAP2, cfg->number_of_layers_mapping2, AF_IN_XYT, 0, 2, 0u, false, cfg->number_of_channels_mapping2);
-    describe_net(h->nets[AF_NET_ALPHA], AF_NET_ALPHA, cfg->number_of_layers_alpha, AF_IN_PE3, cfg->positional_encoding_num_alpha, 1, 0u, false, cfg->number_of_channels_alpha);
-  }
-  for (NetDesc& n : h->nets) if (n.used) {
-    auto lw = [&](int w) { return w == AF_HID ? n.hid : (w > AF_HID ? w - AF_HID + n.hid : w); };
-    double f = 0, d = n.dx0 ? (double)n.in_feat0 * n.hid : 0.0;
-    for (int l = 0; l < n.NL; ++l) {
-      const double lin = l == 0 ? n.in_feat0 : lw(n.in_feat[l]), lout = l == n.NL - 1 ? n.out : n.hid;
-      f += lin * lout; if (l >= 1) d += (double)n.hid * lout;
-    }
-    h->flop_fwd[n.id] = 2.0 * f; h->flop_dx[n.id] = 2.0 * d;
-  }
   size_t fc = 0, bc = 0, biasc = 0, pc = 0;
-  for (NetDesc& n : h->nets) if (n.used) {
-    n.p_base = pc; pc += n.nparams; plan_images(n, fc, bc, biasc);
-    if (!check_chunk_plan(n)) { h->fail(AF_EINVAL, "weight-image plan does not match the kernels' chunk sequence"); return die(AF_EINVAL); }
-    if (!plan_stream(n, n.bf, k_bf16x6, h->sf_bytes, h->sb_bytes)) { h->fail(AF_EINVAL, "bf16 stream plan does not match the kernels' chunk sizes"); return die(AF_EINVAL); }
-    if (!plan_stream(n, n.hf, k_f16x3, h->hf_bytes, h->hb_bytes)) { h->fail(AF_EINVAL, "fp16 stream plan does not match the kernels' chunk sizes"); return die(AF_EINVAL); }
-  }
+  if (const char* m = describe_and_plan(h, fc, bc, biasc, pc)) { h->fail(AF_EINVAL, m); return die(AF_EINVAL); }
   h->sf_bytes += 49152 + 65536; h->sb_bytes += 49152 + 65536;
   if (h->sf_bytes >= ((size_t)1 << 31) || h->sb_bytes >= ((size_t)1 << 31)) { h->fail(AF_EINVAL, "stream images exceed 2 GB"); return die(AF_EINVAL); }
   CCHK(hipMalloc((void**)&h->img_sf, h->sf_bytes)); CCHK(hipMalloc((void**)&h->img_sb, h->sb_bytes));
@@ -1170,7 +1197,9 @@
   if (!h) return AF_EINVAL;
   if (mode < 0 || mode > 3) return h->fail(AF_EINVAL, "af_set_mlp_mode: 0 (fp32 MFMA), 1 (bf16x6), 2 (bf16x6 forward, three-product bf16 backward chain) or 3 (f16x3: two-term fp16 split with a scale per row)");
   const int cls_old = chain_family(h->mlp_mode).cls, cls_new = chain_family(mode).cls;
+  const bool recut = (h->mlp_mode == 3) != (mode == 3);
   h->mlp_mode = mode;
+  if (recut) { const int rc = rebuild_dw_scheds(h); if (rc) return rc; }
   if (cls_new != cls_old && cls_new != 0) {
     HCHK(hipSetDevice(h->device));
     const int rc = repack(h, h->sched[0]); if (rc) return rc;
@@ -1253,7 +1282,7 @@
       if (hf) { if ((rc = launch_bwd(h, T_BWD_2, {{net, bwd_args(h, M, NT), NB}})) != 0) break; }
       else { Timer t(h, T_BWD_2, (double)NB * h->flop_dx[net]); const BwdArgs ba = fp32_images(bwd_args(h, M, NT), h, M);
         if (af_launch_bwd16(M.kern, &ba, h->stream)) { rc = h->fail(AF_EHIP, "bwd16"); break; } }
-      rc = finish_step(h, sc, h->pre_m, h->pre_v, (long long)s + 1, h->loss_log + s * AF_LOSS_W, (NB + 255) / 256, (double)NB * h->flop_fwd[net], false);
+      rc = finish_step(h, sc, h->pre_m, h->pre_v, (long long)s + 1, h->loss_log + s * AF_LOSS_W, (NB + 255) / 256, (double)NB * kdw_flops(h, net), false);
     }
   hipError_t e = hipStreamSynchronize(h->stream);
   drain_timers(h);
@@ -1373,6 +1402,41 @@
   return AF_OK;
 }
 
+int af_debug_plan_sched(const af_config* cfg, int ncu, int mlp_mode, int which, int32_t* shapes, int cap, int32_t* chain) {
+  if (!cfg || ncu <= 0 || mlp_mode < 0 || mlp_mode > 3 || which < 0 || which > 3 || cfg->samples_batch <= 0) return AF_EINVAL;
+  auto layers_ok = [](int n) { return n >= 2 && n <= AF_MAX_LAYERS; };
+  if (!layers_ok(cfg->number_of_layers_mapping1) || !layers_ok(cfg->number_of_layers_atlas)) return AF_EINVAL;
+  if (cfg->two_layer && (!layers_ok(cfg->number_of_layers_mapping2) || !layers_ok(cfg->number_of_layers_alpha))) return AF_EINVAL;
+  if (which == 3 && !cfg->two_layer) return AF_EINVAL;
+  af_handle hd; af_handle* h = &hd;
+  h->cfg = *cfg; h->seg = cfg->two_layer != 0; h->ncu = ncu; h->mlp_mode = mlp_mode; h->N = cfg->samples_batch;
+  if (h->cfg.pretrain_batch <= 0) h->cfg.pretrain_batch = 10000;
+  size_t fc = 0, bc = 0, biasc = 0, pc = 0;
+  if (describe_and_plan(h, fc, bc, biasc, pc)) return AF_EINVAL;
+  bool ok;
+  if (which < 2) ok = build_main_scheds(h);
+  else ok = build_sched(h, h->sched[which], {{&h->nets[which == 2 ? AF_NET_MAP1 : AF_NET_MAP2], tiles_of(h->cfg.pretrain_batch)}});
+  if (!ok) return AF_EINVAL;
+  const Sched& sc = h->sched[which];
+  for (int j = 0; j < (int)sc.jobs.size() && j < cap; ++j) if (shapes) shapes[j] = sc.jobs[j].shape;
+  if (chain) {
+    for (int i = 0; i < 2 * AF_MAX_NETS; ++i) chain[i] = 0;
+    for (size_t i = 0; i < sc.ajobs.size(); ++i) {
+      if (std::find(sc.ajob_of.begin(), sc.ajob_of.end(), (int)i) != sc.ajob_of.end()) continue;
+      const AdamJob& a = sc.ajobs[i];
+      for (int n = 0; n < AF_MAX_NETS; ++n)
+        if (h->nets[n].used && a.p_off >= h->nets[n].p_base && a.p_off < h->nets[n].p_base + h->nets[n].nparams) { chain[2 * n] = (int32_t)a.nslots; chain[2 * n + 1] = (int32_t)a.part_blk; }
+    }
+  }
+  return (int)sc.jobs.size();
+}
+
+int af_debug_chain_slots(int tile0, int NT, int32_t out2[2]) {
+  if (!out2 || tile0 < 0 || NT < tile0 || (tile0 & 3)) return AF_EINVAL;
+  out2[0] = af_chain_slot(tile0, 0); out2[1] = (NT - tile0 + 3) / 4;
+  return AF_OK;
+}
+
 int af_debug_dw_clocks(af_handle* h, int enable, uint64_t* out, int cap_wg) {
   if (!h) return AF_EINVAL;
   HCHK(hipSetDevice(h->device)); HCHK(hipStreamSynchronize(h->stream));
diff --git a/all-in-one-deflicker_amd/csrc/mlphf.hip b/all-in-one-deflicker_amd/csrc/mlphf.hip
--- a/all-in-one-deflicker_amd/csrc/mlphf.hip
+++ b/all-in-one-deflicker_amd/csrc/mlphf.hip
@@ -302,10 +302,76 @@
   return mx;
 }
 
+#define AF_CHAIN_WAVE_BYTES 6144
+AF_DEV float* chain_dw_block(const BwdArgs& a, int wg) { return a.chain_part + (size_t)af_chain_slot(a.tile0, wg) * a.chain_blk; }
+AF_DEV void chain_dw_zero(const BwdArgs& a, int wg, int tid) {
+  float* blk = chain_dw_block(a, wg);
+  for (int i = tid * 4; i < a.chain_blk; i += 1024) *(f32x4*)(blk + i) = f32x4{0.f, 0.f, 0.f, 0.f};
+}
+struct ChainDwOps { f32x4 bv[8], av[4][8], pv[8]; };
+template <class NS>
+AF_DEV void chain_dw_load(ChainDwOps& o, const BwdArgs& a, int nl, int lane, int tile) {
+  const float* xl = a.acts + ((size_t)(nl - 2) * a.nt_stride + tile) * AF_TILE_F + lane * 32;
+  const float* dzp = a.dz_last + ((size_t)tile * 32 + (lane & 3)) * 32;
+#pragma unroll
+  for (int q = 0; q < 8; ++q) o.bv[q] = *(const f32x4*)(dzp + 4 * q);
+#pragma unroll
+  for (int g = 0; g < 4; ++g)
+#pragma unroll
+    for (int q = 0; q < 8; ++q) o.av[g][q] = *(const f32x4*)(xl + g * 64 * 32 + 4 * q);
+  if constexpr (NS::SKIP != 0) {
+    if (ChunkBytes<NS>::out_skip(nl)) {
+      const float* pt = a.pe_tile + (size_t)tile * 64 * 32 + lane * 32;
+#pragma unroll
+      for (int q = 0; q < 8; ++q) o.pv[q] = *(const f32x4*)(pt + 4 * q);
+    }
+  }
+  __builtin_amdgcn_sched_barrier(0);
+}
+AF_DEV f32x4 chain_dw_group(const f32x4 (&av)[8], const f32x4 (&bv)[8]) {
+  f32x4 acc = {0.f, 0.f, 0.f, 0.f};
+#pragma unroll
+  for (int r = 0; r < 32; ++r) acc = __builtin_amdgcn_mfma_f32_4x4x1f32(av[r >> 2][r & 3], bv[r >> 2][r & 3], acc, 0, 0, 0);
+  return acc;
+}
+template <class NS>
+AF_DEV void chain_out_dw(const ChainDwOps& o, const BwdArgs& a, int nl, int wg, int tid, int wave, int lane, bool live, char* smem) {
+  const bool skip = NS::SKIP != 0 && ChunkBytes<NS>::out_skip(nl);
+  const int nhid = 256 + (skip ? 64 : 0);
+  __builtin_amdgcn_sched_barrier(0);
+  f32x4 g4[5];
+#pragma unroll
+  for (int g = 0; g < 4; ++g) g4[g] = chain_dw_group(o.av[g], o.bv);
+  g4[4] = f32x4{0.f, 0.f, 0.f, 0.f};
+  if constexpr (NS::SKIP != 0) {
+    if (skip) g4[4] = chain_dw_group(o.pv, o.bv);
+  }
+  float db = 0.f;
+#pragma unroll
+  for (int r = 0; r < 32; ++r) db += o.bv[r >> 2][r & 3];
+  __builtin_amdgcn_sched_barrier(0);
+  af_wait_vm0();
+  __syncthreads();
+  f32x4* mine = (f32x4*)(smem + wave * AF_CHAIN_WAVE_BYTES);
+  const f32x4 z4 = {0.f, 0.f, 0.f, 0.f};
+#pragma unroll
+  for (int g = 0; g < 4; ++g) mine[g * 64 + lane] = live ? g4[g] : z4;
+  if (skip) mine[256 + lane] = live ? g4[4] : z4;
+  if (lane < 4) ((float*)(mine + nhid))[lane] = live ? db : 0.f;
+  __syncthreads();
+  float* blk = chain_dw_block(a, wg);
+  for (int v = tid; v <= nhid; v += 256) {
+    f32x4 s = *(const f32x4*)(smem + v * 16);
+#pragma unroll
+    for (int w = 1; w < 4; ++w) s += *(const f32x4*)(smem + w * AF_CHAIN_WAVE_BYTES + v * 16);
+    *(f32x4*)(blk + 4 * v) = s;
+  }
+}
+
 template <class NS>
 AF_DEV void mlp_bwd_body_hf(const BwdArgs& a, int wg, char* smem) {
   ChainRows cr;
-  if (!chain_rows(a, wg, cr)) return;
+  if (!chain_rows(a, wg, cr)) { if (a.chain_part) chain_dw_zero(a, wg, cr.tid); return; }
   const int tid = cr.tid, wave = cr.wave, lane = cr.lane, j = cr.j, h = cr.h, tile = cr.tile, row = cr.row; const bool live = cr.live;
 
   using CB = ChunkBytesHf<NS>;
@@ -367,15 +433,20 @@
   hf_finish_range<3, 0>(in, fin, std::make_integer_sequence<int, 128>{});
   AF_ELEMWISE_FENCE();
 
+  ChainDwOps ops;
   if constexpr (NS::DX0) {
     f32x16 acc2[2];
     mm_block<2, 16, 0, 4, true>(acc2, in, lane_base + (h * 64 + j) * 16, hook_dma_store);
     const char* half2 = cs.publish(CB::BL0C);
     mm_block<2, 16, 64, 4>(acc2, in, half2 + (h * 64 + j) * 16, hook_dma);
+    if (a.chain_part) chain_dw_load<NS>(ops, a, nl, lane, tile);
     chain_dpe_to_uv<NS>(a, acc2, row, tile, j, h, live);
   } else {
+    if (a.chain_part) chain_dw_load<NS>(ops, a, nl, lane, tile);
     ts.all(in);
   }
+  HF_MARK(29);
+  if (a.chain_part) chain_out_dw<NS>(ops, a, nl, wg, tid, wave, lane, live, smem);
   HF_MARK(30);
 }
 
diff --git a/include/atlasfit.h b/include/atlasfit.h
--- a/include/atlasfit.h
+++ b/include/atlasfit.h
@@ -122,6 +122,8 @@
 int af_debug_forward(af_handle* h, int net, const float* in, int rows, float* out);
 int af_debug_tiles(af_handle* h, int net, int which, int layer, int nt_stride, int tile0, int ntiles, float* out);
 int af_debug_plan(int ncu, int rows_map, int rows_atlas, int dep_rows, int out3[3]);
+int af_debug_plan_sched(const af_config* cfg, int ncu, int mlp_mode, int which, int32_t* shapes, int cap, int32_t* chain);
+int af_debug_chain_slots(int tile0, int NT, int32_t out2[2]);
 int af_debug_dw_clocks(af_handle* h, int enable, uint64_t* out, int cap_wg);
 int af_debug_step_clocks(af_handle* h, int enable, uint64_t* out, int cap_wg);
 int af_debug_dw_schedule(af_handle* h, int which, int32_t* out, int cap_wg);
```

Result: slower. 11.42 million (-1.1%).
